# jasperlinthorst/reveal

Measured on AMD Instinct MI355X. Metric: Mbp/s indexed+MUM-anchored (reveal rem), higher is better.
Workload: dtype int32

## Files before the change

### include/reveal_amd.h

```cpp
#ifndef REVEAL_AMD_H
#define REVEAL_AMD_H
#include <stdint.h>

#ifdef __cplusplus
extern "C" {
#endif

typedef struct rv_index rv_index;

const char *rv_last_error(void);
int  rv_abi_version(void);
int  rv_sa_bits(void);
int  rv_device_count(void);

rv_index *rv_new(int device);
void rv_free(rv_index *h);

int rv_add_sample(rv_index *h);
int rv_add_sequence(rv_index *h, const char *seq, int64_t len, int64_t *begin, int64_t *end);
int rv_reset(rv_index *h);
int rv_reserve_text(rv_index *h, int64_t bytes);
int64_t rv_n(const rv_index *h);
int rv_nsamples(const rv_index *h);
int rv_nnodes(const rv_index *h);
int rv_add_sequences(rv_index *h, const char *text, int64_t total, const int64_t *lens, int64_t count);
int rv_node_list(const rv_index *h, int64_t *begin_end);

int rv_construct(rv_index *h, int rc, const char *safile, const char *lcpfile, int cache);
int rv_upload(rv_index *h);
int rv_upload_again(rv_index *h);

enum { RV_T = 0, RV_SA = 1, RV_SAI = 2, RV_LCP = 3, RV_SO = 4, RV_NSEP = 5, RV_NODES = 6 };
int64_t rv_get_array(rv_index *h, int which, void *out, int64_t cap);

int64_t rv_getmums(rv_index *h, int minl);
int rv_fetch_mums(rv_index *h, uint32_t *l, int64_t *a, int64_t *b, int64_t cap);
int64_t rv_getmultimums(rv_index *h, int minlength, int minn, int mems, int64_t *members);
int rv_fetch_multi(rv_index *h, uint32_t *l, int32_t *n, int64_t *off, uint16_t *so, int64_t *pos);

typedef struct {
    int64_t n;
    int32_t depth;
    int32_t nsamples;
    int32_t nnodes;
    int32_t parent;
    int32_t kind;
    int32_t reserved;
    int64_t nmums;
    int64_t nmembers;
} rv_sub;

int rv_align_begin(rv_index *h, int minl, int minn);
int rv_frontier_size(rv_index *h);
int rv_frontier_scan(rv_index *h);
int rv_sub_skip_scan(rv_index *h, int s);
int rv_sub_info(rv_index *h, int s, rv_sub *out);
int rv_sub_nodes(rv_index *h, int s, int64_t *begin_end );
int rv_sub_mums(rv_index *h, int s, uint32_t *l, int32_t *n, int64_t *off, uint16_t *so, int64_t *pos);
int64_t rv_sub_array(rv_index *h, int s, int which, void *out, int64_t cap);
int rv_sub_split(rv_index *h, int s, uint32_t l, int nsp, const int64_t *sp,
                 const int64_t *lead, int nlead, const int64_t *trail, int ntrail,
                 const int64_t *match, int nmatch, const int64_t *rest, int nrest);
int rv_frontier_commit(rv_index *h, int32_t *children);
int rv_align_end(rv_index *h);

typedef struct {
    int64_t steps;
    int64_t splits;
    int64_t anchored_bp;
    int32_t levels;
    int32_t maxdepth;
    int64_t scanned_ranks;
    double  t_scan, t_host, t_split, t_bubble;
} rv_align_stats;
int rv_align_builtin(rv_index *h, int minl, int minn, rv_align_stats *st);

int rv_align_builtin_until(rv_index *h, int minl, int minn, int stop_subs, rv_align_stats *st);
int rv_align_builtin_resume(rv_index *h, rv_align_stats *st);
int rv_align_builtin_continue(rv_index *h, int stop_subs, rv_align_stats *st);
int rv_frontier_counts(rv_index *h, int64_t *out);
int rv_frontier_export(rv_index *h, int64_t *meta, int64_t *node_first, int64_t *nodes);
int64_t rv_frontier_pack(rv_index *h, const int32_t *subs, int k, void *sa, void *lcp, void *bwt, int on_device);
int rv_frontier_import(rv_index *h, int minl, int minn, uint32_t maxlcp, int level, int nsubs, const int64_t *meta,
                       const int64_t *node_first, const int64_t *nodes, int64_t m,
                       const void *sa, const void *lcp, const void *bwt, int on_device);
int64_t rv_frontier_seeds_export(rv_index *h, const int32_t *subs, int k, int64_t *out, int64_t cap);
int rv_frontier_seeds_import(rv_index *h, int nsubs, const int64_t *words, int64_t nwords);
uint32_t rv_maxlcp(const rv_index *h);
int rv_cascade_info(const rv_index *h, int64_t *out);
int rv_capacity_events(const rv_index *h, int64_t *out);
const char *rv_cascade_why(const rv_index *h);
int64_t rv_anchor_count(rv_index *h, int64_t *members);
int rv_fetch_anchors(rv_index *h, uint32_t *l, int64_t *off, int64_t *pos);
int rv_set_result_buffers(rv_index *h, uint32_t *l, int64_t l_cap, int64_t *off, int64_t off_cap, int64_t *pos, int64_t pos_cap);
typedef struct {
    int64_t  key, n;
    int32_t  depth, nsamples, nnodes, picked;
    int64_t  nmums;
    uint32_t l; int32_t mn;
    int64_t  sp_min;
    uint64_t h_sa, h_lcp, h_mums;
} rv_trace;
int rv_set_trace(rv_index *h, int on);
int rv_set_preselect(rv_index *h, int64_t maxmums);
int rv_set_option(rv_index *h, const char *name, int64_t value);
int rv_get_option(rv_index *h, const char *name, int64_t *value);
int rv_set_launch_trace(int on);
int rv_option_count(void);
const char *rv_option_name(int k);
int64_t rv_trace_count(rv_index *h);
int rv_fetch_trace(rv_index *h, rv_trace *out, int64_t cap);

typedef struct rv_subindex rv_subindex;
rv_index *rv_clone(rv_index *h);
rv_subindex *rv_sx_main(rv_index *h);
rv_subindex *rv_sx_copy(rv_subindex *x);
void rv_sx_free(rv_subindex *x);
int rv_sx_info(const rv_subindex *x, rv_sub *out);
int rv_sx_nodes(const rv_subindex *x, int64_t *begin_end);
int64_t rv_sx_array(rv_subindex *x, int which, void *out, int64_t cap);
int64_t rv_sx_scan(rv_subindex *x, int minl, int minn, int64_t *members);
int rv_sx_fetch(rv_subindex *x, uint32_t *l, int32_t *n, int64_t *off, uint16_t *so, int64_t *pos);
int rv_sx_split(rv_subindex *x, const int64_t *lead, int nlead, const int64_t *trail, int ntrail,
                const int64_t *match, int nmatch, const int64_t *rest, int nrest, rv_subindex **out);
int rv_sx_extract(rv_subindex *x, int64_t *intervals, int niv);

int64_t rv_chain(int64_t m, int k, const uint32_t *len, const int32_t *nmem, const int64_t *crd, const int64_t *left,
                 const int64_t *right, int64_t wscore, int64_t wpen, int model, int64_t *out_idx, int64_t *out_score);

typedef struct { int64_t wscore, wpen, maxmums, seedsize; int gcmodel; int trim; double pcutoff; } rv_picker_args;
typedef struct {
    int picked; uint32_t pick_l; int32_t pick_n; int pick_members; uint16_t *pick_so; int64_t *pick_pos; int64_t member_cap;
    int64_t nleft, nright, nseed_members, seed_cap, seed_member_cap;
    uint32_t *seed_l; int32_t *seed_n; int64_t *seed_off; uint16_t *seed_so; int64_t *seed_pos; int64_t *seed_score; uint8_t *seed_right;
} rv_picker_out;
int rv_set_picker(rv_index *h, int kind, const rv_picker_args *args);
int rv_picker_info(const rv_index *h, int64_t *out);
int rv_pick_chain(const rv_picker_args *args, int nsub, int64_t m, const uint32_t *l, const int32_t *n, const int64_t *off, const uint16_t *so,
                  const int64_t *pos, int nsamples, const int64_t *seq_begin, const int64_t *iv_begin, const int64_t *iv_end, int minlength,
                  rv_picker_out *out);

typedef struct rv_graph rv_graph;
rv_graph *rv_graph_import(int64_t nnodes, const int64_t *node_b, const int64_t *node_e, const int8_t *node_aligned, const int8_t *node_sent,
                          const int64_t *off_ptr, const int32_t *off_sid, const int64_t *off_val,
                          int64_t nedges, const int32_t *edge_u, const int32_t *edge_v, const int64_t *edge_ptr, const int32_t *edge_paths,
                          const int64_t *pred_ptr, const int32_t *pred_edge, int npaths, const uint8_t *star, const int64_t *id2end,
                          int nstart, const int32_t *start_nodes, int literal_segments);
int rv_graph_pick(rv_graph *g, const rv_picker_args *args, int nsub, int64_t m, const uint32_t *l, const int32_t *n, const int64_t *off, const uint16_t *so, const int64_t *pos,
                  const int64_t *left, const int64_t *right, int minlength, rv_picker_out *out);
int rv_graph_align(rv_graph *g, const int64_t *nodes, int64_t nn, const int64_t *left, const int64_t *right, uint32_t l, const int64_t *pos, int npos,
                   int64_t *counts, int64_t *out6);
int rv_graph_align_fetch(rv_graph *g, int64_t *out);
int rv_set_graph_picker(rv_index *h, rv_graph *g, const rv_picker_args *args);
rv_graph *rv_graph_new(void);
int rv_graph_add_linear(rv_graph *g, int64_t b, int64_t e, int star);
int64_t rv_graph_read_gfa(rv_graph *g, rv_index *h, int64_t *text_n, const char *data, int64_t len, const char **names);
typedef struct GfaParsed rv_gfa_parsed;
rv_gfa_parsed *rv_gfa_parse(const char *data, int64_t len);
int64_t rv_graph_adopt(rv_graph *g, rv_index *h, int64_t *text_n, rv_gfa_parsed *parsed, const char **names);
void rv_gfa_parsed_free(rv_gfa_parsed *parsed);
int rv_graph_seal(rv_graph *g);
int rv_graph_paths(const rv_graph *g, int64_t *id2end);
int rv_graph_node_kinds(const rv_graph *g, int8_t *out);
int rv_graph_literal(const rv_graph *g);
int rv_graph_finish(rv_graph *g);
rv_graph *rv_graph_replay_begin(int nseq, const int64_t *begin, const int64_t *end);
int rv_set_replay_graph(rv_index *h, rv_graph *g);
rv_graph *rv_graph_replay(int nseq, const int64_t *begin, const int64_t *end, int64_t na, const uint32_t *an_l, const int64_t *an_off, const int64_t *an_pos);
const char *rv_graph_error(const rv_graph *g);
int rv_graph_sizes(const rv_graph *g, int64_t *out);
int rv_graph_export(const rv_graph *g, int64_t *node_b, int64_t *node_e, int8_t *node_aligned, int64_t *off_ptr, int32_t *off_sid, int64_t *off_val,
                    int64_t *succ_ptr, int32_t *succ_to, int32_t *succ_edge, int64_t *pred_ptr, int32_t *pred_from, int32_t *pred_edge, int64_t *edge_ptr, int32_t *edge_paths);
int rv_graph_prune(rv_graph *g, const char *T);
int64_t rv_graph_gfa(rv_graph *g, const char *T, int npaths, const char *const *names, const char *cmdline, const char **out);
void rv_graph_free(rv_graph *g);

enum { RV_K_SCAN_PAIR = 0, RV_K_SCAN_MULTI = 1, RV_K_SA_SORT = 2, RV_K_LCP = 3, RV_K_SPLIT = 4, RV_K_LABEL = 5,
       RV_K_BUBBLE = 6,
       RV_K_RADIX_SCATTER = 7, RV_K_RADIX_HIST = 8, RV_K_TEXT_ROUND = 9,
       RV_K_CASCADE = 10,
       RV_K_DIAG_TABLE = 11,
       RV_K_INIT_KEYS = 12,
       RV_K_PUBLISH = 13,
       RV_K_COUNT = 14 };
int rv_prof_enable(rv_index *h, int on);
int rv_prof_reset(rv_index *h);
int rv_prof_get(rv_index *h, int k, int64_t *launches, double *ms, double *bytes);
typedef struct rv_batch rv_batch;
rv_batch *rv_batch_new(void);
int rv_batch_add(rv_batch *b, rv_index *h);
int rv_batch_run(rv_batch *b, int minl, int minn, int construct, rv_align_stats *stats, int *status);
int rv_batch_info(const rv_batch *b, int64_t *out);
void rv_batch_free(rv_batch *b);
typedef struct rv_many rv_many;
rv_many *rv_many_new(int device);
void rv_many_free(rv_many *m);
int rv_many_option(rv_many *m, const char *name, int64_t value);
int rv_many_set_picker(rv_many *m, int kind, const rv_picker_args *args);
int64_t rv_many_add(rv_many *m, const char *const *seqs, const int64_t *lens, int k);
int rv_many_clear(rv_many *m);
int rv_many_run(rv_many *m, int minl, int minn, rv_align_stats *total);
int64_t rv_many_anchor_count(rv_many *m, int64_t *first, int64_t *members);
int rv_many_fetch(rv_many *m, uint32_t *l, int64_t *off, int64_t *pos);
int64_t rv_many_text(rv_many *m, int64_t job, char *out, int64_t cap);
int rv_many_info(const rv_many *m, int64_t *out);
int64_t rv_many_arrays(rv_many *m, int64_t job, int which, void *out, int64_t cap);
void *rv_dev_alloc(int device, int64_t bytes);
int rv_dev_free(int device, void *p);
int rv_ipc_export(int device, const void *p, uint8_t handle[64]);
void *rv_ipc_open(int device, const uint8_t handle[64]);
int rv_ipc_close(int device, void *p);
int rv_dev_copy(int device, void *dst, const void *src, int64_t bytes);
int rv_measure_bandwidth(int device, int64_t bytes, int iters, double *read_gbs, double *copy_gbs);
int rv_sa_stats(rv_index *h, int *sigma, int *bits, int *k0, int *rounds, int64_t *sorted_elems, int *radix_passes);
int rv_sa_diag_table(rv_index *h);
int rv_sa_tail(rv_index *h, int64_t *out);

int rv_test_exclusive_sum_u32(const uint32_t *in, uint32_t *out, int64_t n);
int rv_test_inclusive_max_u32(const uint32_t *in, uint32_t *out, int64_t n);
int rv_test_radix_sort(uint64_t *keys, uint32_t *vals, int64_t n, int bit_lo, int bit_hi);
int rv_test_radix_time(int64_t n, int bits, int dist, int flags, int iters, double *ms, int64_t *bad);

#ifdef __cplusplus
}
#endif
#endif
```

### reveal_amd/_index.py

```python
import ctypes
import mmap
import os
import sys
import numpy as np

from . import _lib
from ._lib import RV_T, RV_SA, RV_SAI, RV_LCP, RV_SO, RV_NSEP


def _page_array(count, dtype):
    nbytes = max(int(count), 1) * np.dtype(dtype).itemsize
    m = mmap.mmap(-1, (nbytes + mmap.PAGESIZE - 1) // mmap.PAGESIZE * mmap.PAGESIZE)
    return np.frombuffer(m, dtype=dtype, count=max(int(count), 1))


def _pairs(iv, sa64):
    a = np.ascontiguousarray(np.array([(int(b), int(e)) for b, e in iv], dtype=np.int64).reshape(-1, 2))
    return a, len(a)


_OPTION_DEFAULTS = {}


def make_index_type(sa64, error):
# ... 426 lines not shown
            if self._dll.rv_sx_extract(sx, a.ctypes.data, k) != 0:
                self._fail()
            if isinstance(intervals, list):
                for q in range(k):
                    if (a[q] != before[q]).any():
                        intervals[q] = (int(a[q][0]), int(a[q][1]))
            return None

        def copy(self):
            if not self._constructed:
                raise TypeError("Index not yet constructed.")
            if self._slot is not None:
                raise error("not available on a sub-index handed to an align() callback")
            c = index.__new__(index)
            c._lib, c._dll = self._lib, self._dll
            c._safile, c._lcpfile, c._cache = "", "", 0
            c._samples, c._nodes, c.skipmums = list(self._samples), set(self._nodes), list(self.skipmums)
            c._leftnode, c._rightnode, c._depth = self._leftnode, self._rightnode, self._depth
            c._constructed, c._slot, c._sx = True, None, None
            c._n_sub = c._nsamples_sub = None
            c._rc = getattr(self, "_rc", 0)
            if self._main is self:
                if self._sx:
                    raise error("copy() after extract() / splitindex() on the main index is not supported")
                c._h = self._dll.rv_clone(self._h)
                if not c._h:
                    self._fail()
                c._main = c
            else:
                c._h, c._main = self._h, self._main
                c._samples = self._main._samples
                c._sx = self._dll.rv_sx_copy(self._sx)
                if not c._sx:
                    self._fail()
            return c

        def preselect(self, maxmums):
            if self._depth != 0:
                raise error("preselect() is set on the main index")
            if self._dll.rv_set_preselect(self._h, int(maxmums or 0)) != 0:
                self._fail()

        def align_builtin(self, minl=20, minn=2, trace=False):
            if not self._constructed:
                raise error("Index not yet constructed, alignment stopped.")
            dll, h = self._dll, self._h
            dll.rv_set_trace(h, 1 if trace else 0)
            self._offer_result_buffers()
            st = _lib.RvAlignStats()
            if dll.rv_align_builtin(h, int(minl), int(minn), ctypes.byref(st)) != 0:
                self._fail()
            return self._builtin_result(st, trace)

        def set_picker(self, args=None):
            from . import schemes
            if args is None:
                r = self._dll.rv_set_picker(self._h, 0, None)
            else:
                if args.maxsize is not None or args.maxdepth is not None:
                    raise error("the native picker does not take --maxbubblesize / maxdepth")
                A = schemes._RvPickerArgs(int(args.wscore), int(args.wpen), int(args.maxmums or 0), int(args.seedsize or 0), schemes.GCMODELS[args.gcmodel],
                                          1 if args.trim else 0, float(args.pcutoff))
                r = self._dll.rv_set_picker(self._h, 1, ctypes.byref(A))
            if r != 0:
                self._fail()

        def set_replay_graph(self, graph=None):
            if graph is not None and graph._dll is not self._dll:
                raise error("the graph was made by the other build of the library (32 / 64-bit suffix arrays)")
            if self._dll.rv_set_replay_graph(self._h, None if graph is None else graph._g) != 0:
                self._fail()

        def _sync_nodes(self):
            self._nodes_stale = False
            k = self._dll.rv_nnodes(self._h)
            if k != len(self._nodes):
                buf = np.zeros(2 * max(k, 1), np.int64)
                if self._dll.rv_node_list(self._h, buf.ctypes.data) != 0:
                    self._fail()
                self._nodes = set(map(tuple, buf[:2 * k].reshape(-1, 2).tolist()))
                self._constructed = False

        def set_graph_picker(self, graph=None, args=None):
            from . import schemes
            if graph is None:
                r = self._dll.rv_set_graph_picker(self._h, None, None)
            else:
                if args.maxsize is not None or args.maxdepth is not None:
                    raise error("the native picker does not take --maxbubblesize / maxdepth")
                if graph._dll is not self._dll:
                    raise error("the graph was made by the other build of the library (32 / 64-bit suffix arrays)")
                A = schemes._RvPickerArgs(int(args.wscore), int(args.wpen), int(args.maxmums or 0), int(args.seedsize or 0), schemes.GCMODELS[args.gcmodel],
                                          1 if args.trim else 0, float(args.pcutoff))
                r = self._dll.rv_set_graph_picker(self._h, graph._g, ctypes.byref(A))
            if r != 0:
                self._fail()

        def picker_info(self):
            o = (ctypes.c_int64 * 6)()
            self._dll.rv_picker_info(self._h, o)
            return dict(kind=int(o[0]), calls=int(o[1]), seeded=int(o[2]), picker_s=o[3] / 1e9, lists_s=o[4] / 1e9, graphalign_s=o[5] / 1e9)

        def _result_buffers_free(self):
            c = self.__dict__.get("_res_bufs")
            if c is not None and sys.getrefcount(c[0]) == 2 and sys.getrefcount(c[1]) == 2 and sys.getrefcount(c[2]) == 2:
                return c
            return None

        def _offer_result_buffers(self):
            c = self._result_buffers_free()
            if c is not None:
                self._dll.rv_set_result_buffers(self._h, c[0].ctypes.data, len(c[0]), c[1].ctypes.data, len(c[1]), c[2].ctypes.data, len(c[2]))
            else:
                self._dll.rv_set_result_buffers(self._h, None, 0, None, 0, None, 0)

        def _builtin_result(self, st, trace):
            dll, h = self._dll, self._h
            mem = ctypes.c_int64(0)
            na = dll.rv_anchor_count(h, ctypes.byref(mem))
            c = self._result_buffers_free()
            if c is not None and len(c[0]) >= max(na, 1) and len(c[1]) >= na + 1 and len(c[2]) >= max(mem.value, 1):
                l, off, pos = c
            else:
                dll.rv_set_result_buffers(h, None, 0, None, 0, None, 0)
                if os.environ.get("RV_RESULT_BUFS", "") == "heap":
                    l = np.empty(max(na, 1), dtype=np.uint32); off = np.empty(na + 1, dtype=np.int64); pos = np.empty(max(mem.value, 1), dtype=np.int64)
                else:
                    l = _page_array(max(na, 1), np.uint32); off = _page_array(na + 1, np.int64); pos = _page_array(max(mem.value, 1), np.int64)
                self.__dict__["_res_bufs"] = (l, off, pos)
            c = None
            off[0] = 0
            if dll.rv_fetch_anchors(h, l.ctypes.data, off.ctypes.data, pos.ctypes.data) != 0:
                self._fail()
            tr = None
            if trace:
                nt = dll.rv_trace_count(h)
                tr = np.zeros(max(nt, 1), dtype=_lib.TRACE_DTYPE)
                if dll.rv_fetch_trace(h, tr.ctypes.data, len(tr)) != 0:
                    self._fail()
                tr = tr[:nt]
            stats = {f[0]: getattr(st, f[0]) for f in _lib.RvAlignStats._fields_}
            return dict(stats=stats, anchors=(l[:na], off[:na + 1], pos[:mem.value]), trace=tr)

        @property
        def maxlcp(self):
            return int(self._dll.rv_maxlcp(self._h))

        def cascade_info(self):
            o = np.zeros(8, dtype=np.int64)
            self._dll.rv_cascade_info(self._h, o.ctypes.data)
            return dict(done=bool(o[0]), levels=int(o[1]), matches=int(o[2]), witnesses=int(o[3]), subindices=int(o[4]), undecided=int(o[5]), rebuilt_ranks=int(o[6]), decided_from_witnesses=int(o[7]),
                        why=(self._dll.rv_cascade_why(self._h) or b"").decode())

        def capacity_events(self):
            o = np.zeros(len(_lib.CAPACITY_EVENTS), dtype=np.int64)
            if self._dll.rv_capacity_events(self._main._h, o.ctypes.data) != 0:
                self._fail()
            return {k: int(v) for k, v in zip(_lib.CAPACITY_EVENTS, o)}

        def align_builtin_until(self, stop_subs, minl=20, minn=2, trace=False):
            if not self._constructed:
                raise error("Index not yet constructed, alignment stopped.")
            self._dll.rv_set_trace(self._h, 1 if trace else 0)
            self._offer_result_buffers()
            self._st = _lib.RvAlignStats()
            self._trace = bool(trace)
            r = self._dll.rv_align_builtin_until(self._h, int(minl), int(minn), int(stop_subs), ctypes.byref(self._st))
            if r < 0:
                self._fail()
            self._pending = r > 0
            return r

        def align_builtin_continue(self, stop_subs):
            if not getattr(self, "_pending", False):
                return 0
            self._offer_result_buffers()
            r = self._dll.rv_align_builtin_continue(self._h, int(stop_subs), ctypes.byref(self._st))
            if r < 0:
                self._fail()
            self._pending = r > 0
            return r

        def frontier(self):
            c = np.zeros(4, dtype=np.int64)
            if self._dll.rv_frontier_counts(self._h, c.ctypes.data) != 0:
                self._fail()
            ns, m, nn, level = (int(x) for x in c)
            meta = np.zeros((max(ns, 1), 6), dtype=np.int64); nf = np.zeros(ns + 1, dtype=np.int64); nodes = np.zeros((max(nn, 1), 2), dtype=np.int64)
            if self._dll.rv_frontier_export(self._h, meta.ctypes.data, nf.ctypes.data, nodes.ctypes.data) != 0:
                self._fail()
            return dict(level=level, m=m, meta=meta[:ns], node_first=nf, nodes=nodes[:nn])

        def frontier_pack(self, subs, sa, lcp, bwt):
            subs = np.ascontiguousarray(subs, dtype=np.int32)
            ptr, dev = _pointers(sa, lcp, bwt)
            r = self._dll.rv_frontier_pack(self._h, subs.ctypes.data, len(subs), ptr[0], ptr[1], ptr[2], dev)
            if r < 0:
                self._fail()
            return int(r)

        def frontier_seeds(self, subs):
            subs = np.ascontiguousarray(subs, dtype=np.int32)
            need = self._dll.rv_frontier_seeds_export(self._h, subs.ctypes.data, len(subs), None, 0)
            if need < 0:
                self._fail()
            out = np.zeros(max(int(need), 1), dtype=np.int64)
            if self._dll.rv_frontier_seeds_export(self._h, subs.ctypes.data, len(subs), out.ctypes.data, int(need)) != need:
                self._fail()
            return out[:int(need)]

        def frontier_import(self, part, sa, lcp, bwt, minl=20, minn=2, maxlcp=None, trace=False):
            meta = np.ascontiguousarray(part["meta"], dtype=np.int64).reshape(-1, 6)
            nf = np.ascontiguousarray(part["node_first"], dtype=np.int64); nodes = np.ascontiguousarray(part["nodes"], dtype=np.int64).reshape(-1, 2)
            m = int(meta[:, 1].sum()) if len(meta) else 0
            ptr, dev = _pointers(sa, lcp, bwt)
            self._offer_result_buffers()
            if not getattr(self, "_pending", False):
                self._dll.rv_set_trace(self._h, 1 if trace else 0)
                self._st = _lib.RvAlignStats()
                self._trace = bool(trace)
            ml = self.maxlcp if maxlcp is None else int(maxlcp)
            if self._dll.rv_frontier_import(self._h, int(minl), int(minn), ml, int(part.get("level", 1)), len(meta), meta.ctypes.data, nf.ctypes.data,
                                            nodes.ctypes.data, m, ptr[0], ptr[1], ptr[2], dev) != 0:
                self._fail()
            self._pending = True
            seeds = part.get("seeds")
            if seeds is not None and len(seeds) > len(meta):
                seeds = np.ascontiguousarray(seeds, dtype=np.int64)
                if self._dll.rv_frontier_seeds_import(self._h, len(meta), seeds.ctypes.data, len(seeds)) != 0:
                    self._fail()

        def align_builtin_resume(self):
            if getattr(self, "_pending", False):
                self._offer_result_buffers()
                if self._dll.rv_align_builtin_resume(self._h, ctypes.byref(self._st)) != 0:
                    self._fail()
            self._pending = False
            return self._builtin_result(self._st, self._trace)

        def _fetch_sub_mums(self, s, info):
            cnt, mem = info.nmums, info.nmembers
            l = np.zeros(max(cnt, 1), dtype=np.uint32); n = np.zeros(max(cnt, 1), dtype=np.int32)
            off = np.zeros(cnt + 1, dtype=np.int64)
            so = np.zeros(max(mem, 1), dtype=np.uint16); pos = np.zeros(max(mem, 1), dtype=np.int64)
            if self._dll.rv_sub_mums(self._h, s, l.ctypes.data, n.ctypes.data, off.ctypes.data, so.ctypes.data, pos.ctypes.data) != 0:
                self._fail()
            return _csr_to_tuples(cnt, l, n, off, so, pos)

        def __reduce__(self):
            return None

    index.__name__ = "index"
    index.__qualname__ = "index"
    return index


def _pointers(*bufs):
    ptr, dev = [], None
    for b in bufs:
        on_dev = bool(getattr(b, "is_cuda", False))
        if dev is not None and on_dev != dev:
            raise ValueError("sa, lcp and bwt must live in the same kind of memory")
        dev = on_dev
        if hasattr(b, "data_ptr"):
            if not b.is_contiguous():
                raise ValueError("contiguous buffers needed")
            ptr.append(b.data_ptr())
        else:
            if not b.flags["C_CONTIGUOUS"]:
                raise ValueError("contiguous buffers needed")
            ptr.append(b.ctypes.data)
    return ptr, 1 if dev else 0


def _csr_to_tuples(cnt, l, n, off, so, pos):
    l, n, off = l.tolist(), n.tolist(), off.tolist()
    members = list(zip(so.tolist(), pos.tolist()))
    return [(l[k], n[k], tuple(members[off[k]:off[k + 1]])) for k in range(cnt)]
```

### reveal_amd/_lib.py

```python
import ctypes
import importlib.util
import os
import sys
import numpy as np

_HERE = os.path.dirname(os.path.abspath(__file__))

RV_T, RV_SA, RV_SAI, RV_LCP, RV_SO, RV_NSEP, RV_NODES = range(7)
K_SCAN_PAIR, K_SCAN_MULTI, K_SA_SORT, K_LCP, K_SPLIT, K_LABEL, K_BUBBLE, K_RADIX_SCATTER, K_RADIX_HIST, K_TEXT_ROUND, K_CASCADE, K_DIAG_TABLE, K_INIT_KEYS, K_PUBLISH = range(14)

CAPACITY_EVENTS = ("pair_ovf", "pair_out", "pair_pick_ovf", "pair_second_copy", "multi_rec", "multi_mem", "multi_cand",
                   "mems_rec", "mems_mem", "mems_long")
CAP_SITES = {"multi_cand": 1, "cas_wit": 2, "cas_tables": 4, "casm_matches": 8, "casm_wit": 16, "casm_tables": 32,
             "mems_rec": 64, "mems_mem": 128, "mems_long": 256}

c_i64p = ctypes.POINTER(ctypes.c_int64)
V = ctypes.c_void_p


class RvSub(ctypes.Structure):
    _fields_ = [("n", ctypes.c_int64), ("depth", ctypes.c_int32), ("nsamples", ctypes.c_int32),
                ("nnodes", ctypes.c_int32), ("parent", ctypes.c_int32), ("kind", ctypes.c_int32),
                ("reserved", ctypes.c_int32), ("nmums", ctypes.c_int64), ("nmembers", ctypes.c_int64)]


class RvAlignStats(ctypes.Structure):
    _fields_ = [("steps", ctypes.c_int64), ("splits", ctypes.c_int64), ("anchored_bp", ctypes.c_int64),
                ("levels", ctypes.c_int32), ("maxdepth", ctypes.c_int32), ("scanned_ranks", ctypes.c_int64),
                ("t_scan", ctypes.c_double), ("t_host", ctypes.c_double), ("t_split", ctypes.c_double),
                ("t_bubble", ctypes.c_double)]


TRACE_DTYPE = np.dtype([("key", np.int64), ("n", np.int64), ("depth", np.int32), ("nsamples", np.int32),
                        ("nnodes", np.int32), ("picked", np.int32), ("nmums", np.int64), ("l", np.uint32),
                        ("mn", np.int32), ("sp_min", np.int64), ("h_sa", np.uint64), ("h_lcp", np.uint64),
                        ("h_mums", np.uint64)], align=True)

_I, _L, _D = ctypes.c_int, ctypes.c_int64, ctypes.c_double
SYMBOLS = {
    "rv_last_error": (ctypes.c_char_p, []),
    "rv_abi_version": (_I, []),
    "rv_sa_bits": (_I, []),
    "rv_device_count": (_I, []),
    "rv_new": (V, [_I]),
    "rv_free": (None, [V]),
    "rv_add_sample": (_I, [V]),
    "rv_add_sequence": (_I, [V, ctypes.c_char_p, _L, c_i64p, c_i64p]),
    "rv_reset": (_I, [V]),
    "rv_reserve_text": (_I, [V, _L]),
    "rv_n": (_L, [V]),
    "rv_nsamples": (_I, [V]),
    "rv_nnodes": (_I, [V]),
    "rv_node_list": (_I, [V, V]),
    "rv_construct": (_I, [V, _I, ctypes.c_char_p, ctypes.c_char_p, _I]),
    "rv_upload": (_I, [V]),
    "rv_upload_again": (_I, [V]),
    "rv_get_array": (_L, [V, _I, V, _L]),
    "rv_getmums": (_L, [V, _I]),
    "rv_fetch_mums": (_I, [V, V, V, V, _L]),
    "rv_getmultimums": (_L, [V, _I, _I, _I, c_i64p]),
    "rv_fetch_multi": (_I, [V, V, V, V, V, V]),
    "rv_align_begin": (_I, [V, _I, _I]),
    "rv_frontier_size": (_I, [V]),
    "rv_frontier_scan": (_I, [V]),
    "rv_sub_skip_scan": (_I, [V, _I]),
    "rv_sub_info": (_I, [V, _I, ctypes.POINTER(RvSub)]),
    "rv_sub_nodes": (_I, [V, _I, V]),
    "rv_sub_mums": (_I, [V, _I, V, V, V, V, V]),
    "rv_sub_array": (_L, [V, _I, _I, V, _L]),
    "rv_sub_split": (_I, [V, _I, ctypes.c_uint32, _I, V, V, _I, V, _I, V, _I, V, _I]),
    "rv_frontier_commit": (_I, [V, V]),
    "rv_align_end": (_I, [V]),
    "rv_align_builtin": (_I, [V, _I, _I, ctypes.POINTER(RvAlignStats)]),
    "rv_align_builtin_until": (_I, [V, _I, _I, _I, ctypes.POINTER(RvAlignStats)]),
    "rv_align_builtin_resume": (_I, [V, ctypes.POINTER(RvAlignStats)]),
    "rv_align_builtin_continue": (_I, [V, _I, ctypes.POINTER(RvAlignStats)]),
    "rv_frontier_counts": (_I, [V, V]),
    "rv_frontier_export": (_I, [V, V, V, V]),
    "rv_frontier_pack": (_L, [V, V, _I, V, V, V, _I]),
    "rv_frontier_import": (_I, [V, _I, _I, ctypes.c_uint32, _I, _I, V, V, V, _L, V, V, V, _I]),
    "rv_frontier_seeds_export": (_L, [V, V, _I, V, _L]),
    "rv_frontier_seeds_import": (_I, [V, _I, V, _L]),
    "rv_maxlcp": (ctypes.c_uint32, [V]),
    "rv_cascade_info": (ctypes.c_int, [V, V]),
    "rv_cascade_why": (ctypes.c_char_p, [V]),
    "rv_capacity_events": (_I, [V, V]),
    "rv_anchor_count": (_L, [V, c_i64p]),
    "rv_fetch_anchors": (_I, [V, V, V, V]),
    "rv_set_result_buffers": (_I, [V, V, _L, V, _L, V, _L]),
    "rv_set_trace": (_I, [V, _I]),
    "rv_set_preselect": (_I, [V, _L]),
    "rv_set_option": (_I, [V, ctypes.c_char_p, _L]),
    "rv_set_launch_trace": (_I, [_I]),
    "rv_batch_new": (V, []),
    "rv_batch_add": (_I, [V, V]),
    "rv_batch_run": (_I, [V, _I, _I, _I, V, V]),
    "rv_batch_info": (_I, [V, V]),
    "rv_batch_free": (None, [V]),
    "rv_dev_alloc": (V, [_I, _L]),
    "rv_dev_free": (_I, [_I, V]),
    "rv_ipc_export": (_I, [_I, V, V]),
    "rv_ipc_open": (V, [_I, V]),
    "rv_ipc_close": (_I, [_I, V]),
    "rv_dev_copy": (_I, [_I, V, V, _L]),
    "rv_get_option": (_I, [V, ctypes.c_char_p, c_i64p]),
    "rv_option_count": (_I, []),
    "rv_option_name": (ctypes.c_char_p, [_I]),
    "rv_trace_count": (_L, [V]),
    "rv_fetch_trace": (_I, [V, V, _L]),
    "rv_clone": (V, [V]),
    "rv_sx_main": (V, [V]),
    "rv_sx_copy": (V, [V]),
    "rv_sx_free": (None, [V]),
    "rv_sx_info": (_I, [V, ctypes.POINTER(RvSub)]),
    "rv_sx_nodes": (_I, [V, V]),
    "rv_sx_array": (_L, [V, _I, V, _L]),
    "rv_sx_scan": (_L, [V, _I, _I, c_i64p]),
    "rv_sx_fetch": (_I, [V, V, V, V, V, V]),
    "rv_sx_split": (_I, [V, V, _I, V, _I, V, _I, V, _I, V]),
    "rv_sx_extract": (_I, [V, V, _I]),
    "rv_chain": (_L, [_L, _I, V, V, V, V, V, _L, _L, _I, V, V]),
    "rv_prof_enable": (_I, [V, _I]),
    "rv_prof_reset": (_I, [V]),
    "rv_prof_get": (_I, [V, _I, c_i64p, ctypes.POINTER(_D), ctypes.POINTER(_D)]),
    "rv_measure_bandwidth": (_I, [_I, _L, _I, ctypes.POINTER(_D), ctypes.POINTER(_D)]),
    "rv_sa_stats": (_I, [V] + [ctypes.POINTER(_I)] * 4 + [c_i64p, ctypes.POINTER(_I)]),
    "rv_sa_diag_table": (_I, [V]),
    "rv_sa_tail": (_I, [V, c_i64p]),
    "rv_set_picker": (_I, [V, _I, V]),
    "rv_picker_info": (_I, [V, c_i64p]),
    "rv_pick_chain": (_I, [V, _I, _L, V, V, V, V, V, _I, V, V, V, _I, V]),
    "rv_graph_import": (V, [_L, V, V, V, V, V, V, V, _L, V, V, V, V, V, V, _I, V, V, _I, V, _I]),
    "rv_graph_pick": (_I, [V, V, _I, _L, V, V, V, V, V, V, V, _I, V]),
    "rv_graph_align": (_I, [V, V, _L, V, V, ctypes.c_uint32, V, _I, V, V]),
    "rv_graph_align_fetch": (_I, [V, V]),
    "rv_graph_finish": (_I, [V]),
    "rv_set_graph_picker": (_I, [V, V, V]),
    "rv_graph_new": (V, []),
    "rv_graph_replay_begin": (V, [_I, V, V]),
    "rv_set_replay_graph": (_I, [V, V]),
    "rv_graph_add_linear": (_I, [V, _L, _L, _I]),
    "rv_graph_read_gfa": (_L, [V, V, V, V, _L, V]),
    "rv_graph_paths": (_I, [V, V]),
    "rv_graph_seal": (_I, [V]),
    "rv_gfa_parse": (V, [V, _L]),
    "rv_graph_adopt": (_L, [V, V, V, V, V]),
    "rv_gfa_parsed_free": (None, [V]),
    "rv_add_sequences": (_I, [V, V, _L, V, _L]),
    "rv_graph_node_kinds": (_I, [V, V]),
    "rv_graph_literal": (_I, [V]),
    "rv_graph_replay": (V, [_I, V, V, _L, V, V, V]),
    "rv_graph_error": (ctypes.c_char_p, [V]),
    "rv_graph_sizes": (_I, [V, c_i64p]),
    "rv_graph_export": (_I, [V] * 15),
    "rv_graph_prune": (_I, [V, V]),
    "rv_graph_gfa": (_L, [V, V, _I, V, V, V]),
    "rv_graph_free": (None, [V]),
    "rv_many_new": (V, [_I]),
    "rv_many_free": (None, [V]),
    "rv_many_option": (_I, [V, ctypes.c_char_p, _L]),
    "rv_many_set_picker": (_I, [V, _I, V]),
    "rv_many_add": (_L, [V, V, V, _I]),
    "rv_many_clear": (_I, [V]),
    "rv_many_run": (_I, [V, _I, _I, ctypes.POINTER(RvAlignStats)]),
    "rv_many_anchor_count": (_L, [V, V, c_i64p]),
    "rv_many_fetch": (_I, [V, V, V, V]),
    "rv_many_text": (_L, [V, _L, V, _L]),
    "rv_many_info": (_I, [V, V]),
    "rv_many_arrays": (_L, [V, _L, _I, V, _L]),
    "rv_test_exclusive_sum_u32": (_I, [V, V, _L]),
    "rv_test_inclusive_max_u32": (_I, [V, V, _L]),
    "rv_test_radix_sort": (_I, [V, V, _L, _I, _I]),
    "rv_test_radix_time": (_I, [_L, _I, _I, _I, _I, ctypes.POINTER(_D), c_i64p]),
}


def _share_torch_runtime():
    if os.environ.get("RV_SYSTEM_HIP") or "torch" in sys.modules:
        return
    try:
        spec = importlib.util.find_spec("torch")
    except (ImportError, ValueError):
        spec = None
    if spec is None or not spec.origin:
        return
    path = os.path.join(os.path.dirname(spec.origin), "lib", "libamdhip64.so")
    if os.path.exists(path):
        ctypes.CDLL(path, mode=ctypes.RTLD_GLOBAL)


class Lib:
    def __init__(self, sa64=False):
        self.sa64 = sa64
        _share_torch_runtime()
        name = "libreveal_amd64.so" if sa64 else "libreveal_amd.so"
        self.path = os.path.join(os.environ.get("RV_LIB_DIR") or _HERE, name)
        if not os.path.exists(self.path):
            raise ImportError("%s is missing: build it with `python -c 'import __graft_entry__ as g; g.build()'` "
                              "(hipcc --offload-arch=gfx950); reveal_amd has no CPU fallback" % self.path)
        self.dll = ctypes.CDLL(self.path)
        for sym, (res, args) in SYMBOLS.items():
            fn = getattr(self.dll, sym)
            fn.restype, fn.argtypes = res, args
        self.sa_t = np.int64 if sa64 else np.int32
        self.lcp_t = np.uint32 if sa64 else np.int32
        assert self.dll.rv_sa_bits() == (64 if sa64 else 32)
        v = os.environ.get("RV_LAUNCH_TRACE")
        if v is not None and v.strip() not in ("", "0"):
            self.dll.rv_set_launch_trace(1)

    def err(self):
        return (self.dll.rv_last_error() or b"").decode(errors="replace")


_libs = {}
_device = 0


def set_device(i):
    global _device
    _device = int(i)


def device():
    return _device


def measure_bandwidth(nbytes=1 << 30, iters=10):
    lib = get(False)
    r, c = _D(0), _D(0)
    if lib.dll.rv_measure_bandwidth(device(), int(nbytes), int(iters), ctypes.byref(r), ctypes.byref(c)) != 0:
        raise RuntimeError(lib.err())
    return r.value, c.value


def set_launch_trace(on=True):
    return [bool(get(w).dll.rv_set_launch_trace(1 if on else 0)) for w in (False, True)]
# ... 7 lines not shown
```

### reveal_amd/csrc/rv_align.hip

```cpp
#include "rv_index.h"
#include "rv_split.h"
#include "rv_decide.h"
static_assert(RV_TSUB_TILE == RV_SPLIT_TILE, "one tile -> sub-index table serves the split passes and the multi-sample picker");
#include "rv_leaf.h"
#include "rv_cascade.h"
#include <string.h>
#include <algorithm>
#include <chrono>
#include <thread>
#include <atomic>
#include "rv_graphrem.h"

namespace {

double now_s() {
    return std::chrono::duration<double>(std::chrono::steady_clock::now().time_since_epoch()).count();
}

u64 hash_step(u64 acc, u64 i, int64_t v) {
    u64 x = (u64)v + (i + 1) * 0x9E3779B97F4A7C15ULL;
    x ^= x >> 30; x *= 0xbf58476d1ce4e5b9ULL;
    x ^= x >> 27; x *= 0x94d049bb133111ebULL;
    x ^= x >> 31;
    return acc + x;
// ... 1799 lines not shown
        th.emplace_back([=]() { for (size_t k = lo; k < hi; k++) off[k] = base + 2 * (int64_t)(k + 1); });
    }
    for (size_t k = 0; k < na / nt; k++) off[k] = base + 2 * (int64_t)(k + 1);
    for (auto &x : th) x.join();
}
static int builtin_finish(rv_index *h, rv_align_stats *out) {
    Align *a = h->al;
    hipStream_t q = h->ws.stream;
    h->rb.direct = false;
    if (a->use_leaf && a->running) {
        u32 *lf_counters = a->lf_counters; u32 *lf_l = a->lf_l; int64_t *lf_pos = a->lf_pos; rv_trace *lf_tr = a->lf_tr;
        RV_HIP(hipStreamSynchronize(a->leaf_stream));
        RV_HIP(hipStreamSynchronize(a->leaf_stream2));
        for (int k = 0; k <= RV_LEVEL_BUFS; k++) a->leaf_pending[k] = false;
        RV_TRY(a->hLeafOut.reserve(256));
        RV_HIP(hipMemcpyAsync(a->hLeafOut.p, lf_counters, 128, hipMemcpyDeviceToHost, q));
        RV_HIP(hipStreamSynchronize(q));
        u32 cnt[4]; unsigned long long stv[8];
        memcpy(cnt, a->hLeafOut.p, sizeof cnt); memcpy(stv, a->hLeafOut.as<uint8_t>() + 64, sizeof stv);
        if (h->ws.opt.leaf_prof)
            fprintf(stderr, "leaf: steps %llu splits %llu | cycles idle %llu scan %llu split %llu bubble %llu\n", stv[0], stv[1], stv[4], stv[5], stv[6], stv[7]);
        if (cnt[2]) { rv_set_error(cnt[2] & 4u ? "leaf kernel: recursion stack overflow" : "leaf kernel: a sub-index does not match its intervals"); return -1; }
        if (cnt[0] > a->leaf_anchor_cap || cnt[1] > a->leaf_trace_cap) { rv_set_error("leaf kernel: output buffer too small"); return -1; }
        a->leaf_na = 0;
        if (cnt[0]) {
            const size_t na = cnt[0];
            const size_t nl = a->an_l.size(), np = a->an_pos.size();
            rv_index::ResultBufs &rb = h->rb;
            rb.direct = rb.l && (int64_t)(nl + na) <= rb.l_cap && (int64_t)(nl + na + 1) <= rb.off_cap && (int64_t)(np + 2 * na) <= rb.pos_cap;
            int64_t *pp; u32 *pl;
            if (rb.direct) { pp = rb.pos + np; pl = rb.l + nl; }
            else { RV_TRY(a->hLeafOut.reserve(na * 20 + 64)); pp = a->hLeafOut.as<int64_t>(); pl = (u32 *)(pp + 2 * na); }
            const size_t sent = (rb.direct && a->early_l == pl && a->early_pos == pp) ? std::min(a->early_sent, na) : 0;
            if (sent < na) {
                RV_HIP(hipMemcpyAsync(pp + 2 * sent, lf_pos + 2 * sent, (na - sent) * 16, hipMemcpyDeviceToHost, a->leaf_stream));
                RV_HIP(hipMemcpyAsync(pl + sent, lf_l + sent, (na - sent) * 4, hipMemcpyDeviceToHost, a->leaf_stream));
            }
            RV_TRY(rv_ensure_working_text(h));
            RV_TRY(rv_leaf_lower_launch(h->ws, h->dT.as<uint8_t>(), lf_pos, lf_l, (u32)na));
            if (rb.direct) fill_offsets(rb.off + nl + 1, na, (int64_t)np);
            RV_HIP(hipStreamSynchronize(a->leaf_stream));
            RV_HIP(hipStreamSynchronize(q));
            a->leaf_na = na;
        }
        if (a->trace_on && cnt[1]) {
            const size_t at = a->trace.size();
            a->trace.resize(at + cnt[1]);
            RV_HIP(hipMemcpy(a->trace.data() + at, lf_tr, (size_t)cnt[1] * sizeof(rv_trace), hipMemcpyDeviceToHost));
        }
        a->st.steps += (int64_t)stv[0]; a->st.splits += (int64_t)stv[1]; a->st.anchored_bp += (int64_t)stv[2];
        if ((int64_t)stv[3] > a->st.maxdepth) a->st.maxdepth = (int32_t)stv[3];
    }
    a->running = false;
    if (out) *out = a->st;
    return 0;
}

static int install_frontier(rv_index *h, int level, int nsubs, const int64_t *meta, const int64_t *node_first, const int64_t *nodes, int64_t m,
                            const void *sa, const void *lcp, const void *bwt, int on_device);
static int builtin_cascade(rv_index *h) {
    Align *a = h->al;
    memset(&a->cas_out, 0, sizeof a->cas_out);
    if (a->trace_on || h->rc != 0 || h->n <= RV_LEAF_N || a->minl < 4 || h->ws.opt.no_cascade || a->picker != 0) return 0;
    const bool second_try = !a->multi && a->use_leaf && h->ws.opt.cascade_second == 2;
    auto interval_cascade = [&]() -> int {
        RvCascadeMultiOut mo;
        RV_TRY(rv_cascade_multi_run(h, a->cas, a->minl, &mo));
        a->cas_out.done = mo.done; a->cas_out.levels = mo.levels; a->cas_out.cands = mo.cands; a->cas_out.witnesses = mo.witnesses; a->cas_out.children = mo.children;
        a->cas_out.undecided = mo.undecided; a->cas_out.rebuilt_ranks = mo.rebuilt_ranks; a->cas_out.why = mo.why;
        if (!mo.done) return 0;
        const int k = h->nsamples;
        a->st.splits += (int64_t)mo.an_l.size(); a->st.steps += mo.steps; a->st.levels += mo.levels; a->st.scanned_ranks += h->n;
        if (mo.maxdepth > a->st.maxdepth) a->st.maxdepth = mo.maxdepth;
        h->main_arrays_freed = true;
        if (mo.undecided > 0) {
            RV_TRY(install_frontier(h, 1, (int)mo.undecided, mo.meta.data(), mo.node_first.data(), mo.nodes.data(), mo.rebuilt_ranks, mo.d_sa, mo.d_lcp, mo.d_bwt, 1));
        } else {
            a->lv.clear();
            a->level = 1;
        }
        {
            const size_t na = mo.an_l.size(), l0 = a->an_l.size(), p0 = a->an_pos.size(), o0 = a->an_off.size();
            a->an_l.insert(a->an_l.end(), mo.an_l.begin(), mo.an_l.end());
            a->an_pos.resize(p0 + na * (size_t)k);
            for (size_t x = 0; x < na * (size_t)k; x++) a->an_pos[p0 + x] = (int64_t)mo.an_pos[x];
            a->an_off.resize(o0 + na);
            for (size_t x = 0; x < na; x++) a->an_off[o0 + x] = (int64_t)(p0 + (x + 1) * (size_t)k);
            int64_t bp = 0;
            for (size_t x = 0; x < na; x++) bp += mo.an_l[x];
            a->st.anchored_bp += bp;
            (void)l0;
        }
        return 0;
    };
    if (a->multi || second_try) return interval_cascade();
    if (!a->use_leaf) return 0;
    RvCascadeIO io;
    io.anchor_count = a->lf_counters; io.anchor_cap = (u32)a->leaf_anchor_cap; io.anchor_l = a->lf_l; io.anchor_pos = a->lf_pos;
    io.stats = a->lf_stats; io.leaf_err = a->lf_counters + 2;
    io.stage_cap = (u32)h->ws.opt.leaf_acap;
    RvCascadeHost hx;
    hx.side = a->leaf_stream;
    a->early_sent = 0;
    if (h->rb.l) {
        const int64_t nl = (int64_t)a->an_l.size(), np = (int64_t)a->an_pos.size();
        const int64_t room = std::min(std::min(h->rb.l_cap - nl, h->rb.off_cap - nl - 1), (h->rb.pos_cap - np) / 2);
        if (room > 0) { hx.l = h->rb.l + nl; hx.pos = h->rb.pos + np; hx.cap = (u32)std::min<int64_t>(room, 0xffffffffll); }
    }
    io.lvSA = &a->lvSA[0]; io.lvLCP = &a->lvLCP[0]; io.lvBWT = &a->lvBWT[0]; io.roots = &a->dLeafRoots[0];
    const int dmode = (int)h->ws.opt.cascade_danger;
    RV_TRY(rv_cascade_run(h, a->cas, io, a->minl, &a->cas_out, dmode == 2 ? 1 : 0, 0, &hx));
    if (!a->cas_out.done && a->cas_out.undecided > 0 && dmode == 1) {
        RV_HIP(hipMemsetAsync(a->dLeaf.p, 0, 256, h->ws.stream));
        RV_TRY(rv_cascade_run(h, a->cas, io, a->minl, &a->cas_out, 1, 1, &hx));
    }
    if (!a->cas_out.done) {
        if (hx.l) RV_HIP(hipStreamSynchronize(a->leaf_stream));
        RV_HIP(hipMemsetAsync(a->dLeaf.p, 0, 256, h->ws.stream));
        if (a->cas_out.undecided > 0 && !h->ws.opt.cascade_second_off) return interval_cascade();
        return 0;
    }
    a->st.levels += a->cas_out.levels;
    a->st.scanned_ranks += h->n;
    a->early_sent = a->cas_out.sent; a->early_l = hx.l; a->early_pos = hx.pos;
    if (!a->cas.lin_rest.empty() && h->nodes.size() > 2) {
        std::vector<RvIntv> rest, gone;
        for (size_t k = 0; k + 1 < a->cas.lin_rest.size(); k += 2) rest.push_back({a->cas.lin_rest[k], a->cas.lin_rest[k + 1]});
        std::sort(rest.begin(), rest.end(), intv_less);
        for (const RvIntv &v : h->nodes) {
            if (v.end <= v.begin) continue;
            const auto it = std::lower_bound(rest.begin(), rest.end(), v, intv_less);
            if (it == rest.end() || it->begin != v.begin) gone.push_back(v);
        }
        RV_TRY(add_decision(h, 0, 0, nullptr, 0, gone.data(), (int)gone.size(), nullptr, 0, nullptr, 0, rest.data(), (int)rest.size()));
        a->dec.drop_lead = true;
        RV_TRY(rv_frontier_commit(h, nullptr));
        for (size_t s2 = 0; s2 < a->lv.depth.size(); s2++) a->lv.depth[s2] = a->cas.lin_rest_depth;
        return 0;
    }
    h->main_arrays_freed = true;
    a->level = 1;
    a->lv.clear();
    return 0;
}

int rv_cascade_info(const rv_index *h, int64_t *out) {
    for (int k = 0; k < 8; k++) out[k] = 0;
    if (!h->al) return 0;
    const RvCascadeOut &c = h->al->cas_out;
    out[0] = c.done ? 1 : 0; out[1] = c.levels; out[2] = c.cands; out[3] = c.witnesses; out[4] = c.children; out[5] = c.undecided; out[6] = c.rebuilt_ranks; out[7] = c.solved;
    return 0;
}

const char *rv_cascade_why(const rv_index *h) {
    if (!h->al || h->al->cas_out.done || !h->al->cas_out.why) return "";
    return h->al->cas_out.why;
}

int rv_align_builtin(rv_index *h, int minl, int minn, rv_align_stats *out) {
    RV_TRY(builtin_setup(h, minl, minn));
    Align *a = h->al;
    if (a->replay_graph && a->picker == 1) {
        a->feed = rv_replay_feed_start(a->replay_graph);
        a->fed = 0;
        a->replay_graph = nullptr;
        if (!a->feed) return -1;
    }
    int rc = builtin_cascade(h);
    if (rc == 0) rc = builtin_levels(h, 0);
    if (rc == 0) rc = builtin_finish(h, out);
    if (a->feed) {
        RvReplayFeed *f = a->feed; a->feed = nullptr;
        if (rc == 0) { if (rv_replay_feed_finish(f) != 0) return -1; }
        else { const std::string keep = rv_last_error(); (void)rv_replay_feed_finish(f); rv_set_error("%s", keep.c_str()); }
    }
    return rc;
}

int rv_align_builtin_until(rv_index *h, int minl, int minn, int stop_subs, rv_align_stats *out) {
    RV_TRY(builtin_setup(h, minl, minn));
    RV_TRY(builtin_cascade(h));
    RV_TRY(builtin_levels(h, stop_subs));
    Align *a = h->al;
    if (a->lv.size() == 0) { RV_TRY(builtin_finish(h, out)); return 0; }
    if (out) *out = a->st;
    return a->lv.size();
}

int rv_align_builtin_continue(rv_index *h, int stop_subs, rv_align_stats *out) {
    RV_TRY(need_align(h));
    if (!h->al->running) { rv_set_error("no built-in run in progress (rv_align_builtin_until / rv_frontier_import)"); return -1; }
    if (stop_subs < 1) { rv_set_error("rv_align_builtin_continue: stop_subs must be positive"); return -1; }
    RV_HIP(hipSetDevice(h->device));
    Align *a = h->al;
    RV_TRY(builtin_levels(h, std::max(stop_subs, a->lv.size() + 1)));
    if (a->lv.size() == 0) { RV_TRY(builtin_finish(h, out)); return 0; }
    if (out) *out = a->st;
    return a->lv.size();
}

int rv_align_builtin_resume(rv_index *h, rv_align_stats *out) {
    RV_TRY(need_align(h));
    if (!h->al->running) { rv_set_error("no built-in run in progress (rv_align_builtin_until / rv_frontier_import)"); return -1; }
    RV_HIP(hipSetDevice(h->device));
    RV_TRY(builtin_levels(h, 0));
    return builtin_finish(h, out);
}

int rv_frontier_counts(rv_index *h, int64_t *out) {
    RV_TRY(need_align(h));
    const Level &lv = h->al->lv;
    out[0] = lv.size(); out[1] = lv.size() ? lv.m : 0; out[2] = (int64_t)lv.nodes.size(); out[3] = h->al->level;
    return 0;
}

int rv_frontier_export(rv_index *h, int64_t *meta, int64_t *node_first, int64_t *nodes) {
    RV_TRY(need_align(h));
    if (h->al->picker == 2) { rv_set_error("rv_frontier_export: a run on a graph (rv_set_graph_picker) is not handed off -- its sub-indices share the graph"); return -1; }
    const Level &lv = h->al->lv;
    for (int s = 0; s < lv.size(); s++) {
        int64_t *m6 = meta + 6 * (size_t)s;
        m6[0] = lv.off[(size_t)s]; m6[1] = lv.n[(size_t)s]; m6[2] = lv.depth[(size_t)s]; m6[3] = lv.nsamples[(size_t)s]; m6[4] = lv.kind[(size_t)s]; m6[5] = lv.parent[(size_t)s];
    }
    for (size_t k = 0; k < lv.node_first.size(); k++) node_first[k] = lv.node_first[k];
    for (size_t k = 0; k < lv.nodes.size(); k++) { nodes[2 * k] = lv.nodes[k].begin; nodes[2 * k + 1] = lv.nodes[k].end; }
    return 0;
}

int64_t rv_frontier_pack(rv_index *h, const int32_t *subs, int k, void *sa, void *lcp, void *bwt, int on_device) {
    if (need_align(h)) return -1;
    Align *a = h->al;
    if (hipSetDevice(h->device) != hipSuccess) { rv_set_error("hipSetDevice failed"); return -1; }
    hipStream_t q = h->ws.stream;
    const Level &lv = a->lv;
    const hipMemcpyKind kind = on_device ? hipMemcpyDeviceToDevice : hipMemcpyDeviceToHost;
    int64_t at = 0;
    for (int i = 0; i < k;) {
        if (subs[i] < 0 || subs[i] >= lv.size()) { rv_set_error("sub-index %d out of range", (int)subs[i]); return -1; }
        int j = i;
        int64_t cnt = lv.n[(size_t)subs[i]];
        while (j + 1 < k && subs[j + 1] == subs[j] + 1) { j++; cnt += lv.n[(size_t)subs[j]]; }
        const int64_t off = lv.off[(size_t)subs[i]];
        hipError_t e = hipMemcpyAsync((sa_t *)sa + at, cur_sa(h) + off, (size_t)cnt * sizeof(sa_t), kind, q);
        if (e == hipSuccess) e = hipMemcpyAsync((lcp_t *)lcp + at, cur_lcp(h) + off, (size_t)cnt * sizeof(lcp_t), kind, q);
        if (e == hipSuccess) e = hipMemcpyAsync((uint8_t *)bwt + at, cur_bwt(h) + off, (size_t)cnt, kind, q);
        if (e != hipSuccess) { rv_set_error("rv_frontier_pack: copy failed: %s", hipGetErrorString(e)); return -1; }
        at += cnt;
        i = j + 1;
    }
    if (hipStreamSynchronize(q) != hipSuccess) { rv_set_error("rv_frontier_pack: stream failed"); return -1; }
    return at;
}

static int install_frontier(rv_index *h, int level, int nsubs, const int64_t *meta, const int64_t *node_first, const int64_t *nodes, int64_t m,
                            const void *sa, const void *lcp, const void *bwt, int on_device) {
    hipStream_t q = h->ws.stream;
    Align *a = h->al;
    RV_HIP(hipStreamSynchronize(q));
    if (a->leaf_stream) { RV_HIP(hipStreamSynchronize(a->leaf_stream)); RV_HIP(hipStreamSynchronize(a->leaf_stream2)); }
    for (int k = 0; k <= RV_LEVEL_BUFS; k++) a->leaf_pending[k] = false;
    RV_HIP(hipMemsetAsync(a->dErr.p, 0, 64, q));
    Level &lv = a->lv;
    lv.clear();
    int64_t off = 0;
    for (int s = 0; s < nsubs; s++) {
        const int64_t *m6 = meta + 6 * (size_t)s;
        const int64_t nf = node_first[s], nl = node_first[s + 1];
        if (m6[1] <= 0 || nf > nl) { rv_set_error("rv_frontier_import: bad sub-index %d", s); return -1; }
        lv.off.push_back(off); lv.n.push_back(m6[1]); lv.depth.push_back((int32_t)m6[2]); lv.nsamples.push_back((int32_t)m6[3]);
        lv.kind.push_back((int32_t)m6[4]); lv.parent.push_back(-1);
        for (int64_t k = nf; k < nl; k++) {
            if (nodes[2 * k] < 0 || nodes[2 * k + 1] > h->nT || nodes[2 * k] > nodes[2 * k + 1]) { rv_set_error("rv_frontier_import: interval outside the text"); return -1; }
            lv.nodes.push_back({nodes[2 * k], nodes[2 * k + 1]});
        }
        lv.node_first.push_back((int64_t)lv.nodes.size());
        off += m6[1];
    }
    if (off != m) { rv_set_error("rv_frontier_import: the sub-index sizes add up to %lld, not %lld", (long long)off, (long long)m); return -1; }
    lv.m = m;
    a->nx.clear();
    a->level = std::max(level, 1);
    a->cur = 0;
    RV_TRY(a->lvSA[0].reserve((size_t)(m + 64) * sizeof(sa_t)));
    RV_TRY(a->lvLCP[0].reserve((size_t)(m + 64) * sizeof(lcp_t)));
    RV_TRY(a->lvBWT[0].reserve((size_t)m + 64));
    const hipMemcpyKind kind = on_device ? hipMemcpyDeviceToDevice : hipMemcpyHostToDevice;
    if (m) {
        RV_HIP(hipMemcpyAsync(a->lvSA[0].p, sa, (size_t)m * sizeof(sa_t), kind, q));
        RV_HIP(hipMemcpyAsync(a->lvLCP[0].p, lcp, (size_t)m * sizeof(lcp_t), kind, q));
        RV_HIP(hipMemcpyAsync(a->lvBWT[0].p, bwt, (size_t)m, kind, q));
    }
    prep_level_tables(h, lv, m);
    a->pk.clear();
    RV_TRY(publish_next_tables(h, a->dTab0, lv.nsamples, false));
    RV_HIP(hipStreamSynchronize(q));
    a->cur_dev_ok = a->next_dev_ok; a->early_done = false; a->early_bubble = false;
    a->scanned = false; a->d_err = nullptr;
    a->dec.reset(lv.size());
    a->skip_scan.assign((size_t)lv.size(), 0);
    a->seeds_cur.clear(); a->seeds_lead.clear(); a->seeds_trail.clear();
    return 0;
}


int rv_frontier_import(rv_index *h, int minl, int minn, uint32_t maxlcp, int level, int nsubs, const int64_t *meta,
                       const int64_t *node_first, const int64_t *nodes, int64_t m, const void *sa, const void *lcp, const void *bwt, int on_device) {
// ... 431 lines not shown
```

### reveal_amd/csrc/rv_cascade.h

```cpp
#pragma once
#include "rv_common.h"
#include <vector>

struct RvCascadeBufs {
    DBuf d[40];
    HBuf hstage, hstage2;
    u32 M = 0, NW = 0;
    u32 lin_roots = 0, lin_picks = 0, lin_nA = 0, lin_nB = 0;
    int64_t lin_steps = 0; int lin_maxdepth = 0; size_t lin_off[6] = {0, 0, 0, 0, 0, 0};
    std::vector<int64_t> lin_rest; int lin_rest_depth = 0;
    hipStream_t prio_stream = nullptr; hipEvent_t ev_in = nullptr, ev_out = nullptr;
    void release() {
        for (auto &b : d) b.release(); hstage.release(); hstage2.release();
        if (prio_stream) { (void)hipStreamDestroy(prio_stream); prio_stream = nullptr; }
        if (ev_in) { (void)hipEventDestroy(ev_in); ev_in = nullptr; }
        if (ev_out) { (void)hipEventDestroy(ev_out); ev_out = nullptr; }
    }
};

struct RvCascadeIO {
    u32 *anchor_count; u32 anchor_cap; u32 *anchor_l; int64_t *anchor_pos;
    unsigned long long *stats;
    u32 *leaf_err;
    u32 stage_cap;
    DBuf *lvSA, *lvLCP, *lvBWT, *roots;
};

struct RvCascadeHost {
    hipStream_t side = nullptr;
    int64_t *pos = nullptr; u32 *l = nullptr; u32 cap = 0;
};

struct RvCascadeOut {
    bool done;
    int levels;
    int64_t cands, witnesses, children, undecided, rebuilt_ranks;
    int64_t solved, unsolved;
    const char *why;
    u32 sent;
};

#define RV_CASM_K 16
struct RvCascadeMultiOut {
    bool done; int levels; int64_t cands, witnesses, children, undecided, rebuilt_ranks, steps; int maxdepth; const char *why;
    int64_t big, big_ranks;
    std::vector<u32> an_l; std::vector<int64_t> an_pos;
    std::vector<int64_t> meta, node_first, nodes;
    const void *d_sa, *d_lcp, *d_bwt;
};

struct rv_index;
struct RvBatchGroup;
RvBatchGroup *rv_batch_group_new(int device);
void rv_batch_group_begin(RvBatchGroup *g, int total);
void rv_batch_group_leave(RvBatchGroup *g);
void rv_batch_group_free(RvBatchGroup *g);
void rv_batch_group_info(const RvBatchGroup *g, int64_t *out);
int rv_cascade_multi_run(rv_index *h, RvCascadeBufs &cb, int minl, RvCascadeMultiOut *out);
int rv_cascade_run(rv_index *h, RvCascadeBufs &cb, const RvCascadeIO &io, int minl, RvCascadeOut *out, int danger = 0, int reuse = 0,
                   const RvCascadeHost *host = nullptr);
```

### reveal_amd/csrc/rv_cascade.hip

```cpp
#include "rv_index.h"
#include "rv_cascade.h"
#include "rv_leaf.h"
#include <algorithm>
#include <string.h>
#include <stdio.h>
#include <stdlib.h>
#include <chrono>

namespace {

constexpr int TB = 256;
constexpr u32 NONE = 0xFFFFFFFFu;
#ifdef RV_SA64
constexpr int KEY_SHIFT = 40;
#else
constexpr int KEY_SHIFT = 32;
#endif
constexpr u64 KEY_LOW = (1ull << KEY_SHIFT) - 1;

struct CasIv { sa_t a0, a1, b0, b1; };
struct CasRes { sa_t qa, qb; u32 ql, lead, trail, state; };
enum { C_NCHILD = 0, C_NUND = 1, C_NWIT = 2, C_ERR = 3, C_MAXN = 4, C_LO = 5, C_HI = 6, C_LEVELS = 7, C_NSOLVED = 8, C_NUNSOLVED = 9, C_NRETRY = 10, C_TICKET = 11,
       C_NANCH = 12  };

__device__ inline bool cas_cut(const CasIv &iv, int64_t pa, int64_t pb, int64_t len, int64_t minl, int64_t *qa, int64_t *qb, int64_t *ql) {
    const int64_t ka = (int64_t)iv.a0 - pa, kb = (int64_t)iv.b0 - pb;
    int64_t k = ka > kb ? ka : kb;
    k = k > 0 ? k : 0;
    const int64_t a = pa + k, b = pb + k;
    int64_t l = len - k;
    const int64_t ra = (int64_t)iv.a1 - a, rb = (int64_t)iv.b1 - b;
    l = l < ra ? l : ra;
    l = l < rb ? l : rb;
    *qa = a; *qb = b; *ql = l;
    return l >= minl;
}
__device__ inline u64 cas_key(int64_t qa, int64_t ql) { return ((u64)ql << KEY_SHIFT) | (KEY_LOW - (u64)qa); }

__device__ inline u64 shfl_up64(u64 v, int d) {
    const u32 lo = __shfl_up((u32)v, d, 64), hi = __shfl_up((u32)(v >> 32), d, 64);
    return ((u64)hi << 32) | lo;
}
__device__ inline void seg_atomic_max64(u64 *__restrict__ dst, u32 child, u64 val, bool active) {
    const int lane = threadIdx.x & 63;
    if (!active) { child = NONE; val = 0; }
    val = rv_wave_seg_max_u64(child, val);
    const u32 nc = __shfl_down(child, 1, 64);
    const bool last = lane == 63 || nc != child;
    if (active && last && val > dst[child]) atomicMax((unsigned long long *)&dst[child], (unsigned long long)val);
}
__device__ inline void seg_atomic_max32(u32 *__restrict__ dst, u32 child, u32 val, bool active) {
    const int lane = threadIdx.x & 63;
    if (!active) { child = NONE; val = 0; }
    val = rv_wave_seg_max_u32(child, val);
    const u32 nc = __shfl_down(child, 1, 64);
    const bool last = lane == 63 || nc != child;
    if (active && last && val > dst[child]) atomicMax(&dst[child], val);
}

constexpr int WT_ITEMS = 8;
constexpr int WT_TILE = TB * WT_ITEMS;
constexpr int WT_REGIONS = RV_WIT_REGIONS;
__global__ __launch_bounds__(TB) void k_cas_witness(const sa_t *__restrict__ SA, const lcp_t *__restrict__ LCP, const uint8_t *__restrict__ BWT, int64_t n,
                                                    u32 minl, sa_t *__restrict__ w_pos, u32 *__restrict__ w_val, u32 *__restrict__ w_rank, u32 cap , u32 *__restrict__ counters ) {
    __shared__ __attribute__((aligned(16))) u32 sl0[WT_TILE + 8];
    __shared__ __attribute__((aligned(16))) uint8_t ss0[WT_TILE + 32];
    u32 *const sl = sl0 + 3;
    uint8_t *const ss = ss0 + 15;
    const int64_t j0 = (int64_t)blockIdx.x * WT_TILE;
    if (j0 + WT_TILE + 2 <= n && sizeof(lcp_t) == 4) {
        const uint4 *L4 = reinterpret_cast<const uint4 *>(LCP + j0);
        uint4 *d4 = reinterpret_cast<uint4 *>(sl + 1);
        for (int k = threadIdx.x; k < WT_TILE / 4; k += TB) d4[k] = L4[k];
        const uint4 *B4 = reinterpret_cast<const uint4 *>(BWT + j0);
        for (int k = threadIdx.x; k < WT_TILE / 16; k += TB) {
            uint4 v = B4[k];
            v.x = (v.x >> 7) & 0x01010101u; v.y = (v.y >> 7) & 0x01010101u; v.z = (v.z >> 7) & 0x01010101u; v.w = (v.w >> 7) & 0x01010101u;
            reinterpret_cast<uint4 *>(ss + 1)[k] = v;
        }
        if (threadIdx.x == 0) { sl[0] = j0 > 0 ? (u32)LCP[j0 - 1] : 0u; ss[0] = j0 > 0 ? (uint8_t)(BWT[j0 - 1] >> 7) : (uint8_t)0; }
        if (threadIdx.x == 1) { sl[WT_TILE + 1] = (u32)LCP[j0 + WT_TILE]; ss[WT_TILE + 1] = (uint8_t)(BWT[j0 + WT_TILE] >> 7); }
        if (threadIdx.x == 2) sl[WT_TILE + 2] = (u32)LCP[j0 + WT_TILE + 1];
    } else {
        for (int k = threadIdx.x; k < WT_TILE + 3; k += TB) { const int64_t j = j0 - 1 + k; sl[k] = (j >= 0 && j < n) ? (u32)LCP[j] : 0u; }
        for (int k = threadIdx.x; k < WT_TILE + 2; k += TB) { const int64_t j = j0 - 1 + k; ss[k] = (j >= 0 && j < n) ? (uint8_t)(BWT[j] >> 7) : (uint8_t)0; }
    }
    __syncthreads();
    const int lane = threadIdx.x & 63;
    const u64 lt = (lane == 0) ? 0ull : (~0ull >> (64 - lane));
#pragma unroll 1
    for (int r = 0; r < WT_ITEMS; r++) {
        const int k = r * TB + threadIdx.x;
        const int64_t j = j0 + k;
        const u32 lm1 = sl[k], l0 = sl[k + 1], l1 = sl[k + 2], l2 = sl[k + 3];
        const u32 sm1 = ss[k], s0 = ss[k + 1], s1 = ss[k + 2];
        const bool pair0 = (j >= 1) & (l0 > lm1) & (l0 > l1) & (s0 != sm1);
        const bool pair1 = (j + 1 < n) & (l1 > l0) & (l1 > l2) & (s1 != s0);
        const u32 w = pair0 ? (lm1 > l1 ? lm1 : l1) : pair1 ? (l0 > l2 ? l0 : l2) : (l0 > l1 ? l0 : l1);
        const bool hit = (j < n) & (w >= minl);
        const u64 bal = __ballot(hit);
        if (bal) {
            const u32 reg = blockIdx.x & (WT_REGIONS - 1);
            u32 base = 0;
            if (lane == 0) base = atomicAdd(&counters[reg], (u32)__popcll(bal));
            base = (u32)__shfl((int)base, 0, 64);
            if (hit) {
                const u32 i = base + (u32)__popcll(bal & lt);
                if (i < cap) { w_pos[(size_t)reg * cap + i] = SA[j]; w_val[(size_t)reg * cap + i] = w; w_rank[(size_t)reg * cap + i] = (u32)j; }
            }
        }
    }
}
__global__ __launch_bounds__(TB) void k_cas_wpack(const sa_t *__restrict__ src_pos, const u32 *__restrict__ src_val, const u32 *__restrict__ src_rank, u32 rcap,
                                                  const u32 *__restrict__ region_cnt, const u32 *__restrict__ region_off, sa_t *__restrict__ w_pos, u32 *__restrict__ w_val,
                                                  u32 *__restrict__ w_rank) {
    const u32 reg = blockIdx.y, i = blockIdx.x * TB + threadIdx.x;
    if (i >= region_cnt[reg]) return;
    const size_t f = (size_t)reg * rcap + i;
    const u32 o = region_off[reg] + i;
    w_pos[o] = src_pos[f]; w_val[o] = src_val[f]; w_rank[o] = src_rank[f];
}
__global__ __launch_bounds__(TB) void k_cas_wkeys(const u32 *__restrict__ w_rank, u32 NW, u64 *__restrict__ keys, u32 *__restrict__ vals) {
    const u32 i = blockIdx.x * TB + threadIdx.x;
    if (i < NW) { keys[i] = (u64)w_rank[i]; vals[i] = i; }
}
__global__ __launch_bounds__(TB) void k_cas_wgather(const sa_t *__restrict__ src_pos, const u32 *__restrict__ src_val, const u32 *__restrict__ perm, u32 NW,
                                                    sa_t *__restrict__ w_pos, u32 *__restrict__ w_val) {
    const u32 i = blockIdx.x * TB + threadIdx.x;
    if (i < NW) { const u32 f = perm[i]; w_pos[i] = src_pos[f]; w_val[i] = src_val[f]; }
}

__global__ __launch_bounds__(TB) void k_cas_keys(const RvPairRec *__restrict__ recs, u32 M, u64 *__restrict__ keys, u32 *__restrict__ vals) {
    const u32 i = blockIdx.x * TB + threadIdx.x;
    if (i < M) { keys[i] = (u64)recs[i].a; vals[i] = i; }
}
__global__ __launch_bounds__(TB) void k_cas_gather(const RvPairRec *__restrict__ recs, const u32 *__restrict__ perm, u32 M, sa_t *__restrict__ c_pa,
                                                   sa_t *__restrict__ c_pb, u32 *__restrict__ c_len, u32 *__restrict__ c_child) {
    const u32 i = blockIdx.x * TB + threadIdx.x;
    if (i >= M) return;
    const RvPairRec r = recs[perm[i]];
    c_pa[i] = r.a; c_pb[i] = r.b; c_len[i] = r.l; c_child[i] = 0u;
}
__global__ void k_cas_init(CasIv *__restrict__ iv, u64 *__restrict__ best, u32 *__restrict__ wmax, int32_t *__restrict__ depth, CasRes *__restrict__ res,
                           u32 *__restrict__ counters, CasIv root, u32 *__restrict__ w_child, u32 nw, u64 *__restrict__ dbest, u32 *__restrict__ dflag, u64 *__restrict__ dceil) {
    const u32 i = blockIdx.x * blockDim.x + threadIdx.x;
    if (i == 0) {
        if (dbest) { dbest[0] = 0; dflag[0] = 0; dceil[0] = 0; }
        iv[0] = root; best[0] = 0; wmax[0] = 0; depth[0] = 0;
        CasRes r; r.qa = 0; r.qb = 0; r.ql = 0; r.lead = NONE; r.trail = NONE; r.state = 0;
        res[0] = r;
        counters[C_NCHILD] = 1; counters[C_NUND] = 0; counters[C_ERR] = 0; counters[C_MAXN] = 0; counters[C_LO] = 0; counters[C_HI] = 1; counters[C_LEVELS] = 0; counters[C_NSOLVED] = 0; counters[C_NUNSOLVED] = 0; counters[C_NRETRY] = 0; counters[C_TICKET] = 0;
    }
    if (i < nw) w_child[i] = 0u;
}

struct CasRootTabs { const sa_t *beginA, *beginB; const int32_t *pickA, *pickB; const u32 *rootLead, *rootTrail; u32 nA, nB; };
__device__ inline int cas_contig_of(const sa_t *__restrict__ begins, u32 cnt, int64_t pos) {
    u32 lo = 0, hi = cnt;
    while (lo < hi) { const u32 mid = (lo + hi) >> 1; if ((int64_t)begins[mid] <= pos) lo = mid + 1; else hi = mid; }
    return (int)lo - 1;
}
__global__ void k_cas_init_roots(CasIv *__restrict__ iv, u64 *__restrict__ best, u32 *__restrict__ wmax, int32_t *__restrict__ depth, CasRes *__restrict__ res,
                                 u32 *__restrict__ counters, const CasIv *__restrict__ roots, const int32_t *__restrict__ rdepth, u32 nroots,
                                 u64 *__restrict__ dbest, u32 *__restrict__ dflag, u64 *__restrict__ dceil) {
    const u32 i = blockIdx.x * blockDim.x + threadIdx.x;
    if (i == 0) {
        counters[C_NCHILD] = nroots; counters[C_NUND] = 0; counters[C_ERR] = 0; counters[C_MAXN] = 0; counters[C_LO] = 0; counters[C_HI] = nroots; counters[C_LEVELS] = 0;
        counters[C_NSOLVED] = 0; counters[C_NUNSOLVED] = 0; counters[C_NRETRY] = 0; counters[C_TICKET] = 0;
    }
    if (i < nroots) {
        if (dbest) { dbest[i] = 0; dflag[i] = 0; dceil[i] = 0; }
        iv[i] = roots[i]; best[i] = 0; wmax[i] = 0; depth[i] = rdepth[i];
        CasRes r; r.qa = 0; r.qb = 0; r.ql = 0; r.lead = NONE; r.trail = NONE; r.state = 0;
        res[i] = r;
    }
}
__global__ __launch_bounds__(TB) void k_cas_assign_roots(const sa_t *__restrict__ c_pa, const sa_t *__restrict__ c_pb, const u32 *__restrict__ c_len, u32 *__restrict__ c_child, u32 M,
                                                         const sa_t *__restrict__ w_pos, u32 *__restrict__ w_child, u32 NW, const CasIv *__restrict__ roots, CasRootTabs t, int64_t minl) {
    const u32 i = blockIdx.x * TB + threadIdx.x;
    if (i < M) {
        const int64_t pa = (int64_t)c_pa[i], pb = (int64_t)c_pb[i], len = (int64_t)c_len[i];
        const int ca = cas_contig_of(t.beginA, t.nA, pa), cb = cas_contig_of(t.beginB, t.nB, pb);
        u32 c = NONE;
        if (ca >= 0 && cb >= 0 && t.pickA[ca] >= 0 && t.pickA[ca] == t.pickB[cb]) {
            const u32 k = (u32)t.pickA[ca];
            int64_t qa, qb, ql;
            if (t.rootLead[k] != NONE && cas_cut(roots[t.rootLead[k]], pa, pb, len, minl, &qa, &qb, &ql)) c = t.rootLead[k];
            else if (t.rootTrail[k] != NONE && cas_cut(roots[t.rootTrail[k]], pa, pb, len, minl, &qa, &qb, &ql)) c = t.rootTrail[k];
        }
        c_child[i] = c;
    }
    if (i < NW) {
        const int64_t pos = (int64_t)w_pos[i];
        const bool a_side = t.nB == 0 || pos < (int64_t)t.beginB[0];
        const int ct = a_side ? cas_contig_of(t.beginA, t.nA, pos) : cas_contig_of(t.beginB, t.nB, pos);
        u32 c = NONE;
        if (ct >= 0) {
            const int32_t k = a_side ? t.pickA[ct] : t.pickB[ct];
            if (k >= 0) {
                for (int which = 0; which < 2 && c == NONE; which++) {
                    const u32 r = which ? t.rootTrail[k] : t.rootLead[k];
                    if (r == NONE) continue;
                    const CasIv p = roots[r];
                    if ((pos >= (int64_t)p.a0 && pos < (int64_t)p.a1) || (pos >= (int64_t)p.b0 && pos < (int64_t)p.b1)) c = r;
                }
            }
        }
        w_child[i] = c;
    }
}
__global__ void k_cas_lineage_stats(unsigned long long *__restrict__ stats, unsigned long long steps, unsigned long long maxdepth) {
    if (threadIdx.x == 0 && blockIdx.x == 0) { atomicAdd(&stats[0], steps); atomicMax(&stats[3], maxdepth); }
}
__global__ __launch_bounds__(TB) void k_cas_lkeys(const sa_t *__restrict__ c_pa, const u32 *__restrict__ c_len, u32 M, u64 *__restrict__ keys, u32 *__restrict__ vals) {
    const u32 i = blockIdx.x * TB + threadIdx.x;
    if (i < M) { keys[i] = (((1ull << (64 - KEY_SHIFT)) - 1ull - (u64)c_len[i]) << KEY_SHIFT) | (u64)c_pa[i]; vals[i] = i; }
}
__global__ __launch_bounds__(TB) void k_cas_lgather(const sa_t *__restrict__ c_pa, const sa_t *__restrict__ c_pb, const u32 *__restrict__ c_len, const u32 *__restrict__ perm, u32 M,
                                                    sa_t *__restrict__ o_pa, sa_t *__restrict__ o_pb, u32 *__restrict__ o_len) {
    const u32 i = blockIdx.x * TB + threadIdx.x;
    if (i < M) { const u32 f = perm[i]; o_pa[i] = c_pa[f]; o_pb[i] = c_pb[f]; o_len[i] = c_len[f]; }
}

constexpr int CAS_ITEMS = 4;
__global__ __launch_bounds__(TB) void k_cas_assign(const sa_t *__restrict__ c_pa, const sa_t *__restrict__ c_pb, const u32 *__restrict__ c_len, u32 *__restrict__ c_child,
                                                   u32 M, const sa_t *__restrict__ w_pos, const u32 *__restrict__ w_val, u32 *__restrict__ w_child, u32 NW,
                                                   const CasIv *__restrict__ iv, const CasRes *__restrict__ res, u64 *__restrict__ best, u32 *__restrict__ wmax,
                                                   int64_t minl, int first, const u64 *__restrict__ ceil ) {
    const u32 mblocks = (M + TB * CAS_ITEMS - 1) / (TB * CAS_ITEMS);
    for (int it = 0; it < CAS_ITEMS; it++) {
    if (blockIdx.x < mblocks) {
        const u32 i = (blockIdx.x * CAS_ITEMS + (u32)it) * TB + threadIdx.x;
        u32 c = i < M ? c_child[i] : NONE;
        bool live = c != NONE;
        u64 key = 0;
        if (live) {
            const int64_t pa = (int64_t)c_pa[i], pb = (int64_t)c_pb[i], len = (int64_t)c_len[i];
            int64_t qa, qb, ql;
            if (!first) {
                const CasRes r = res[c];
                const CasIv p = iv[c];
                u32 nc = NONE;
                if (r.state == 1u) {
                    CasIv lv; lv.a0 = p.a0; lv.a1 = r.qa; lv.b0 = p.b0; lv.b1 = r.qb;
                    CasIv tv; tv.a0 = (sa_t)((int64_t)r.qa + r.ql); tv.a1 = p.a1; tv.b0 = (sa_t)((int64_t)r.qb + r.ql); tv.b1 = p.b1;
                    if (r.lead != NONE && cas_cut(lv, pa, pb, len, minl, &qa, &qb, &ql)) nc = r.lead;
                    else if (r.trail != NONE && cas_cut(tv, pa, pb, len, minl, &qa, &qb, &ql)) nc = r.trail;
                } else if (r.state == 3u) {
                    if (cas_cut(p, pa, pb, len, minl, &qa, &qb, &ql)) nc = r.lead;
                }
                c = nc;
                c_child[i] = c;
                live = c != NONE;
            } else {
                live = cas_cut(iv[c], pa, pb, len, minl, &qa, &qb, &ql);
                if (!live) { c = NONE; c_child[i] = NONE; }
            }
            if (live) key = cas_key(qa, ql);
        }
        bool bid = live;
        if (live && ceil) { const u64 ce = ceil[c]; bid = ce == 0 || key < ce; }
        seg_atomic_max64(best, c, key, bid);
    } else {
        const u32 i = ((blockIdx.x - mblocks) * CAS_ITEMS + (u32)it) * TB + threadIdx.x;
        u32 c = i < NW ? w_child[i] : NONE;
        bool live = c != NONE;
        u32 v = 0;
        if (live) {
            const int64_t pos = (int64_t)w_pos[i];
            v = w_val[i];
            if (!first) {
                const CasRes r = res[c];
                const CasIv p = iv[c];
                u32 nc = NONE;
                if (r.state == 1u) {
                    const int64_t ea = (int64_t)r.qa + r.ql, eb = (int64_t)r.qb + r.ql;
                    const bool in_lead = (pos >= p.a0 && pos < r.qa) || (pos >= p.b0 && pos < r.qb);
                    const bool in_trail = (pos >= ea && pos < p.a1) || (pos >= eb && pos < p.b1);
                    nc = in_lead ? r.lead : in_trail ? r.trail : NONE;
                } else if (r.state == 3u) nc = r.lead;
                c = nc;
                w_child[i] = c;
                live = c != NONE;
            } else {
                const CasIv p = iv[c];
                live = (pos >= p.a0 && pos < p.a1) || (pos >= p.b0 && pos < p.b1);
                if (!live) { c = NONE; w_child[i] = NONE; }
            }
        }
        seg_atomic_max32(wmax, c, v, live);
    }
    }
}

__global__ __launch_bounds__(TB) void k_cas_winner(const sa_t *__restrict__ c_pa, const sa_t *__restrict__ c_pb, const u32 *__restrict__ c_len,
                                                   const u32 *__restrict__ c_child, u32 M, const CasIv *__restrict__ iv, CasRes *__restrict__ res,
                                                   const u64 *__restrict__ best, int64_t minl) {
    const u32 i = blockIdx.x * TB + threadIdx.x;
    if (i >= M) return;
    const u32 c = c_child[i];
    if (c == NONE) return;
    int64_t qa, qb, ql;
    if (!cas_cut(iv[c], (int64_t)c_pa[i], (int64_t)c_pb[i], (int64_t)c_len[i], minl, &qa, &qb, &ql)) return;
    if (cas_key(qa, ql) == best[c]) { res[c].qa = (sa_t)qa; res[c].qb = (sa_t)qb; res[c].ql = (u32)ql; }
}

constexpr u32 DWALK = 1024;
struct CasDanger { u64 *best; u32 *flag; sa_t *qb; u64 *ceil; u32 *m1, *p1, *m2; u64 *key; const uint8_t *T0; const lcp_t *LCP; const u64 *rank; u32 leaf_n; uint8_t *dflag; const uint8_t *wcls; };
__device__ inline bool cas_is_danger(const CasIv &p, u64 bk, u32 wm, u32 minl, u32 leaf_n, u32 *theta) {
    const int64_t la = (int64_t)p.a1 - p.a0, lb = (int64_t)p.b1 - p.b0;
    const u32 bl = (u32)(bk >> KEY_SHIFT);
    const bool can = (la >= (int64_t)minl) & (lb >= (int64_t)minl);
    const bool split = can & (bl >= minl) & (bl > wm);
    *theta = bl >= minl ? bl : minl;
    return can & !split & (wm >= minl) & ((u64)(la + lb) > (u64)leaf_n);
}
__global__ __launch_bounds__(TB) void k_cas_dmark(const CasIv *__restrict__ iv, const u64 *__restrict__ best, const u32 *__restrict__ wmax, u32 minl, const u32 *__restrict__ counters, CasDanger dg) {
    const u32 lo = counters[C_LO], hi = counters[C_HI];
    for (u32 id = lo + blockIdx.x * TB + threadIdx.x; id < hi; id += gridDim.x * TB) {
        u32 theta;
        dg.dflag[id] = cas_is_danger(iv[id], best[id], wmax[id], minl, dg.leaf_n, &theta) ? 1 : 0;
    }
}
__global__ __launch_bounds__(TB) void k_cas_dwalk(const sa_t *__restrict__ w_pos, const u32 *__restrict__ w_val, const u32 *__restrict__ w_child, u32 NW,
                                                  const CasIv *__restrict__ iv, const u64 *__restrict__ best, const u32 *__restrict__ wmax, u32 minl, CasDanger dg) {
    const u32 i = blockIdx.x * TB + threadIdx.x;
    if (i >= NW) return;
    if (dg.wcls && dg.wcls[i]) return;
    const u32 c = w_child[i];
    if (c == NONE || !dg.dflag[c]) return;
    dg.m1[i] = 0; dg.key[i] = 0;
    const CasIv p = iv[c];
    u32 theta;
    if (!cas_is_danger(p, best[c], wmax[c], minl, dg.leaf_n, &theta)) return;
    const int64_t pos = (int64_t)w_pos[i];
    const int64_t cap = (pos < (int64_t)p.a1 ? (int64_t)p.a1 : (int64_t)p.b1) - pos;
    if (w_val[i] < theta || cap < (int64_t)theta) return;
    u32 b1 = 0, b2 = 0, part = NONE;
    bool over = false;
#pragma unroll 1
    for (int dir = -1; dir <= 1; dir += 2) {
        u32 steps = 0;
        u64 rk = dg.rank[i];
        u32 run = 0xFFFFFFFFu;
        for (int64_t k = (int64_t)i + dir; k >= 0 && k < (int64_t)NW; k += dir) {
            const u64 r2 = dg.rank[k];
            if (r2 != rk + (u64)(int64_t)dir) break;
            const u32 g = (u32)dg.LCP[dir > 0 ? r2 : rk];
            run = g < run ? g : run;
            rk = r2;
            if (run < theta) break;
            if (++steps > DWALK) { over = true; break; }
            if (w_child[k] != c || w_val[k] < theta) continue;
            const int64_t pk = (int64_t)w_pos[k];
            const int64_t ck = (pk < (int64_t)p.a1 ? (int64_t)p.a1 : (int64_t)p.b1) - pk;
            if (ck < (int64_t)theta) continue;
            u32 l = (u32)(cap < ck ? cap : ck);
            l = run < l ? run : l;
            if (l > b1) { b2 = b1; b1 = l; part = (u32)k; }
            else if (l > b2) b2 = l;
            if (run <= b2) break;
        }
    }
    if (over) atomicOr(&dg.flag[c], 2u);
    dg.m1[i] = b1 >= theta ? b1 : 0u; dg.p1[i] = part; dg.m2[i] = b2;
}
constexpr u32 BLK_MIN = 64, BLK_MAX = 1024;
__global__ __launch_bounds__(TB) void k_cas_blk_flags(const u64 *__restrict__ rank, const lcp_t *__restrict__ LCP, u32 NW, u32 minl, u32 *__restrict__ flag) {
    const u32 i = blockIdx.x * TB + threadIdx.x;
    if (i >= NW) return;
    flag[i] = (i == 0 || rank[i] != rank[i - 1] + 1 || (u32)LCP[rank[i]] < minl) ? 1u : 0u;
}
__global__ __launch_bounds__(TB) void k_cas_blk_off(const u32 *__restrict__ flag, const u32 *__restrict__ bid, u32 NW, u32 nb, u32 *__restrict__ boff) {
    const u32 i = blockIdx.x * TB + threadIdx.x;
    if (i == 0) boff[nb] = NW;
    if (i < NW && flag[i]) boff[bid[i]] = i;
}
__global__ __launch_bounds__(TB) void k_cas_blk_class(const u32 *__restrict__ flag, const u32 *__restrict__ bid, const u32 *__restrict__ boff, u32 NW, u32 *__restrict__ mflag, uint8_t *__restrict__ wcls) {
    const u32 i = blockIdx.x * TB + threadIdx.x;
    if (i >= NW) return;
    const u32 b = bid[i] + flag[i] - 1u;
    const u32 size = boff[b + 1] - boff[b];
    const bool med = size > BLK_MIN && size <= BLK_MAX;
    wcls[i] = med ? 1 : 0;
    if (flag[i]) mflag[b] = med ? 1u : 0u;
}
__global__ __launch_bounds__(TB) void k_cas_blk_list(const u32 *__restrict__ mflag, const u32 *__restrict__ mid, u32 nb, u32 *__restrict__ mlist) {
    const u32 b = blockIdx.x * TB + threadIdx.x;
    if (b < nb && mflag[b]) mlist[mid[b]] = b;
}
__global__ __launch_bounds__(TB) void k_cas_dwalk_blk(const sa_t *__restrict__ w_pos, const u32 *__restrict__ w_val, const u32 *__restrict__ w_child, const u32 *__restrict__ boff,
                                                      const u32 *__restrict__ mlist, u32 nmed, const CasIv *__restrict__ iv, const u64 *__restrict__ best, const u32 *__restrict__ wmax,
                                                      u32 minl, CasDanger dg) {
    __shared__ u32 cc[BLK_MAX], vv[BLK_MAX], ll[BLK_MAX];
    __shared__ sa_t pp[BLK_MAX];
    __shared__ u32 s_any;
    const u32 b = mlist[blockIdx.x];
    const u32 s0 = boff[b], size = boff[b + 1] - s0;
    if (threadIdx.x == 0) s_any = 0;
    __syncthreads();
    bool any = false;
    for (u32 j = threadIdx.x; j < size; j += TB) {
        const u32 c = w_child[s0 + j];
        cc[j] = c;
        any |= c != NONE && dg.dflag[c];
    }
    if (__ballot(any) && (threadIdx.x & 63) == 0) s_any = 1;
    __syncthreads();
    if (!s_any) return;
    for (u32 j = threadIdx.x; j < size; j += TB) {
        vv[j] = w_val[s0 + j]; pp[j] = w_pos[s0 + j];
        ll[j] = (u32)dg.LCP[dg.rank[s0 + j]];
    }
    __syncthreads();
    for (u32 j = threadIdx.x; j < size; j += TB) {
        const u32 c = cc[j];
        if (c == NONE || !dg.dflag[c]) continue;
        const u32 i = s0 + j;
        dg.m1[i] = 0; dg.key[i] = 0;
        const CasIv p = iv[c];
        u32 theta;
        if (!cas_is_danger(p, best[c], wmax[c], minl, dg.leaf_n, &theta)) continue;
        const int64_t pos = (int64_t)pp[j];
        const int64_t cap = (pos < (int64_t)p.a1 ? (int64_t)p.a1 : (int64_t)p.b1) - pos;
        if (vv[j] < theta || cap < (int64_t)theta) continue;
        u32 b1 = 0, b2 = 0, part = NONE;
#pragma unroll 1
        for (int dir = -1; dir <= 1; dir += 2) {
            u32 run = 0xFFFFFFFFu;
            for (int64_t k = (int64_t)j + dir; k >= 0 && k < (int64_t)size; k += dir) {
                const u32 g = ll[dir > 0 ? k : k + 1];
                run = g < run ? g : run;
                if (run < theta) break;
                if (cc[k] != c || vv[k] < theta) continue;
                const int64_t pk = (int64_t)pp[k];
                const int64_t ck = (pk < (int64_t)p.a1 ? (int64_t)p.a1 : (int64_t)p.b1) - pk;
                if (ck < (int64_t)theta) continue;
                u32 l = (u32)(cap < ck ? cap : ck);
                l = run < l ? run : l;
                if (l > b1) { b2 = b1; b1 = l; part = s0 + (u32)k; }
                else if (l > b2) b2 = l;
                if (run <= b2) break;
            }
        }
        dg.m1[i] = b1 >= theta ? b1 : 0u; dg.p1[i] = part; dg.m2[i] = b2;
    }
}
__global__ __launch_bounds__(TB) void k_cas_dpick(const sa_t *__restrict__ w_pos, const u32 *__restrict__ w_val, const u32 *__restrict__ w_child, u32 NW,
                                                  const CasIv *__restrict__ iv, const CasRes *__restrict__ res, const u64 *__restrict__ best, const u32 *__restrict__ wmax,
                                                  u32 minl, CasDanger dg) {
    const u32 i = blockIdx.x * TB + threadIdx.x;
    if (i >= NW) return;
    const u32 c = w_child[i];
    if (c == NONE || !dg.dflag[c]) return;
    const CasIv p = iv[c];
    u32 theta;
    const u64 bk = best[c];
    if (!cas_is_danger(p, bk, wmax[c], minl, dg.leaf_n, &theta)) return;
    const int64_t pos = (int64_t)w_pos[i];
    const int64_t cap = (pos < (int64_t)p.a1 ? (int64_t)p.a1 : (int64_t)p.b1) - pos;
    if (w_val[i] < theta || cap < (int64_t)theta) return;
    if ((u32)(bk >> KEY_SHIFT) >= minl) { const CasRes r = res[c]; if (pos == (int64_t)r.qa || pos == (int64_t)r.qb) atomicOr(&dg.flag[c], 1u); }
    const u32 b1 = dg.m1[i];
    if (b1 == 0) return;
    const u32 w = dg.p1[i];
    if (dg.m1[w] != b1 || dg.p1[w] != i || b1 <= dg.m2[i] || b1 <= dg.m2[w]) return;
    const int64_t pw = (int64_t)w_pos[w];
    const bool a_side = pos < (int64_t)p.a1, w_a_side = pw < (int64_t)p.a1;
    if (!a_side || w_a_side) return;
    const int64_t qa = pos, qb = pw;
    if (!(qa == (int64_t)p.a0 || qb == (int64_t)p.b0)) {
        const uint8_t ca = dg.T0[qa - 1];
        if (ca == dg.T0[qb - 1] && ca != 'N' && ca != '$' && !(ca >= 'a' && ca <= 'z')) return;
    }
    const u64 key = cas_key(qa, (int64_t)b1);
    dg.key[i] = key;
    if (key > dg.best[c]) atomicMax((unsigned long long *)&dg.best[c], (unsigned long long)key);
}
__global__ __launch_bounds__(TB) void k_cas_dwrite(const sa_t *__restrict__ w_pos, const u32 *__restrict__ w_child, u32 NW, CasDanger dg) {
    const u32 i = blockIdx.x * TB + threadIdx.x;
    if (i >= NW) return;
    const u32 c = w_child[i];
    if (c == NONE || !dg.dflag[c]) return;
    const u64 key = dg.key[i];
    if (key == 0) return;
    if (key == dg.best[c]) dg.qb[c] = w_pos[dg.p1[i]];
}

__global__ __launch_bounds__(TB) void k_cas_decide(CasIv *__restrict__ iv, u64 *__restrict__ best, u32 *__restrict__ wmax, int32_t *__restrict__ depth,
                                                   CasRes *__restrict__ res, u32 minl, u32 *__restrict__ counters, u32 child_cap,
                                                   u32 *__restrict__ und_list, u32 leaf_n, RvCascadeIO io, CasDanger dg, int danger) {
    __shared__ u32 s_cnt[TB / 64][3];
    __shared__ u32 s_base[3];
    const u32 lo = counters[C_LO], hi = counters[C_HI];
    const int lane = threadIdx.x & 63, w = threadIdx.x >> 6;
    const u64 lt = (lane == 0) ? 0ull : (~0ull >> (64 - lane));
    for (u32 first = lo + blockIdx.x * TB; first < hi; first += gridDim.x * TB) {
        const u32 id = first + threadIdx.x;
        const bool in = id < hi;
        CasIv p; p.a0 = p.a1 = p.b0 = p.b1 = 0;
        u64 bk = 0; u32 wm = 0; int32_t dp = 0;
        CasRes r; r.qa = r.qb = 0; r.ql = 0; r.lead = r.trail = NONE; r.state = 2;
        if (in) { p = iv[id]; bk = best[id]; wm = wmax[id]; dp = depth[id]; r = res[id]; }
        const int64_t la = (int64_t)p.a1 - p.a0, lb = (int64_t)p.b1 - p.b0;
        const u32 bl = (u32)(bk >> KEY_SHIFT);
        const bool can = in & (la >= (int64_t)minl) & (lb >= (int64_t)minl);
        bool split = can & (bl >= minl) & (bl > wm);
        bool und = can & !split & (wm >= minl);
        bool forced = false, retry = false;
        if (danger && und && (u64)(la + lb) > (u64)dg.leaf_n) {
            const u32 fl = dg.flag[id];
            const u64 kh = dg.best[id], kc = (bl >= minl && !(fl & 1u)) ? bk : 0ull;
            if (!(fl & 2u)) {
                if (kh == 0 && kc == 0) {
                    if (bl < minl) und = false;
                    else if ((fl >> 8) < 16u) { retry = true; und = false; }
                } else {
                    if (kh > kc) { r.qa = (sa_t)(KEY_LOW - (kh & KEY_LOW)); r.qb = dg.qb[id]; r.ql = (u32)(kh >> KEY_SHIFT); }
                    split = true; forced = true; und = false;
                }
            }
            if (!retry) atomicAdd(&counters[und ? C_NUNSOLVED : C_NSOLVED], 1u);
        }
        bool lead = retry, trail = false;
        if (split) {
            if (!forced && r.ql != bl) atomicOr(&counters[C_ERR], 2u);
            lead = ((int64_t)r.qa - p.a0) + ((int64_t)r.qb - p.b0) > 0;
            trail = ((int64_t)p.a1 - r.qa - r.ql) + ((int64_t)p.b1 - r.qb - r.ql) > 0;
        }
        const u64 b_lead = __ballot(lead), b_trail = __ballot(trail), b_split = __ballot(split), b_und = __ballot(und);
        if (retry) atomicAdd(&counters[C_NRETRY], 1u);
        if (lane == 0) { s_cnt[w][0] = (u32)__popcll(b_lead) + (u32)__popcll(b_trail); s_cnt[w][1] = (u32)__popcll(b_split); s_cnt[w][2] = (u32)__popcll(b_und); }
        __syncthreads();
        if (threadIdx.x < 3) {
            u32 tot = 0;
            for (int k = 0; k < TB / 64; k++) tot += s_cnt[k][threadIdx.x];
            u32 *ctr = threadIdx.x == 0 ? &counters[C_NCHILD] : threadIdx.x == 1 ? io.anchor_count : &counters[C_NUND];
            s_base[threadIdx.x] = tot ? atomicAdd(ctr, tot) : 0u;
        }
        __syncthreads();
        u32 base_c = s_base[0], base_a = s_base[1], base_u = s_base[2];
        for (int k = 0; k < w; k++) { base_c += s_cnt[k][0]; base_a += s_cnt[k][1]; base_u += s_cnt[k][2]; }
        if (retry) {
            const u32 slot = base_c + (u32)__popcll(b_lead & lt) + (u32)__popcll(b_trail & lt);
            CasRes nr; nr.qa = 0; nr.qb = 0; nr.ql = 0; nr.lead = NONE; nr.trail = NONE; nr.state = 0;
            if (slot < child_cap) {
                iv[slot] = p; best[slot] = 0; wmax[slot] = 0; depth[slot] = dp; res[slot] = nr;
                dg.best[slot] = 0; dg.flag[slot] = ((dg.flag[id] >> 8) + 1u) << 8; dg.ceil[slot] = bk;
                r.lead = slot; r.trail = NONE;
            } else atomicOr(&counters[C_ERR], 1u);
            r.state = 3;
        } else if (split) {
            u32 slot = base_c + (u32)__popcll(b_lead & lt) + (u32)__popcll(b_trail & lt);
            CasRes nr; nr.qa = 0; nr.qb = 0; nr.ql = 0; nr.lead = NONE; nr.trail = NONE; nr.state = 0;
            if (lead) {
                if (slot < child_cap) {
                    CasIv c; c.a0 = p.a0; c.a1 = r.qa; c.b0 = p.b0; c.b1 = r.qb;
                    iv[slot] = c; best[slot] = 0; wmax[slot] = 0; depth[slot] = dp + 1; res[slot] = nr;
                    if (danger) { dg.best[slot] = 0; dg.flag[slot] = 0; dg.ceil[slot] = 0; }
                    r.lead = slot;
                } else atomicOr(&counters[C_ERR], 1u);
                slot++;
            }
            if (trail) {
                if (slot < child_cap) {
                    CasIv c; c.a0 = (sa_t)((int64_t)r.qa + r.ql); c.a1 = p.a1; c.b0 = (sa_t)((int64_t)r.qb + r.ql); c.b1 = p.b1;
                    iv[slot] = c; best[slot] = 0; wmax[slot] = 0; depth[slot] = dp + 1; res[slot] = nr;
                    if (danger) { dg.best[slot] = 0; dg.flag[slot] = 0; dg.ceil[slot] = 0; }
                    r.trail = slot;
                } else atomicOr(&counters[C_ERR], 1u);
            }
            const u32 as = base_a + (u32)__popcll(b_split & lt);
            if (as < io.anchor_cap) { io.anchor_l[as] = r.ql; io.anchor_pos[2 * (size_t)as] = (int64_t)r.qa; io.anchor_pos[2 * (size_t)as + 1] = (int64_t)r.qb; }
            else atomicOr(&counters[C_ERR], 4u);
            r.state = 1;
        } else {
            r.state = 2;
        }
        if (in) res[id] = r;
        if (und) {
            und_list[base_u + (u32)__popcll(b_und & lt)] = id;
            if ((u64)(la + lb) > (u64)leaf_n) atomicMax(&counters[C_MAXN], (u32)((la + lb) > 0xFFFFFFFFll ? 0xFFFFFFFFll : (la + lb)));
        }
        __syncthreads();
    }
    if (threadIdx.x == 0) {
        __threadfence();
        if (atomicAdd(&counters[C_TICKET], 1u) == gridDim.x - 1) {
            if (hi > lo) counters[C_LEVELS]++;
            const u32 made = atomicAdd(&counters[C_NCHILD], 0u);
            counters[C_LO] = hi; counters[C_HI] = made < child_cap ? made : child_cap;
            counters[C_NANCH] = atomicAdd(io.anchor_count, 0u);
            counters[C_TICKET] = 0;
        }
    }
}
__global__ __launch_bounds__(TB) void k_cas_stats(const u32 *__restrict__ counters, const int32_t *__restrict__ depth, RvCascadeIO io) {
    __shared__ unsigned long long s_bp[TB / 64];
    __shared__ u32 s_md[TB / 64];
    const u32 nchild = counters[C_NCHILD], na = *io.anchor_count;
    unsigned long long bp = 0; u32 md = 0;
    for (u32 i = blockIdx.x * TB + threadIdx.x; i < na; i += gridDim.x * TB) bp += io.anchor_l[i];
    for (u32 i = blockIdx.x * TB + threadIdx.x; i < nchild; i += gridDim.x * TB) { const u32 d = (u32)depth[i]; md = d > md ? d : md; }
#pragma unroll
    for (int d = 32; d >= 1; d >>= 1) {
        bp += ((unsigned long long)(u32)__shfl_down((u32)(bp >> 32), d, 64) << 32) + (unsigned long long)(u32)__shfl_down((u32)bp, d, 64);
        const u32 om = __shfl_down(md, d, 64);
        md = om > md ? om : md;
    }
    if ((threadIdx.x & 63) == 0) { s_bp[threadIdx.x >> 6] = bp; s_md[threadIdx.x >> 6] = md; }
    __syncthreads();
    if (threadIdx.x == 0) {
        for (int k = 1; k < TB / 64; k++) { bp += s_bp[k]; md = s_md[k] > md ? s_md[k] : md; }
        if (bp) atomicAdd(&io.stats[2], bp);
        if (md) atomicMax(&io.stats[3], (unsigned long long)md);
        if (blockIdx.x == 0) { atomicAdd(&io.stats[0], (unsigned long long)(nchild - counters[C_NUND] - counters[C_NRETRY])); atomicAdd(&io.stats[1], (unsigned long long)na); }
    }
}

__global__ __launch_bounds__(TB) void k_cas_sizes(const u32 *__restrict__ und_list, u32 U, const CasIv *__restrict__ iv, u64 *__restrict__ sizes) {
    const u32 u = blockIdx.x * TB + threadIdx.x;
    if (u < U) { const CasIv p = iv[und_list[u]]; sizes[u] = (u64)(((int64_t)p.a1 - p.a0) + ((int64_t)p.b1 - p.b0)); }
    if (u == U) sizes[u] = 0;
}
__global__ __launch_bounds__(TB) void k_cas_roots(const u32 *__restrict__ und_list, u32 U, const CasIv *__restrict__ iv, const int32_t *__restrict__ depth,
                                                  const u64 *__restrict__ offs, RvLeafRoot *__restrict__ roots) {
    const u32 u = blockIdx.x * TB + threadIdx.x;
    if (u >= U) return;
    const u32 id = und_list[u];
    const CasIv p = iv[id];
    RvLeafRoot r;
    r.off = (int64_t)offs[u]; r.n = (int32_t)(((int64_t)p.a1 - p.a0) + ((int64_t)p.b1 - p.b0)); r.depth = depth[id];
    r.a0 = p.a0; r.a1 = p.a1; r.b0 = p.b0; r.b1 = p.b1;
    roots[u] = r;
}

constexpr int BN = RV_LEAF_N;
__device__ inline int cas_first_diff(const uint8_t *txt, int i, int j, int lim) {
    int x = 0;
    while (x + 8 <= lim) {
        u64 a, b;
        __builtin_memcpy(&a, txt + i + x, 8);
        __builtin_memcpy(&b, txt + j + x, 8);
        if (a != b) return x + (__builtin_ctzll(a ^ b) >> 3);
        x += 8;
    }
    while (x < lim && txt[i + x] == txt[j + x]) x++;
    return x;
}
__global__ __launch_bounds__(TB) void k_cas_rank(const RvLeafRoot *__restrict__ roots, const uint8_t *__restrict__ T0, uint16_t *__restrict__ ord) {
    __shared__ __attribute__((aligned(8))) uint8_t txt[BN + 24];
    const RvLeafRoot root = roots[blockIdx.x];
    const int la = (int)(root.a1 - root.a0), lb = (int)(root.b1 - root.b0), n = la + lb;
    if ((int)blockIdx.y * TB >= n) return;
    for (int k = threadIdx.x; k < n; k += TB) txt[k] = k < la ? T0[root.a0 + k] : T0[root.b0 + (k - la)];
    __syncthreads();
    const int i = (int)blockIdx.y * TB + threadIdx.x;
    if (i >= n) return;
    const int ri = (i < la ? la : n) - i;
    int cnt = 0;
    u64 ki = 0, wj = 0;
#pragma unroll
    for (int b = 0; b < 8; b++) { ki |= (u64)txt[i + b] << (8 * b); wj |= (u64)txt[b] << (8 * b); }
    for (int j0 = 0; j0 < n; j0 += 8) {
        u64 nxt = *reinterpret_cast<const u64 *>(txt + j0 + 8);
#pragma unroll
        for (int e = 0; e < 8; e++) {
            const int j = j0 + e;
            if (j < n) {
                const int rj = (j < la ? la : n) - j;
                const int lim = ri < rj ? ri : rj;
                const u64 d = ki ^ wj;
                int k = d ? (__builtin_ctzll(d) >> 3) : 8;
                bool j_less;
                if (k < 8 && k < lim) j_less = (u32)((wj >> (8 * k)) & 0xffu) < (u32)((ki >> (8 * k)) & 0xffu);
                else {
                    if (k >= 8 && lim > 8 && j != i) k = 8 + cas_first_diff(txt, i + 8, j + 8, lim - 8);
                    else if (j == i) k = lim;
                    j_less = (k < lim) ? (txt[j + k] < txt[i + k]) : ((rj < ri) | ((rj == ri) & (j < i)));
                }
                cnt += j_less ? 1 : 0;
            }
            wj = (wj >> 8) | (nxt << 56);
            nxt >>= 8;
        }
    }
    ord[root.off + cnt] = (uint16_t)i;
}
__global__ __launch_bounds__(TB) void k_cas_emit(const RvLeafRoot *__restrict__ roots, const uint8_t *__restrict__ T0, const uint16_t *__restrict__ ord, sa_t *__restrict__ SA,
                                                 lcp_t *__restrict__ LCP, uint8_t *__restrict__ BWT, int64_t nsep0, int64_t root_a0, int64_t root_b0,
                                                 const sa_t *__restrict__ beginA, u32 nA, const sa_t *__restrict__ beginB, u32 nB) {
    __shared__ uint8_t txt[BN + 8];
    const RvLeafRoot root = roots[blockIdx.x];
    const int la = (int)(root.a1 - root.a0), lb = (int)(root.b1 - root.b0), n = la + lb;
    if ((int)blockIdx.y * TB >= n) return;
    for (int k = threadIdx.x; k < n; k += TB) txt[k] = k < la ? T0[root.a0 + k] : T0[root.b0 + (k - la)];
    __syncthreads();
    const int r = (int)blockIdx.y * TB + threadIdx.x;
    if (r >= n) return;
    const int i = ord[root.off + r];
    const int ri = (i < la ? la : n) - i;
    u32 l = 0;
    if (r > 0) {
        const int j = ord[root.off + r - 1];
        const int rj = (j < la ? la : n) - j;
        const int lim = ri < rj ? ri : rj;
        int k = 0;
        while (k < lim) { const uint8_t c = txt[i + k]; if (c != txt[j + k] || c == '$' || c == 'N') break; k++; }
        l = (u32)k;
    }
    const int64_t gp = i < la ? root.a0 + i : root.b0 + (i - la);
    uint8_t ch = gp > 0 ? T0[gp - 1] : (uint8_t)'$';
    bool at_seq_start;
    if (beginA) {
        const int c = i < la ? cas_contig_of(beginA, nA, (int64_t)root.a0) : cas_contig_of(beginB, nB, (int64_t)root.b0);
        at_seq_start = i < la ? (c >= 0 && (int64_t)beginA[c] == (int64_t)root.a0) : (c >= 0 && (int64_t)beginB[c] == (int64_t)root.b0);
    } else at_seq_start = i < la ? !(root.a0 > root_a0) : !(root.b0 > root_b0);
    const bool behind_anchor = (i < la ? i == 0 : i == la) && !at_seq_start;
    if (behind_anchor && ch >= 'A' && ch <= 'Z') ch += 32;
    const int64_t o = root.off + r;
    SA[o] = (sa_t)gp; LCP[o] = (lcp_t)l; BWT[o] = (uint8_t)(ch | (gp > nsep0 ? RV_BWT_SIDE : 0u));
}

int bitlen64(u64 x) { int b = 0; while (x) { b++; x >>= 1; } return b; }
double cas_now() { return std::chrono::duration<double>(std::chrono::steady_clock::now().time_since_epoch()).count(); }

}

static int cas_lineage(rv_index *h, RvCascadeBufs &cb, u32 M, u32 NW, u32 minl, const std::vector<RvIntv> &CA, const std::vector<RvIntv> &CB, const char **why) {
    Workspace &ws = h->ws;
    hipStream_t q = ws.stream;
    *why = nullptr;
    DBuf &k0 = cb.d[0], &k1 = cb.d[1], &v0 = cb.d[2], &v1 = cb.d[3], &bpa = cb.d[4], &bpb = cb.d[5], &blen = cb.d[6], &bwp = cb.d[8], &bwv = cb.d[9];
    DBuf &spa = cb.d[27], &spb = cb.d[28], &slen = cb.d[29], &broots = cb.d[30], &bdepth = cb.d[31], &btabs = cb.d[32], &banch = cb.d[33];
    RV_TRY(spa.reserve((size_t)M * sizeof(sa_t))); RV_TRY(spb.reserve((size_t)M * sizeof(sa_t))); RV_TRY(slen.reserve((size_t)M * 4));
    const unsigned mb = (unsigned)ceil_div((int64_t)M, TB);
    hipLaunchKernelGGL(k_cas_lkeys, dim3(mb), dim3(TB), 0, q, (const sa_t *)bpa.as<sa_t>(), (const u32 *)blen.as<u32>(), M, k0.as<u64>(), v0.as<u32>());
    RV_LAUNCH_CHECK();
    int in1 = 0;
    RV_TRY(rv_radix_sort_pairs<u32>(ws, k0.as<u64>(), v0.as<u32>(), k1.as<u64>(), v1.as<u32>(), (int64_t)M, 0, 64, &in1));
    hipLaunchKernelGGL(k_cas_lgather, dim3(mb), dim3(TB), 0, q, (const sa_t *)bpa.as<sa_t>(), (const sa_t *)bpb.as<sa_t>(), (const u32 *)blen.as<u32>(),
                       (const u32 *)(in1 ? v1.as<u32>() : v0.as<u32>()), M, spa.as<sa_t>(), spb.as<sa_t>(), slen.as<u32>());
    RV_LAUNCH_CHECK();
    std::vector<sa_t> ha(M), hb(M), hwp(NW);
    std::vector<u32> hl(M), hwv(NW);
    RV_HIP(hipMemcpyAsync(ha.data(), spa.p, (size_t)M * sizeof(sa_t), hipMemcpyDeviceToHost, q));
    RV_HIP(hipMemcpyAsync(hb.data(), spb.p, (size_t)M * sizeof(sa_t), hipMemcpyDeviceToHost, q));
    RV_HIP(hipMemcpyAsync(hl.data(), slen.p, (size_t)M * 4, hipMemcpyDeviceToHost, q));
    if (NW) {
        RV_HIP(hipMemcpyAsync(hwp.data(), bwp.p, (size_t)NW * sizeof(sa_t), hipMemcpyDeviceToHost, q));
        RV_HIP(hipMemcpyAsync(hwv.data(), bwv.p, (size_t)NW * 4, hipMemcpyDeviceToHost, q));
    }
    RV_HIP(hipStreamSynchronize(q));
    const size_t nA = CA.size(), nB = CB.size();
    auto contig = [](const std::vector<RvIntv> &C, int64_t pos) -> int {
        size_t lo = 0, hi = C.size();
        while (lo < hi) { const size_t mid = (lo + hi) / 2; if (C[mid].begin <= pos) lo = mid + 1; else hi = mid; }
        return (int)lo - 1;
    };
    std::vector<u32> wA(nA, 0), wB(nB, 0);
    const int64_t firstB = CB[0].begin;
    for (u32 i = 0; i < NW; i++) {
        const int64_t pos = (int64_t)hwp[i];
        if (pos < firstB) { const int c = contig(CA, pos); if (c >= 0 && pos < CA[(size_t)c].end) wA[(size_t)c] = std::max(wA[(size_t)c], hwv[i]); }
        else { const int c = contig(CB, pos); if (c >= 0 && pos < CB[(size_t)c].end) wB[(size_t)c] = std::max(wB[(size_t)c], hwv[i]); }
    }
    struct Ent { u32 w; int side; u32 c; };
    std::vector<Ent> byw;
    for (size_t c = 0; c < nA; c++) byw.push_back({wA[c], 0, (u32)c});
    for (size_t c = 0; c < nB; c++) byw.push_back({wB[c], 1, (u32)c});
    std::sort(byw.begin(), byw.end(), [](const Ent &x, const Ent &y) { return x.w > y.w; });
    std::vector<uint8_t> liveA(nA, 1), liveB(nB, 1);
    size_t wptr = 0, nLiveA = nA, nLiveB = nB;
    auto chain_wmax = [&]() -> u32 {
        while (wptr < byw.size() && !(byw[wptr].side ? liveB[byw[wptr].c] : liveA[byw[wptr].c])) wptr++;
        return wptr < byw.size() ? byw[wptr].w : 0u;
    };
    std::vector<CasIv> roots; std::vector<int32_t> rdepth;
    bool stalled = false;
    std::vector<int32_t> pickA(nA, -1), pickB(nB, -1);
    std::vector<u32> rootLead, rootTrail, anl; std::vector<int64_t> anp;
    int32_t depth = 0;
    for (u32 i = 0; i < M && nLiveA && nLiveB; i++) {
        const u32 l = hl[i];
        if (l < minl) break;
        const int64_t a = (int64_t)ha[i], b = (int64_t)hb[i];
        const int ca = contig(CA, a), cb2 = contig(CB, b);
        if (ca < 0 || cb2 < 0 || !liveA[(size_t)ca] || !liveB[(size_t)cb2]) continue;
        if (a + (int64_t)l > CA[(size_t)ca].end || b + (int64_t)l > CB[(size_t)cb2].end) { *why = "a match that leaves its sequence"; return 0; }
        if (l <= chain_wmax()) { stalled = true; break; }
        const u32 k = (u32)anl.size();
        if (ws.opt.cascade_log) fprintf(stderr, "cascade: chain member %u chooses %u at %lld / %lld (sequences %d / %d), bound %u\n", k, l, (long long)a, (long long)b, ca, cb2, chain_wmax());
        anl.push_back(l); anp.push_back(a); anp.push_back(b);
        pickA[(size_t)ca] = (int32_t)k; pickB[(size_t)cb2] = (int32_t)k;
        u32 rl = NONE, rt = NONE;
        if ((a - CA[(size_t)ca].begin) + (b - CB[(size_t)cb2].begin) > 0) {
            CasIv c; c.a0 = (sa_t)CA[(size_t)ca].begin; c.a1 = (sa_t)a; c.b0 = (sa_t)CB[(size_t)cb2].begin; c.b1 = (sa_t)b;
            rl = (u32)roots.size(); roots.push_back(c); rdepth.push_back(depth + 1);
        }
        if ((CA[(size_t)ca].end - a - (int64_t)l) + (CB[(size_t)cb2].end - b - (int64_t)l) > 0) {
            CasIv c; c.a0 = (sa_t)(a + (int64_t)l); c.a1 = (sa_t)CA[(size_t)ca].end; c.b0 = (sa_t)(b + (int64_t)l); c.b1 = (sa_t)CB[(size_t)cb2].end;
            rt = (u32)roots.size(); roots.push_back(c); rdepth.push_back(depth + 1);
        }
        rootLead.push_back(rl); rootTrail.push_back(rt);
        liveA[(size_t)ca] = 0; liveB[(size_t)cb2] = 0; nLiveA--; nLiveB--;
        depth++;
    }
    if (anl.empty()) { *why = stalled ? "a repeat as long as the best match of the root" : "no match between two sequences at the top level"; return 0; }
    int64_t steps = (int64_t)anl.size();
    int maxdepth = depth - 1;
    cb.lin_rest.clear(); cb.lin_rest_depth = depth;
    if (ws.opt.cascade_log) fprintf(stderr, "cascade: chain of %zu choices, %zu + %zu sequences left, stalled %d, bound %u\n", anl.size(), nLiveA, nLiveB, (int)stalled, chain_wmax());
    if (nLiveA + nLiveB > 0) {
        if (stalled || (nLiveA && nLiveB && chain_wmax() >= minl)) {
            for (size_t c = 0; c < nA; c++) if (liveA[c]) { cb.lin_rest.push_back(CA[c].begin); cb.lin_rest.push_back(CA[c].end); }
            for (size_t c = 0; c < nB; c++) if (liveB[c]) { cb.lin_rest.push_back(CB[c].begin); cb.lin_rest.push_back(CB[c].end); }
        } else { steps++; maxdepth = depth; }
    }
    const u32 R = (u32)roots.size(), P = (u32)anl.size();
    RV_TRY(broots.reserve((size_t)std::max<u32>(R, 1) * sizeof(CasIv))); RV_TRY(bdepth.reserve((size_t)std::max<u32>(R, 1) * 4));
    const size_t tab_bytes = (nA + nB) * (sizeof(sa_t) + 4) + (size_t)P * 8 + 64;
    RV_TRY(btabs.reserve(tab_bytes + 64)); RV_TRY(banch.reserve((size_t)P * (4 + 16) + 64));
    std::vector<uint8_t> stage(tab_bytes + 64, 0);
    size_t o = 0;
    auto put = [&](const void *src, size_t bytes) { memcpy(stage.data() + o, src, bytes); const size_t at = o; o += (bytes + 15) / 16 * 16; return at; };
    std::vector<sa_t> bA(nA), bB(nB);
    for (size_t c = 0; c < nA; c++) bA[c] = (sa_t)CA[c].begin;
    for (size_t c = 0; c < nB; c++) bB[c] = (sa_t)CB[c].begin;
    stage.resize((nA + nB) * (sizeof(sa_t) + 4) + (size_t)P * 8 + 16 * 8 + 64);
    const size_t oA = put(bA.data(), nA * sizeof(sa_t)), oB = put(bB.data(), nB * sizeof(sa_t)), opA = put(pickA.data(), nA * 4), opB = put(pickB.data(), nB * 4),
                 oL = put(rootLead.data(), (size_t)P * 4), oT = put(rootTrail.data(), (size_t)P * 4);
    RV_TRY(btabs.reserve(o + 64));
    RV_HIP(hipMemcpyAsync(btabs.p, stage.data(), o, hipMemcpyHostToDevice, q));
    if (R) {
        RV_HIP(hipMemcpyAsync(broots.p, roots.data(), (size_t)R * sizeof(CasIv), hipMemcpyHostToDevice, q));
        RV_HIP(hipMemcpyAsync(bdepth.p, rdepth.data(), (size_t)R * 4, hipMemcpyHostToDevice, q));
    }
    RV_HIP(hipMemcpyAsync(banch.p, anp.data(), (size_t)P * 16, hipMemcpyHostToDevice, q));
    RV_HIP(hipMemcpyAsync((uint8_t *)banch.p + (size_t)P * 16, anl.data(), (size_t)P * 4, hipMemcpyHostToDevice, q));
    RV_HIP(hipStreamSynchronize(q));
    cb.lin_roots = R; cb.lin_picks = P; cb.lin_nA = (u32)nA; cb.lin_nB = (u32)nB; cb.lin_steps = steps; cb.lin_maxdepth = maxdepth;
    cb.lin_off[0] = oA; cb.lin_off[1] = oB; cb.lin_off[2] = opA; cb.lin_off[3] = opB; cb.lin_off[4] = oL; cb.lin_off[5] = oT;
    return 0;
}

int rv_cascade_run(rv_index *h, RvCascadeBufs &cb, const RvCascadeIO &io, int minl_in, RvCascadeOut *out, int danger, int reuse, const RvCascadeHost *host) {
    memset(out, 0, sizeof *out);
    out->done = false;
    Workspace &ws = h->ws;
    hipStream_t q = ws.stream;
    const int64_t n = h->n;
    const u32 minl = (u32)std::max(minl_in, 1);
    const bool verbose = (ws.opt.cascade_log != 0);
    double tp[6] = {0, 0, 0, 0, 0, 0};
    if (verbose) { (void)hipStreamSynchronize(q); tp[0] = cas_now(); }
#define GIVE_UP(msg) do { out->why = msg; if (verbose) fprintf(stderr, "cascade: gave up: %s\n", msg); return 0; } while (0)
    if (h->nsamples != 2 || h->nsep.size() != 1 || h->nodes.size() < 2) GIVE_UP("not two samples");
    std::vector<RvIntv> CA, CB;
    for (const RvIntv &v : h->nodes) if (v.end > v.begin) (v.begin < h->nsep[0] ? CA : CB).push_back(v);
    std::sort(CA.begin(), CA.end(), [](const RvIntv &x, const RvIntv &y) { return x.begin < y.begin; });
    std::sort(CB.begin(), CB.end(), [](const RvIntv &x, const RvIntv &y) { return x.begin < y.begin; });
    if (CA.empty() || CB.empty()) GIVE_UP("an empty sample");
    const bool chain = CA.size() > 1 || CB.size() > 1;
    if (chain && ws.opt.no_cascade_chain) GIVE_UP("several sequences per sample (switched off)");
    if (n >= ((int64_t)1 << 32) - 2) GIVE_UP("index above 2^32 positions");
#ifdef RV_SA64
    if ((u64)h->maxlcp >= (1ull << 24) || n >= ((int64_t)1 << 40)) GIVE_UP("bid word too narrow");
#endif
    CasIv root; root.a0 = root.a1 = root.b0 = root.b1 = 0;
    root.a0 = (sa_t)CA[0].begin; root.a1 = (sa_t)CA[0].end; root.b0 = (sa_t)CB[0].begin; root.b1 = (sa_t)CB[0].end;
    if (root.a0 >= root.a1 || root.b0 >= root.b1 || (int64_t)root.a1 > h->nsep[0] || (int64_t)root.b0 <= h->nsep[0]) GIVE_UP("an empty sample");

    const sa_t *SA = h->dSA.as<sa_t>(); const lcp_t *LCP = h->dLCP.as<lcp_t>(); const uint8_t *BWT = h->dBWT.as<uint8_t>();

    const int64_t ntile = ceil_div(n, RV_PAIR_TILE);
    DBuf &bcnt = ws.misc[14], &btab = ws.misc[2], &bslot = ws.misc[3], &bovf = ws.misc[4], &bout = ws.misc[5];
    if (bcnt.cap == 0) { RV_TRY(bcnt.reserve(64)); RV_HIP(hipMemsetAsync(bcnt.p, 0, 64, q)); }
    RV_TRY(btab.reserve((size_t)(ntile + 1) * 3 * sizeof(u32)));
    RV_TRY(bslot.reserve((size_t)ntile * RV_PAIR_SLOTS * sizeof(RvPairRec)));
    if (bovf.cap < 4096 * sizeof(RvPairRec)) RV_TRY(bovf.reserve(4096 * sizeof(RvPairRec)));
    if (bout.cap < 4096 * sizeof(RvPairRec)) RV_TRY(bout.reserve(sizeof(RvPairRec) * (size_t)std::max<int64_t>(4096, n / 64)));
    u32 *tilecnt = btab.as<u32>(), *tileovf = tilecnt + (ntile + 1), *tileoff = tileovf + (ntile + 1);
    const bool wit_pass = ws.opt.cas_witness_pass != 0;
    const int64_t wtile = wit_pass ? WT_TILE : RV_PAIR_WG_TILE;
    const int64_t rcap64 = std::min<int64_t>(n / WT_REGIONS + wtile, std::max<int64_t>(16384, n / 1024));
    const u32 wcap = (u32)std::min<int64_t>(rcap64 * WT_REGIONS, 0x7fffffff);
    const u32 wrcap = ws.cap_first(RV_CS_CAS_WIT, wcap / WT_REGIONS);
    DBuf &bwp0 = cb.d[19], &bwv0 = cb.d[20], &bwr = cb.d[21], &bwrk = cb.d[22], &bwrk0 = cb.d[23];
    u32 hreg[2 * WT_REGIONS];
    RV_TRY(bwp0.reserve((size_t)wcap * sizeof(sa_t))); RV_TRY(bwv0.reserve((size_t)wcap * 4)); RV_TRY(bwr.reserve(2 * WT_REGIONS * 4 + 64));
    RV_TRY(bwrk.reserve((size_t)wcap * 4)); RV_TRY(bwrk0.reserve((size_t)wcap * 4));
    const RvScanWit swit = {bwp0.as<sa_t>(), bwv0.as<u32>(), bwrk0.as<u32>(), wrcap, bwr.as<u32>()};
    u32 M = reuse ? cb.M : 0;
    for (int attempt = 0; !reuse; attempt++) {
        if (attempt == 3) { rv_set_error("cascade: scan buffer sizing failed"); return -1; }
        const size_t ocap = bout.cap / sizeof(RvPairRec) - RV_PAIR_HDR, vcap = bovf.cap / sizeof(RvPairRec);
        if (!wit_pass) RV_HIP(hipMemsetAsync(bwr.p, 0, 2 * WT_REGIONS * 4, q));
        hipEvent_t ev_a, ev_b;
        (void)h->prof.attach(RV_K_SCAN_PAIR, (double)n * 8.0, &ev_a, &ev_b);
        RV_TRY(rv_scan_pair_launch(ws, SA, LCP, n, BWT, (sa_t)h->nsep[0], (int)minl, bslot.as<RvPairRec>(), bovf.as<RvPairRec>(),
                                   (u32)std::min<size_t>(vcap, 0xffffffffu), bcnt.as<u32>(), tilecnt, tileovf, nullptr, nullptr, 0, ev_a, ev_b, wit_pass ? nullptr : &swit));
        RV_TRY(rv_exclusive_sum_u32(ws, tilecnt, tileoff, ntile + 1));
        RV_TRY(rv_pair_compact_launch(ws, bslot.as<RvPairRec>(), bovf.as<RvPairRec>(), tilecnt, tileovf, tileoff, ntile, bout.as<RvPairRec>(),
                                      (u32)std::min<size_t>(ocap, 0xffffffffu), bcnt.as<u32>(), nullptr, (u32)std::min<size_t>(vcap, 0xffffffffu)));
        u32 hdr[4];
        if (wit_pass) RV_TRY(rv_read_back(ws, hdr, bout.p, sizeof hdr));
        else RV_TRY(rv_read_back2(ws, hdr, bout.p, sizeof hdr, hreg, bwr.p, WT_REGIONS * 4));
        const u32 total = hdr[0], novf = hdr[1];
        if (total <= ocap && novf <= vcap) { M = total; break; }
        if (novf > vcap) { ws.cap_events[RV_CE_PAIR_OVF]++; RV_TRY(bovf.reserve((size_t)novf * sizeof(RvPairRec))); }
        if (total > ocap) { ws.cap_events[RV_CE_PAIR_OUT]++; RV_TRY(bout.reserve(((size_t)total + RV_PAIR_HDR) * sizeof(RvPairRec))); }
    }
    if (verbose) tp[1] = cas_now();
    out->cands = M;
    struct ProfSpan { Workspace &w; int id; ~ProfSpan() { w.prof_end(id); } } span{ws, ws.prof_begin(RV_K_CASCADE, (wit_pass ? 5.0 * (double)n : 0.0) + 16.0 * (double)M)};
    if (M == 0) GIVE_UP("no match at the top level");
    const RvPairRec *recs = bout.as<RvPairRec>() + RV_PAIR_HDR;
    cb.M = M;

    const int64_t ccap64 = n / (int64_t)minl + 16;
    if (ccap64 >= 0x7fffffff) GIVE_UP("too many sub-indices possible");
    const u32 ccap = (u32)ccap64;
    const u32 ccap_k = ws.cap_first(RV_CS_CAS_TABLES, ccap, 32u);
    RvCascadeIO iok = io;
    iok.anchor_cap = ws.cap_first(RV_CS_CAS_TABLES, io.anchor_cap);
    DBuf &k0 = cb.d[0], &k1 = cb.d[1], &v0 = cb.d[2], &v1 = cb.d[3], &bpa = cb.d[4], &bpb = cb.d[5], &blen = cb.d[6], &bcc = cb.d[7], &bwp = cb.d[8], &bwv = cb.d[9],
         &bwc = cb.d[10], &biv = cb.d[11], &bbest = cb.d[12], &bwm = cb.d[13], &bdep = cb.d[14], &bres = cb.d[15], &bctr = cb.d[16], &bund = cb.d[17], &bsz = cb.d[18];
    RV_TRY(k0.reserve((size_t)M * 8)); RV_TRY(k1.reserve((size_t)M * 8)); RV_TRY(v0.reserve((size_t)M * 4)); RV_TRY(v1.reserve((size_t)M * 4));
    RV_TRY(bpa.reserve((size_t)M * sizeof(sa_t))); RV_TRY(bpb.reserve((size_t)M * sizeof(sa_t))); RV_TRY(blen.reserve((size_t)M * 4)); RV_TRY(bcc.reserve((size_t)M * 4));
    RV_TRY(bwp.reserve((size_t)wcap * sizeof(sa_t))); RV_TRY(bwv.reserve((size_t)wcap * 4)); RV_TRY(bwc.reserve((size_t)wcap * 4));
    RV_TRY(biv.reserve((size_t)ccap * sizeof(CasIv))); RV_TRY(bbest.reserve((size_t)ccap * 8)); RV_TRY(bwm.reserve((size_t)ccap * 4)); RV_TRY(bdep.reserve((size_t)ccap * 4));
    RV_TRY(bres.reserve((size_t)ccap * sizeof(CasRes))); RV_TRY(bctr.reserve(64)); RV_TRY(bund.reserve((size_t)ccap * 4));
    u32 *counters = bctr.as<u32>();
    RV_HIP(hipMemsetAsync(counters, 0, 64, q));

    u32 hc[16];
    u32 NW = reuse ? cb.NW : 0;
    if (!reuse) {
        u32 *wreg = bwr.as<u32>();
        u32 wmaxc = 0;
        auto pack = [&]() -> int {
            for (int r = 0; r < WT_REGIONS; r++) { hreg[WT_REGIONS + r] = NW; NW += hreg[r]; wmaxc = std::max(wmaxc, hreg[r]); }
            out->witnesses = NW;
            if (wmaxc > wrcap || NW == 0) return 0;
            RV_HIP(hipMemcpyAsync(wreg + WT_REGIONS, hreg + WT_REGIONS, WT_REGIONS * 4, hipMemcpyHostToDevice, q));
            RV_HIP(hipStreamSynchronize(q));
            hipLaunchKernelGGL(k_cas_wpack, dim3((unsigned)std::max<int64_t>(1, ceil_div((int64_t)wmaxc, TB)), WT_REGIONS), dim3(TB), 0, q, (const sa_t *)bwp0.as<sa_t>(),
                               (const u32 *)bwv0.as<u32>(), (const u32 *)bwrk0.as<u32>(), wrcap, (const u32 *)wreg, (const u32 *)(wreg + WT_REGIONS), bwp.as<sa_t>(), bwv.as<u32>(),
                               bwrk.as<u32>());
            RV_LAUNCH_CHECK();
            return 0;
        };
        if (wit_pass) {
            RV_HIP(hipMemsetAsync(wreg, 0, 2 * WT_REGIONS * 4, q));
            hipLaunchKernelGGL(k_cas_witness, dim3((unsigned)ceil_div(n, WT_TILE)), dim3(TB), 0, q, SA, LCP, BWT, n, minl, bwp0.as<sa_t>(), bwv0.as<u32>(), bwrk0.as<u32>(), wrcap, wreg);
            RV_LAUNCH_CHECK();
        } else {
            RV_TRY(pack());
            if (wmaxc > wrcap) GIVE_UP("too many repeat witnesses (a repetitive input)");
        }
        {
            const unsigned mb = (unsigned)ceil_div((int64_t)M, TB);
            hipLaunchKernelGGL(k_cas_keys, dim3(mb), dim3(TB), 0, q, recs, M, k0.as<u64>(), v0.as<u32>());
            RV_LAUNCH_CHECK();
            int in1 = 0;
            RV_TRY(rv_radix_sort_pairs<u32>(ws, k0.as<u64>(), v0.as<u32>(), k1.as<u64>(), v1.as<u32>(), (int64_t)M, 0, bitlen64((u64)n), &in1));
            hipLaunchKernelGGL(k_cas_gather, dim3(mb), dim3(TB), 0, q, recs, (const u32 *)(in1 ? v1.as<u32>() : v0.as<u32>()), M, bpa.as<sa_t>(), bpb.as<sa_t>(),
                               blen.as<u32>(), bcc.as<u32>());
            RV_LAUNCH_CHECK();
        }
        if (wit_pass) {
            RV_TRY(rv_read_back(ws, hreg, wreg, WT_REGIONS * 4));
            RV_TRY(pack());
            if (wmaxc > wrcap) GIVE_UP("too many repeat witnesses (a repetitive input)");
        }
        cb.NW = NW;
        if (chain) {
            const char *why = nullptr;
            RV_TRY(cas_lineage(h, cb, M, NW, minl, CA, CB, &why));
            if (why) { cb.lin_picks = 0; cb.lin_rest.clear(); GIVE_UP(why); }
        }
    } else {
        if (chain && cb.lin_picks == 0) GIVE_UP("the chain of rest sub-indices was not decided");
        RV_HIP(hipMemsetAsync(bcc.p, 0, (size_t)M * 4, q));
        out->witnesses = NW;
    }
    const sa_t *wp = bwp.as<sa_t>(); const u32 *wv = bwv.as<u32>();
    CasDanger dg; memset(&dg, 0, sizeof dg);
    u32 dwalk_nmed = 0; const u32 *dwalk_boff = nullptr, *dwalk_mlist = nullptr;
    if (danger) {
        if (NW) {
            RV_TRY(k0.reserve((size_t)NW * 8)); RV_TRY(k1.reserve((size_t)NW * 8)); RV_TRY(v0.reserve((size_t)NW * 4)); RV_TRY(v1.reserve((size_t)NW * 4));
            const unsigned wb = (unsigned)ceil_div((int64_t)NW, TB);
            hipLaunchKernelGGL(k_cas_wkeys, dim3(wb), dim3(TB), 0, q, (const u32 *)bwrk.as<u32>(), NW, k0.as<u64>(), v0.as<u32>());
            RV_LAUNCH_CHECK();
            int in1 = 0;
            RV_TRY(rv_radix_sort_pairs<u32>(ws, k0.as<u64>(), v0.as<u32>(), k1.as<u64>(), v1.as<u32>(), (int64_t)NW, 0, bitlen64((u64)n), &in1));
            hipLaunchKernelGGL(k_cas_wgather, dim3(wb), dim3(TB), 0, q, (const sa_t *)bwp.as<sa_t>(), (const u32 *)bwv.as<u32>(), (const u32 *)(in1 ? v1.as<u32>() : v0.as<u32>()), NW,
                               bwp0.as<sa_t>(), bwv0.as<u32>());
            RV_LAUNCH_CHECK();
            wp = bwp0.as<sa_t>(); wv = bwv0.as<u32>();
            dg.rank = in1 ? k1.as<u64>() : k0.as<u64>();
        }
        DBuf &bdc = cb.d[24], &bdw = cb.d[25];
        const size_t per_child = 8 + 8 + 4 + sizeof(sa_t) + 1, per_wit = 4 + 4 + 4 + 8;
        RV_TRY(bdc.reserve((size_t)ccap * per_child + 64)); RV_TRY(bdw.reserve((size_t)std::max<u32>(NW, 1) * per_wit + 64));
        dg.best = bdc.as<u64>(); dg.ceil = dg.best + ccap; dg.qb = (sa_t *)(dg.ceil + ccap); dg.flag = (u32 *)(dg.qb + ccap); dg.dflag = (uint8_t *)(dg.flag + ccap);
        dg.key = bdw.as<u64>(); dg.m1 = (u32 *)(dg.key + std::max<u32>(NW, 1)); dg.p1 = dg.m1 + std::max<u32>(NW, 1); dg.m2 = dg.p1 + std::max<u32>(NW, 1);
        dg.T0 = h->dT0.as<uint8_t>(); dg.LCP = LCP;
        if (NW && !ws.opt.no_dwalk_blocks) {
            DBuf &bfl = cb.d[35], &bbid = cb.d[36], &bboff = cb.d[37], &bml = cb.d[38], &bwcls = cb.d[39];
            RV_TRY(bfl.reserve((size_t)(NW + 1) * 4)); RV_TRY(bbid.reserve((size_t)(NW + 1) * 4)); RV_TRY(bwcls.reserve((size_t)NW + 16));
            const unsigned wb = (unsigned)ceil_div((int64_t)NW, TB);
            hipLaunchKernelGGL(k_cas_blk_flags, dim3(wb), dim3(TB), 0, q, dg.rank, LCP, NW, minl, bfl.as<u32>());
            RV_LAUNCH_CHECK();
            RV_HIP(hipMemsetAsync(bfl.as<u32>() + NW, 0, 4, q));
            RV_TRY(rv_exclusive_sum_u32(ws, bfl.as<u32>(), bbid.as<u32>(), (int64_t)NW + 1));
            u32 nb = 0;
            RV_TRY(rv_read_back(ws, &nb, bbid.as<u32>() + NW, 4));
            RV_TRY(bboff.reserve((size_t)(nb + 2) * 4)); RV_TRY(bml.reserve((size_t)(nb + 2) * 4 * 3));
            u32 *mflag = bml.as<u32>(), *mid = mflag + (nb + 1), *mlist = mid + (nb + 1);
            hipLaunchKernelGGL(k_cas_blk_off, dim3(wb), dim3(TB), 0, q, (const u32 *)bfl.as<u32>(), (const u32 *)bbid.as<u32>(), NW, nb, bboff.as<u32>());
            RV_LAUNCH_CHECK();
            hipLaunchKernelGGL(k_cas_blk_class, dim3(wb), dim3(TB), 0, q, (const u32 *)bfl.as<u32>(), (const u32 *)bbid.as<u32>(), (const u32 *)bboff.as<u32>(), NW, mflag, bwcls.as<uint8_t>());
            RV_LAUNCH_CHECK();
            RV_HIP(hipMemsetAsync(mflag + nb, 0, 4, q));
            RV_TRY(rv_exclusive_sum_u32(ws, mflag, mid, (int64_t)nb + 1));
            RV_TRY(rv_read_back(ws, &dwalk_nmed, mid + nb, 4));
            if (dwalk_nmed) {
                hipLaunchKernelGGL(k_cas_blk_list, dim3((unsigned)ceil_div((int64_t)nb, TB)), dim3(TB), 0, q, (const u32 *)mflag, (const u32 *)mid, nb, mlist);
                RV_LAUNCH_CHECK();
                dg.wcls = bwcls.as<uint8_t>();
                dwalk_boff = bboff.as<u32>(); dwalk_mlist = mlist;
            }
        }
        dg.leaf_n = (u32)ws.opt.cascade_danger_min;
    }
    const sa_t *d_beginA = nullptr, *d_beginB = nullptr;
    if (!chain) {
        hipLaunchKernelGGL(k_cas_init, dim3((unsigned)std::max<int64_t>(1, ceil_div((int64_t)NW, TB))), dim3(TB), 0, q, biv.as<CasIv>(), bbest.as<u64>(), bwm.as<u32>(),
                           bdep.as<int32_t>(), bres.as<CasRes>(), counters, root, bwc.as<u32>(), NW, dg.best, dg.flag, dg.ceil);
        RV_LAUNCH_CHECK();
    } else {
        const u32 R = cb.lin_roots, P = cb.lin_picks;
        if ((int64_t)R + 16 > (int64_t)ccap_k || P > iok.anchor_cap) GIVE_UP("more sequences than the cascade's tables hold");
        const uint8_t *tb = cb.d[32].as<uint8_t>();
        CasRootTabs rt;
        rt.beginA = (const sa_t *)(tb + cb.lin_off[0]); rt.beginB = (const sa_t *)(tb + cb.lin_off[1]);
        rt.pickA = (const int32_t *)(tb + cb.lin_off[2]); rt.pickB = (const int32_t *)(tb + cb.lin_off[3]);
        rt.rootLead = (const u32 *)(tb + cb.lin_off[4]); rt.rootTrail = (const u32 *)(tb + cb.lin_off[5]);
        rt.nA = cb.lin_nA; rt.nB = cb.lin_nB;
        d_beginA = rt.beginA; d_beginB = rt.beginB;
        hipLaunchKernelGGL(k_cas_init_roots, dim3((unsigned)std::max<int64_t>(1, ceil_div((int64_t)R, TB))), dim3(TB), 0, q, biv.as<CasIv>(), bbest.as<u64>(), bwm.as<u32>(),
                           bdep.as<int32_t>(), bres.as<CasRes>(), counters, (const CasIv *)cb.d[30].as<CasIv>(), (const int32_t *)cb.d[31].as<int32_t>(), R, dg.best, dg.flag, dg.ceil);
        RV_LAUNCH_CHECK();
        hipLaunchKernelGGL(k_cas_assign_roots, dim3((unsigned)std::max<int64_t>(1, ceil_div((int64_t)std::max(M, NW), TB))), dim3(TB), 0, q, (const sa_t *)bpa.as<sa_t>(),
                           (const sa_t *)bpb.as<sa_t>(), (const u32 *)blen.as<u32>(), bcc.as<u32>(), M, wp, bwc.as<u32>(), NW, (const CasIv *)cb.d[30].as<CasIv>(), rt, (int64_t)minl);
        RV_LAUNCH_CHECK();
        RV_HIP(hipMemcpyAsync(io.anchor_pos, cb.d[33].p, (size_t)P * 16, hipMemcpyDeviceToDevice, q));
        RV_HIP(hipMemcpyAsync(io.anchor_l, (const uint8_t *)cb.d[33].p + (size_t)P * 16, (size_t)P * 4, hipMemcpyDeviceToDevice, q));
        RV_HIP(hipMemcpyAsync(io.anchor_count, &cb.lin_picks, 4, hipMemcpyHostToDevice, q));
    }

    if (verbose) { (void)hipStreamSynchronize(q); tp[2] = cas_now(); }
    const unsigned agrid = (unsigned)(ceil_div((int64_t)M, TB * CAS_ITEMS) + ceil_div((int64_t)NW, TB * CAS_ITEMS));
    const int batch = std::max(1, (int)ws.opt.cascade_batch);
    int queued = 0;
    RV_TRY(rv_working_text_begin(h, host ? host->side : nullptr));
    u32 sent = 0, known = 0;
    auto send_known = [&]() -> int {
        if (!host || !host->side || !host->l || known <= sent || known > host->cap) return 0;
        RV_HIP(hipMemcpyAsync(host->pos + 2 * (size_t)sent, io.anchor_pos + 2 * (size_t)sent, (size_t)(known - sent) * 16, hipMemcpyDeviceToHost, host->side));
        RV_HIP(hipMemcpyAsync(host->l + sent, io.anchor_l + sent, (size_t)(known - sent) * 4, hipMemcpyDeviceToHost, host->side));
        sent = known;
        return 0;
    };
    struct PrioScope {
        Workspace &w; hipStream_t home; RvCascadeBufs &cb; bool on = false;
        ~PrioScope() { leave(); }
        void leave() {
            if (!on) return;
            on = false;
            (void)hipEventRecord(cb.ev_out, w.stream);
            w.stream = home;
            (void)hipStreamWaitEvent(home, cb.ev_out, 0);
        }
    } prio{ws, q, cb};
    if (ws.opt.cascade_prio) {
        if (!cb.prio_stream) {
            int plo = 0, phi = 0;
            RV_HIP(hipDeviceGetStreamPriorityRange(&plo, &phi));
            RV_HIP(hipStreamCreateWithPriority(&cb.prio_stream, hipStreamNonBlocking, phi));
            RV_HIP(hipEventCreateWithFlags(&cb.ev_in, hipEventDisableTiming));
            RV_HIP(hipEventCreateWithFlags(&cb.ev_out, hipEventDisableTiming));
        }
        RV_HIP(hipEventRecord(cb.ev_in, q));
        RV_HIP(hipStreamWaitEvent(cb.prio_stream, cb.ev_in, 0));
        ws.stream = cb.prio_stream; prio.on = true;
        q = cb.prio_stream;
    }
    for (;;) {
        for (int b = 0; b < batch; b++, queued++) {
            hipLaunchKernelGGL(k_cas_assign, dim3(agrid), dim3(TB), 0, q, (const sa_t *)bpa.as<sa_t>(), (const sa_t *)bpb.as<sa_t>(), (const u32 *)blen.as<u32>(), bcc.as<u32>(), M,
                               wp, wv, bwc.as<u32>(), NW, (const CasIv *)biv.as<CasIv>(), (const CasRes *)bres.as<CasRes>(),
                               bbest.as<u64>(), bwm.as<u32>(), (int64_t)minl, queued == 0 ? 1 : 0, (const u64 *)((danger && NW) ? dg.ceil : nullptr));
            RV_LAUNCH_CHECK();
            hipLaunchKernelGGL(k_cas_winner, dim3((unsigned)ceil_div((int64_t)M, TB)), dim3(TB), 0, q, (const sa_t *)bpa.as<sa_t>(), (const sa_t *)bpb.as<sa_t>(),
                               (const u32 *)blen.as<u32>(), (const u32 *)bcc.as<u32>(), M, (const CasIv *)biv.as<CasIv>(), bres.as<CasRes>(), (const u64 *)bbest.as<u64>(), (int64_t)minl);
            RV_LAUNCH_CHECK();
            if (danger && NW) {
                const unsigned wb = (unsigned)ceil_div((int64_t)NW, TB);
                hipLaunchKernelGGL(k_cas_dmark, dim3(256), dim3(TB), 0, q, (const CasIv *)biv.as<CasIv>(), (const u64 *)bbest.as<u64>(), (const u32 *)bwm.as<u32>(), minl, (const u32 *)counters, dg);
                RV_LAUNCH_CHECK();
                hipLaunchKernelGGL(k_cas_dwalk, dim3(wb), dim3(TB), 0, q, wp, wv, (const u32 *)bwc.as<u32>(), NW, (const CasIv *)biv.as<CasIv>(), (const u64 *)bbest.as<u64>(),
                                   (const u32 *)bwm.as<u32>(), minl, dg);
                RV_LAUNCH_CHECK();
                if (dwalk_nmed) {
                    hipLaunchKernelGGL(k_cas_dwalk_blk, dim3((unsigned)dwalk_nmed), dim3(TB), 0, q, wp, wv, (const u32 *)bwc.as<u32>(), dwalk_boff, dwalk_mlist, dwalk_nmed,
                                       (const CasIv *)biv.as<CasIv>(), (const u64 *)bbest.as<u64>(), (const u32 *)bwm.as<u32>(), minl, dg);
                    RV_LAUNCH_CHECK();
                }
                hipLaunchKernelGGL(k_cas_dpick, dim3(wb), dim3(TB), 0, q, wp, wv, (const u32 *)bwc.as<u32>(), NW, (const CasIv *)biv.as<CasIv>(), (const CasRes *)bres.as<CasRes>(),
                                   (const u64 *)bbest.as<u64>(), (const u32 *)bwm.as<u32>(), minl, dg);
                RV_LAUNCH_CHECK();
                hipLaunchKernelGGL(k_cas_dwrite, dim3(wb), dim3(TB), 0, q, wp, (const u32 *)bwc.as<u32>(), NW, dg);
                RV_LAUNCH_CHECK();
            }
            hipLaunchKernelGGL(k_cas_decide, dim3(256), dim3(TB), 0, q, biv.as<CasIv>(), bbest.as<u64>(), bwm.as<u32>(), bdep.as<int32_t>(),
                               bres.as<CasRes>(), minl, counters, ccap_k, bund.as<u32>(), (u32)RV_LEAF_N, iok, dg, (danger && NW) ? 1 : 0);
            RV_LAUNCH_CHECK();
        }
        RV_TRY(send_known());
        RV_TRY(rv_read_back(ws, hc, counters, sizeof hc));
        if (hc[C_ERR] & ~5u) { rv_set_error("cascade: device error %u", hc[C_ERR]); return -1; }
        if (hc[C_ERR]) GIVE_UP("the cascade's tables are full");
        known = hc[C_NANCH];
        if (hc[C_MAXN] > (u32)RV_LEAF_N) break;
        if (hc[C_HI] == hc[C_LO]) break;
        if (queued > 1000000) { rv_set_error("cascade: no progress"); return -1; }
    }
    prio.leave(); q = ws.stream;
    const int level = (int)hc[C_LEVELS];
    const u32 hi = hc[C_NCHILD];
    if (verbose) tp[3] = cas_now();
    out->levels = level; out->children = hi; out->solved = hc[C_NSOLVED]; out->unsolved = hc[C_NUNSOLVED];
    const u32 U = hc[C_NUND];
    out->undecided = U;
    if (hc[C_MAXN] > (u32)RV_LEAF_N) {
        out->why = "an undecided sub-index above the leaf kernel's size";
        if (verbose) fprintf(stderr, "cascade%s: gave up: %s (%u ranks; %u levels, %u sub-indices, %u undecided, %u decided from witnesses, %u not)\n", danger ? " (second attempt)" : "", out->why, hc[C_MAXN], level, hi, U, hc[C_NSOLVED], hc[C_NUNSOLVED]);
        return 0;
    }
    hipLaunchKernelGGL(k_cas_stats, dim3(256), dim3(TB), 0, q, (const u32 *)counters, (const int32_t *)bdep.as<int32_t>(), io);
    RV_LAUNCH_CHECK();
    RV_TRY(send_known());
    if (chain) {
        hipLaunchKernelGGL(k_cas_lineage_stats, dim3(1), dim3(64), 0, q, io.stats, (unsigned long long)cb.lin_steps, (unsigned long long)cb.lin_maxdepth);
        RV_LAUNCH_CHECK();
    }
    if (U > 0) {
        RV_TRY(bsz.reserve((size_t)(U + 1) * 8));
        u64 *sizes = bsz.as<u64>();
        hipLaunchKernelGGL(k_cas_sizes, dim3((unsigned)ceil_div((int64_t)U + 1, TB)), dim3(TB), 0, q, (const u32 *)bund.as<u32>(), U, (const CasIv *)biv.as<CasIv>(), sizes);
        RV_LAUNCH_CHECK();
        RV_TRY(rv_exclusive_sum_u64(ws, sizes, sizes, (int64_t)U + 1));
        u64 mu = 0;
        RV_TRY(rv_read_back(ws, &mu, sizes + U, 8));
        out->rebuilt_ranks = (int64_t)mu;
        RV_TRY(io.lvSA->reserve((size_t)(mu + 64) * sizeof(sa_t))); RV_TRY(io.lvLCP->reserve((size_t)(mu + 64) * sizeof(lcp_t))); RV_TRY(io.lvBWT->reserve((size_t)mu + 64));
        RV_TRY(io.roots->reserve((size_t)U * sizeof(RvLeafRoot)));
        RvLeafRoot *roots = io.roots->as<RvLeafRoot>();
        hipLaunchKernelGGL(k_cas_roots, dim3((unsigned)ceil_div((int64_t)U, TB)), dim3(TB), 0, q, (const u32 *)bund.as<u32>(), U, (const CasIv *)biv.as<CasIv>(),
                           (const int32_t *)bdep.as<int32_t>(), (const u64 *)sizes, roots);
        RV_LAUNCH_CHECK();
        DBuf &bord = cb.d[26];
        RV_TRY(bord.reserve((size_t)(mu + 64) * 2));
        hipLaunchKernelGGL(k_cas_rank, dim3(U, BN / TB), dim3(TB), 0, q, (const RvLeafRoot *)roots, (const uint8_t *)h->dT0.as<uint8_t>(), bord.as<uint16_t>());
        RV_LAUNCH_CHECK();
        hipLaunchKernelGGL(k_cas_emit, dim3(U, BN / TB), dim3(TB), 0, q, (const RvLeafRoot *)roots, (const uint8_t *)h->dT0.as<uint8_t>(), (const uint16_t *)bord.as<uint16_t>(),
                           io.lvSA->as<sa_t>(), io.lvLCP->as<lcp_t>(), io.lvBWT->as<uint8_t>(), h->nsep[0], (int64_t)root.a0, (int64_t)root.b0,
                           d_beginA, cb.lin_nA, d_beginB, cb.lin_nB);
        RV_LAUNCH_CHECK();
        RvLeafArgs la;
        la.roots = roots;
        la.SA = io.lvSA->as<sa_t>(); la.LCP = io.lvLCP->as<lcp_t>(); la.BWT = io.lvBWT->as<uint8_t>();
        la.nsep0 = h->nsep[0]; la.minl = minl_in; la.lcap = h->maxlcp;
        la.stage_cap = io.stage_cap;
        la.anchor_count = io.anchor_count; la.anchor_cap = io.anchor_cap; la.anchor_l = io.anchor_l; la.anchor_pos = io.anchor_pos;
        la.stats = io.stats;
        la.trace = 0; la.trace_count = io.anchor_count + 1; la.trace_cap = 0; la.trace_out = nullptr;
        la.err = io.leaf_err;
        RV_TRY(rv_leaf_launch(ws, la, (int)U));
    }
    if (verbose) {
        (void)hipStreamSynchronize(q); tp[4] = cas_now();
        fprintf(stderr, "cascade%s: %u matches, %u witnesses, %d levels, %u sub-indices, %u undecided (%lld ranks rebuilt), %lld decided from witnesses | ms: scan %.2f witnesses+sort %.2f levels %.2f rebuild+leaf %.2f\n",
                danger ? " (second attempt)" : "", M, NW, level, hi, U, (long long)out->rebuilt_ranks, (long long)out->solved, (tp[1] - tp[0]) * 1e3, (tp[2] - tp[1]) * 1e3, (tp[3] - tp[2]) * 1e3, (tp[4] - tp[3]) * 1e3);
    }
    out->done = true;
    out->sent = sent;
    return 0;
#undef GIVE_UP
}
```

### reveal_amd/csrc/rv_common.h

```cpp
#pragma once
#include <algorithm>
#include <mutex>
#include <thread>
#include <vector>
#include <utility>
#include <hip/hip_runtime.h>
#include <stdint.h>
#include <string.h>
#include <stddef.h>
#include <vector>
#include <string>

#ifdef RV_SA64
typedef int64_t  sa_t;
typedef uint32_t lcp_t;
#else
typedef int32_t  sa_t;
typedef int32_t  lcp_t;
#endif

typedef unsigned long long u64;
typedef unsigned int       u32;

void rv_set_error(const char *fmt, ...);

#define RV_HIP(x)                                                                              \
    do {                                                                                       \
        hipError_t e_ = (x);                                                                   \
        if (e_ != hipSuccess) {                                                                \
            rv_set_error("%s:%d %s: %s", __FILE__, __LINE__, #x, hipGetErrorString(e_));       \
            return -1;                                                                         \
        }                                                                                      \
    } while (0)
#define RV_TRY(x)                                                                              \
    do {                                                                                       \
        int r_ = (x);                                                                          \
        if (r_ != 0) return r_;                                                                \
    } while (0)
#define RV_OPTION_LIST(X) \
    X(bubble_par_min, "RV_BUBBLE_PAR_MIN", -1) \
    X(presel_log, "RV_PRESEL_LOG", 0) \
    X(presel_host, "RV_PRESEL_HOST", 0) \
    X(leaf_acap, "RV_LEAF_ACAP", 256) \
    X(bubble_lds_always, "RV_BUBBLE_LDS_ALWAYS", 0) \
    X(no_early_bubble, "RV_NO_EARLY_BUBBLE", 0) \
    X(early_bubble_many, "RV_EARLY_BUBBLE_MANY", 0) \
    X(no_early_split, "RV_NO_EARLY_SPLIT", 0) \
    X(keep_dead, "RV_KEEP_DEAD", 0) \
    X(bubble_no_lds, "RV_BUBBLE_NO_LDS", 0) \
    X(bubble_no_join, "RV_BUBBLE_NO_JOIN", 0) \
    X(bubble_no_merge, "RV_BUBBLE_NO_MERGE", 0) \
    X(tables_memcpy, "RV_TABLES_MEMCPY", 0) \
    X(bubble_parent_scratch, "RV_BUBBLE_PARENT_SCRATCH", 0) \
    X(level_log, "RV_LEVEL_LOG", 0) \
    X(pb_two_pass, "RV_PB_TWO_PASS", 0) \
    X(no_leaf, "RV_NO_LEAF", 0) \
    X(leaf_prof, "RV_LEAF_PROF", 0) \
    X(no_cascade, "RV_NO_CASCADE", 0) \
    X(cascade_second, "RV_CASCADE_SECOND", 0) \
    X(cascade_danger, "RV_CASCADE_DANGER", 1) \
    X(cascade_second_off, "RV_CASCADE_SECOND_OFF", 0) \
    X(sync_block, "RV_SYNC_BLOCK", 0) \
    X(pb_refresh_tmin, "RV_PB_REFRESH_TMIN", 0) \
    X(cascade_log, "RV_CASCADE_LOG", 0) \
    X(cascade_danger_min, "RV_CASCADE_DANGER_MIN", 0) \
    X(cascade_batch, "RV_CASCADE_BATCH", 8) \
    X(lcp_by_rank, "RV_LCP_BY_RANK", 0) \
    X(no_tiny_sa, "RV_NO_TINY_SA", 0) \
    X(no_short_alphabet, "RV_NO_SHORT_ALPHABET", 0) \
    X(no_fused_lcp, "RV_NO_FUSED_LCP", 0) \
    X(no_diag, "RV_NO_DIAG", 0) \
    X(no_packed_text, "RV_NO_PACKED_TEXT", 0) \
    X(no_heads_fusion, "RV_NO_HEADS_FUSION", 0) \
    X(no_twin_collapse, "RV_NO_TWIN_COLLAPSE", 0) \
    X(no_far_twins, "RV_NO_FAR_TWINS", 0) \
    X(no_lcp_list, "RV_NO_LCP_LIST", 0) \
    X(no_text_jump, "RV_NO_TEXT_JUMP", 0) \
    X(far_table, "RV_FAR_TABLE", 0) \
    X(no_slow_class, "RV_NO_SLOW_CLASS", 0) \
    X(no_dwalk_blocks, "RV_NO_DWALK_BLOCKS", 0) \
    X(no_pub_twins, "RV_NO_PUB_TWINS", 0) \
    X(sa_no_text, "RV_SA_NO_TEXT", 0) \
    X(text_mode, "RV_TEXT_MODE", -1) \
    X(carry_ch, "RV_CARRY_CH", -1) \
    X(rs_bits, "RV_RS_BITS", 8) \
    X(rs_xcd, "RV_RS_XCD", 1) \
    X(rs_cnt16, "RV_RS_CNT16", 1) \
    X(rs_no_digit_bytes, "RV_RS_NO_DIGIT_BYTES", 0) \
    X(diag_table, "RV_DIAG_TABLE", -1) \
    X(no_cascade_chain, "RV_NO_CASCADE_CHAIN", 0) \
    X(casm_rank_count, "RV_CASM_RANK_COUNT", 0) \
    X(casm_big_min, "RV_CASM_BIG_MIN", -1) \
    X(casm_no_big, "RV_CASM_NO_BIG", 0) \
    X(casm_big_root, "RV_CASM_BIG_ROOT", 1 << 22) \
    X(casm_big_total, "RV_CASM_BIG_TOTAL", 1 << 26) \
    X(lock_any, "RV_LOCK_ANY", 0) \
    X(presel_dev_min, "RV_PRESEL_DEV_MIN", 65536) \
    X(scan_v1, "RV_SCAN_V1", 0) \
    X(pick_threads, "RV_PICK_THREADS", 0) \
    X(cascade_prio, "RV_CASCADE_PRIO", 0) \
    X(cas_witness_pass, "RV_CAS_WITNESS_PASS", 0) \
    X(cap_limit, "RV_CAP_LIMIT", 0) \
    X(cap_sites, "RV_CAP_SITES", -1) \
    X(many_chain_multi, "RV_MANY_CHAIN_MULTI", 0)
struct RvOptions {
#define RV_X_(f, name, def) int64_t f = def;
    RV_OPTION_LIST(RV_X_)
#undef RV_X_
    int64_t *find(const char *name) {
#define RV_X_(f, nm, def) if (strcmp(name, nm) == 0) return &f;
        RV_OPTION_LIST(RV_X_)
#undef RV_X_
        return nullptr;
    }
};
extern int g_rv_launch_trace;
static inline bool rv_launch_trace_on() { return g_rv_launch_trace != 0; }
#define RV_LAUNCH_CHECK()                                                                      \
    do {                                                                                       \
        RV_HIP(hipGetLastError());                                                             \
        if (rv_launch_trace_on()) {                                                            \
            fprintf(stderr, "launch %s:%d\n", __FILE__, __LINE__);                             \
            fflush(stderr);                                                                    \
            RV_HIP(hipDeviceSynchronize());                                                    \
        }                                                                                      \
    } while (0)

static inline int64_t ceil_div(int64_t a, int64_t b) { return (a + b - 1) / b; }

#define RV_BWT_SIDE 0x80u
#define RV_BWT_CHAR 0x7fu

#ifdef __HIPCC__
__device__ inline u32 rv_wave_min_u32(u32 v) {
    const int inf = -1;
    int x = (int)v, y;
#define RV_DPP_MIN(ctrl, rmask)                                                        \
    y = __builtin_amdgcn_update_dpp(inf, x, ctrl, rmask, 0xf, false);                  \
    x = (int)(((u32)y < (u32)x) ? (u32)y : (u32)x);
    RV_DPP_MIN(0xB1, 0xf)
    RV_DPP_MIN(0x4E, 0xf)
    RV_DPP_MIN(0x141, 0xf)
    RV_DPP_MIN(0x140, 0xf)
    RV_DPP_MIN(0x142, 0xa)
    RV_DPP_MIN(0x143, 0xc)
#undef RV_DPP_MIN
    return (u32)__builtin_amdgcn_readlane(x, 63);
}
#endif

#ifdef __HIPCC__
template <int CTRL, int ROWMASK> __device__ inline u32 rv_dpp_u32(u32 x) { return (u32)__builtin_amdgcn_update_dpp(0, (int)x, CTRL, ROWMASK, 0xf, false); }
#define RV_WAVE_SCAN_STEPS(STEP)                                                     \
    STEP(0x111, 0xf, (lane & 15) >= 1)                                               \
    STEP(0x112, 0xf, (lane & 15) >= 2)                                               \
    STEP(0x114, 0xf, (lane & 15) >= 4)                                               \
    STEP(0x118, 0xf, (lane & 15) >= 8)                                               \
    STEP(0x142, 0xa, (lane & 31) >= 16)                                              \
    STEP(0x143, 0xc, lane >= 32)
__device__ inline u64 rv_wave_max_u64(u64 v) {
#define RV_STEP_(CTRL, RM, TAKE) { const u64 t = ((u64)rv_dpp_u32<CTRL, RM>((u32)(v >> 32)) << 32) | rv_dpp_u32<CTRL, RM>((u32)v); v = t > v ? t : v; }
    RV_WAVE_SCAN_STEPS(RV_STEP_)
#undef RV_STEP_
    return ((u64)(u32)__builtin_amdgcn_readlane((int)(u32)(v >> 32), 63) << 32) | (u32)__builtin_amdgcn_readlane((int)(u32)v, 63);
}
__device__ inline u64 rv_wave_seg_max_u64(u32 seg, u64 v) {
    const int lane = threadIdx.x & 63;
    u32 lo = (u32)v, hi = (u32)(v >> 32);
#define RV_STEP_(CTRL, RM, TAKE) { const u32 os = rv_dpp_u32<CTRL, RM>(seg), ol = rv_dpp_u32<CTRL, RM>(lo), oh = rv_dpp_u32<CTRL, RM>(hi); \
                                   const bool up = (TAKE) && os == seg && (oh > hi || (oh == hi && ol > lo)); lo = up ? ol : lo; hi = up ? oh : hi; }
    RV_WAVE_SCAN_STEPS(RV_STEP_)
#undef RV_STEP_
    return ((u64)hi << 32) | lo;
}
__device__ inline u32 rv_wave_seg_max_u32(u32 seg, u32 v) {
    const int lane = threadIdx.x & 63;
#define RV_STEP_(CTRL, RM, TAKE) { const u32 os = rv_dpp_u32<CTRL, RM>(seg), ov = rv_dpp_u32<CTRL, RM>(v); v = ((TAKE) && os == seg && ov > v) ? ov : v; }
    RV_WAVE_SCAN_STEPS(RV_STEP_)
#undef RV_STEP_
    return v;
}
__device__ inline u32 rv_wave_incl_sum_u32(u32 v) {
    const int lane = threadIdx.x & 63;
#define RV_STEP_(CTRL, RM, TAKE) { const u32 t = rv_dpp_u32<CTRL, RM>(v); v += (TAKE) ? t : 0u; }
    RV_WAVE_SCAN_STEPS(RV_STEP_)
#undef RV_STEP_
    return v;
}
#endif

bool rv_oom_trim();

inline hipError_t rv_event_wait(hipEvent_t ev) {
    hipError_t e;
    for (int spins = 0; (e = hipEventQuery(ev)) == hipErrorNotReady; spins++) {
        if (spins < 64) { __builtin_ia32_pause(); continue; }
        if (spins < 640) { std::this_thread::yield(); continue; }
        return hipEventSynchronize(ev);
    }
    return e;
}

struct DBuf {
    void  *p = nullptr;
    size_t cap = 0;
    int reserve(size_t bytes) {
        if (bytes <= cap) return 0;
        if (p) { (void)hipFree(p); p = nullptr; cap = 0; }
        size_t want = bytes + (bytes >= ((size_t)256 << 20) ? bytes / 64 : bytes / 8) + 256;
        hipError_t e = hipMalloc(&p, want);
        if (e == hipErrorOutOfMemory) {
            (void)hipGetLastError();
            if (rv_oom_trim()) e = hipMalloc(&p, want);
            if (e == hipErrorOutOfMemory) { (void)hipGetLastError(); want = bytes + 256; e = hipMalloc(&p, want); }
        }
        if (e != hipSuccess) { p = nullptr; rv_set_error("%s:%d hipMalloc(%zu bytes): %s", __FILE__, __LINE__, want, hipGetErrorString(e)); return -1; }
        cap = want;
        return 0;
    }
    void release() { if (p) (void)hipFree(p); p = nullptr; cap = 0; }
    template <class T> T *as() const { return (T *)p; }
};

struct RvPools {
    std::mutex mu;
    std::vector<std::pair<int, hipStream_t>> streams;
    struct Pin { int dev; void *p; size_t cap; };
    std::vector<Pin> pinned;
    size_t pinned_bytes = 0;
};
inline RvPools &rv_pools() { static RvPools *p = new RvPools(); return *p; }
inline hipError_t rv_stream_get(hipStream_t *s) {
    int dev = 0; (void)hipGetDevice(&dev);
    {
        RvPools &P = rv_pools();
        std::lock_guard<std::mutex> g(P.mu);
        for (size_t k = P.streams.size(); k-- > 0;)
            if (P.streams[k].first == dev) { *s = P.streams[k].second; P.streams.erase(P.streams.begin() + (ptrdiff_t)k); return hipSuccess; }
    }
    return hipStreamCreateWithFlags(s, hipStreamNonBlocking);
}
inline void rv_stream_put(hipStream_t s) {
    if (!s) return;
    (void)hipStreamSynchronize(s);
    int dev = 0; (void)hipGetDevice(&dev);
    RvPools &P = rv_pools();
    {
        std::lock_guard<std::mutex> g(P.mu);
        if (P.streams.size() < 64) { P.streams.push_back({dev, s}); return; }
    }
    (void)hipStreamDestroy(s);
}
inline hipError_t rv_pinned_get(size_t bytes, void **p, size_t *cap) {
    int dev = 0; (void)hipGetDevice(&dev);
    {
        RvPools &P = rv_pools();
        std::lock_guard<std::mutex> g(P.mu);
// ... 116 lines not shown
```

Baseline: 23900.

## Compact live cascade lists, skip empty levels, finish small tails in one workgroup

The cascade level loop now counts live matches and witnesses after each batch and packs the lists into fresh buffers when the live fraction drops below a threshold. Kernels exit early when the level range is empty. Once the live set is small enough, the remaining levels run inside a single-workgroup tail kernel that uses coherent atomic loads. The aim is to stop launching and scanning dead entries and to cut per-level launch overhead on the long shallow tail, at the cost of extra count, scan and pack kernels and more buffers.

After: 23710. Within noise of the previous version (-0.8%).

```diff
diff --git a/include/reveal_amd.h b/include/reveal_amd.h
--- a/include/reveal_amd.h
+++ b/include/reveal_amd.h
@@ -88,6 +88,7 @@
 int rv_frontier_seeds_import(rv_index *h, int nsubs, const int64_t *words, int64_t nwords);
 uint32_t rv_maxlcp(const rv_index *h);
 int rv_cascade_info(const rv_index *h, int64_t *out);
+int rv_cascade_tail_info(const rv_index *h, int64_t *out);
 int rv_capacity_events(const rv_index *h, int64_t *out);
 const char *rv_cascade_why(const rv_index *h);
 int64_t rv_anchor_count(rv_index *h, int64_t *members);
diff --git a/reveal_amd/_index.py b/reveal_amd/_index.py
--- a/reveal_amd/_index.py
+++ b/reveal_amd/_index.py
@@ -602,6 +602,11 @@
             return dict(done=bool(o[0]), levels=int(o[1]), matches=int(o[2]), witnesses=int(o[3]), subindices=int(o[4]), undecided=int(o[5]), rebuilt_ranks=int(o[6]), decided_from_witnesses=int(o[7]),
                         why=(self._dll.rv_cascade_why(self._h) or b"").decode())
 
+        def cascade_tail_info(self):
+            o = np.zeros(4, dtype=np.int64)
+            self._dll.rv_cascade_tail_info(self._h, o.ctypes.data)
+            return dict(compactions=int(o[0]), tail_entries=int(o[1]), tail_from=int(o[2]), tail_levels=int(o[3]))
+
         def capacity_events(self):
             o = np.zeros(len(_lib.CAPACITY_EVENTS), dtype=np.int64)
             if self._dll.rv_capacity_events(self._main._h, o.ctypes.data) != 0:
diff --git a/reveal_amd/_lib.py b/reveal_amd/_lib.py
--- a/reveal_amd/_lib.py
+++ b/reveal_amd/_lib.py
@@ -83,6 +83,7 @@
     "rv_frontier_seeds_import": (_I, [V, _I, V, _L]),
     "rv_maxlcp": (ctypes.c_uint32, [V]),
     "rv_cascade_info": (ctypes.c_int, [V, V]),
+    "rv_cascade_tail_info": (ctypes.c_int, [V, V]),
     "rv_cascade_why": (ctypes.c_char_p, [V]),
     "rv_capacity_events": (_I, [V, V]),
     "rv_anchor_count": (_L, [V, c_i64p]),
diff --git a/reveal_amd/csrc/rv_align.hip b/reveal_amd/csrc/rv_align.hip
--- a/reveal_amd/csrc/rv_align.hip
+++ b/reveal_amd/csrc/rv_align.hip
@@ -1975,6 +1975,14 @@
     return 0;
 }
 
+int rv_cascade_tail_info(const rv_index *h, int64_t *out) {
+    for (int k = 0; k < 4; k++) out[k] = 0;
+    if (!h->al) return 0;
+    const RvCascadeOut &c = h->al->cas_out;
+    out[0] = c.compactions; out[1] = c.tail_entries; out[2] = c.tail_from; out[3] = c.tail_levels;
+    return 0;
+}
+
 const char *rv_cascade_why(const rv_index *h) {
     if (!h->al || h->al->cas_out.done || !h->al->cas_out.why) return "";
     return h->al->cas_out.why;
diff --git a/reveal_amd/csrc/rv_cascade.h b/reveal_amd/csrc/rv_cascade.h
--- a/reveal_amd/csrc/rv_cascade.h
+++ b/reveal_amd/csrc/rv_cascade.h
@@ -3,7 +3,7 @@
 #include <vector>
 
 struct RvCascadeBufs {
-    DBuf d[40];
+    DBuf d[43];
     HBuf hstage, hstage2;
     u32 M = 0, NW = 0;
     u32 lin_roots = 0, lin_picks = 0, lin_nA = 0, lin_nB = 0;
@@ -37,6 +37,7 @@
     int64_t cands, witnesses, children, undecided, rebuilt_ranks;
     int64_t solved, unsolved;
     const char *why;
+    int64_t compactions, tail_entries, tail_from, tail_levels;
     u32 sent;
 };
 
diff --git a/reveal_amd/csrc/rv_cascade.hip b/reveal_amd/csrc/rv_cascade.hip
--- a/reveal_amd/csrc/rv_cascade.hip
+++ b/reveal_amd/csrc/rv_cascade.hip
@@ -21,7 +21,9 @@
 struct CasIv { sa_t a0, a1, b0, b1; };
 struct CasRes { sa_t qa, qb; u32 ql, lead, trail, state; };
 enum { C_NCHILD = 0, C_NUND = 1, C_NWIT = 2, C_ERR = 3, C_MAXN = 4, C_LO = 5, C_HI = 6, C_LEVELS = 7, C_NSOLVED = 8, C_NUNSOLVED = 9, C_NRETRY = 10, C_TICKET = 11,
-       C_NANCH = 12  };
+       C_NANCH = 12 ,
+       C_LIVEM = 13, C_LIVEW = 14 ,
+       C_TAILLV = 15  };
 
 __device__ inline bool cas_cut(const CasIv &iv, int64_t pa, int64_t pb, int64_t len, int64_t minl, int64_t *qa, int64_t *qb, int64_t *ql) {
     const int64_t ka = (int64_t)iv.a0 - pa, kb = (int64_t)iv.b0 - pb;
@@ -222,91 +224,111 @@
     if (i < M) { const u32 f = perm[i]; o_pa[i] = c_pa[f]; o_pb[i] = c_pb[f]; o_len[i] = c_len[f]; }
 }
 
-constexpr int CAS_ITEMS = 4;
-__global__ __launch_bounds__(TB) void k_cas_assign(const sa_t *__restrict__ c_pa, const sa_t *__restrict__ c_pb, const u32 *__restrict__ c_len, u32 *__restrict__ c_child,
-                                                   u32 M, const sa_t *__restrict__ w_pos, const u32 *__restrict__ w_val, u32 *__restrict__ w_child, u32 NW,
-                                                   const CasIv *__restrict__ iv, const CasRes *__restrict__ res, u64 *__restrict__ best, u32 *__restrict__ wmax,
-                                                   int64_t minl, int first, const u64 *__restrict__ ceil ) {
-    const u32 mblocks = (M + TB * CAS_ITEMS - 1) / (TB * CAS_ITEMS);
-    for (int it = 0; it < CAS_ITEMS; it++) {
-    if (blockIdx.x < mblocks) {
-        const u32 i = (blockIdx.x * CAS_ITEMS + (u32)it) * TB + threadIdx.x;
-        u32 c = i < M ? c_child[i] : NONE;
-        bool live = c != NONE;
-        u64 key = 0;
-        if (live) {
-            const int64_t pa = (int64_t)c_pa[i], pb = (int64_t)c_pb[i], len = (int64_t)c_len[i];
-            int64_t qa, qb, ql;
-            if (!first) {
-                const CasRes r = res[c];
-                const CasIv p = iv[c];
-                u32 nc = NONE;
-                if (r.state == 1u) {
-                    CasIv lv; lv.a0 = p.a0; lv.a1 = r.qa; lv.b0 = p.b0; lv.b1 = r.qb;
-                    CasIv tv; tv.a0 = (sa_t)((int64_t)r.qa + r.ql); tv.a1 = p.a1; tv.b0 = (sa_t)((int64_t)r.qb + r.ql); tv.b1 = p.b1;
-                    if (r.lead != NONE && cas_cut(lv, pa, pb, len, minl, &qa, &qb, &ql)) nc = r.lead;
-                    else if (r.trail != NONE && cas_cut(tv, pa, pb, len, minl, &qa, &qb, &ql)) nc = r.trail;
-                } else if (r.state == 3u) {
-                    if (cas_cut(p, pa, pb, len, minl, &qa, &qb, &ql)) nc = r.lead;
-                }
-                c = nc;
-                c_child[i] = c;
-                live = c != NONE;
-            } else {
-                live = cas_cut(iv[c], pa, pb, len, minl, &qa, &qb, &ql);
-                if (!live) { c = NONE; c_child[i] = NONE; }
+template <bool COH> __device__ inline u64 cas_ld(const u64 *p) {
+    if (COH) return __hip_atomic_load(const_cast<u64 *>(p), __ATOMIC_RELAXED, __HIP_MEMORY_SCOPE_AGENT);
+    return *p;
+}
+template <bool COH> __device__ inline u32 cas_ld(const u32 *p) {
+    if (COH) return __hip_atomic_load(const_cast<u32 *>(p), __ATOMIC_RELAXED, __HIP_MEMORY_SCOPE_AGENT);
+    return *p;
+}
+__device__ inline void cas_assign_match(u32 i, const sa_t *c_pa, const sa_t *c_pb, const u32 *c_len, u32 *c_child, u32 M, const CasIv *iv, const CasRes *res,
+                                        u64 *best, int64_t minl, int first, const u64 *ceil) {
+    u32 c = i < M ? c_child[i] : NONE;
+    bool live = c != NONE;
+    u64 key = 0;
+    if (live) {
+        const int64_t pa = (int64_t)c_pa[i], pb = (int64_t)c_pb[i], len = (int64_t)c_len[i];
+        int64_t qa, qb, ql;
+        if (!first) {
+            const CasRes r = res[c];
+            const CasIv p = iv[c];
+            u32 nc = NONE;
+            if (r.state == 1u) {
+                CasIv lv; lv.a0 = p.a0; lv.a1 = r.qa; lv.b0 = p.b0; lv.b1 = r.qb;
+                CasIv tv; tv.a0 = (sa_t)((int64_t)r.qa + r.ql); tv.a1 = p.a1; tv.b0 = (sa_t)((int64_t)r.qb + r.ql); tv.b1 = p.b1;
+                if (r.lead != NONE && cas_cut(lv, pa, pb, len, minl, &qa, &qb, &ql)) nc = r.lead;
+                else if (r.trail != NONE && cas_cut(tv, pa, pb, len, minl, &qa, &qb, &ql)) nc = r.trail;
+            } else if (r.state == 3u) {
+                if (cas_cut(p, pa, pb, len, minl, &qa, &qb, &ql)) nc = r.lead;
             }
-            if (live) key = cas_key(qa, ql);
-        }
-        bool bid = live;
-        if (live && ceil) { const u64 ce = ceil[c]; bid = ce == 0 || key < ce; }
-        seg_atomic_max64(best, c, key, bid);
-    } else {
-        const u32 i = ((blockIdx.x - mblocks) * CAS_ITEMS + (u32)it) * TB + threadIdx.x;
-        u32 c = i < NW ? w_child[i] : NONE;
-        bool live = c != NONE;
-        u32 v = 0;
-        if (live) {
-            const int64_t pos = (int64_t)w_pos[i];
-            v = w_val[i];
-            if (!first) {
-                const CasRes r = res[c];
-                const CasIv p = iv[c];
-                u32 nc = NONE;
-                if (r.state == 1u) {
-                    const int64_t ea = (int64_t)r.qa + r.ql, eb = (int64_t)r.qb + r.ql;
-                    const bool in_lead = (pos >= p.a0 && pos < r.qa) || (pos >= p.b0 && pos < r.qb);
-                    const bool in_trail = (pos >= ea && pos < p.a1) || (pos >= eb && pos < p.b1);
-                    nc = in_lead ? r.lead : in_trail ? r.trail : NONE;
-                } else if (r.state == 3u) nc = r.lead;
-                c = nc;
-                w_child[i] = c;
-                live = c != NONE;
-            } else {
-                const CasIv p = iv[c];
-                live = (pos >= p.a0 && pos < p.a1) || (pos >= p.b0 && pos < p.b1);
-                if (!live) { c = NONE; w_child[i] = NONE; }
-            }
-        }
-        seg_atomic_max32(wmax, c, v, live);
-    }
-    }
-}
-
-__global__ __launch_bounds__(TB) void k_cas_winner(const sa_t *__restrict__ c_pa, const sa_t *__restrict__ c_pb, const u32 *__restrict__ c_len,
-                                                   const u32 *__restrict__ c_child, u32 M, const CasIv *__restrict__ iv, CasRes *__restrict__ res,
-                                                   const u64 *__restrict__ best, int64_t minl) {
-    const u32 i = blockIdx.x * TB + threadIdx.x;
+            c = nc;
+            c_child[i] = c;
+            live = c != NONE;
+        } else {
+            live = cas_cut(iv[c], pa, pb, len, minl, &qa, &qb, &ql);
+            if (!live) { c = NONE; c_child[i] = NONE; }
+        }
+        if (live) key = cas_key(qa, ql);
+    }
+    bool bid = live;
+    if (live && ceil) { const u64 ce = ceil[c]; bid = ce == 0 || key < ce; }
+    seg_atomic_max64(best, c, key, bid);
+}
+__device__ inline void cas_assign_witness(u32 i, const sa_t *w_pos, const u32 *w_val, u32 *w_child, u32 NW, const CasIv *iv, const CasRes *res, u32 *wmax, int first) {
+    u32 c = i < NW ? w_child[i] : NONE;
+    bool live = c != NONE;
+    u32 v = 0;
+    if (live) {
+        const int64_t pos = (int64_t)w_pos[i];
+        v = w_val[i];
+        if (!first) {
+            const CasRes r = res[c];
+            const CasIv p = iv[c];
+            u32 nc = NONE;
+            if (r.state == 1u) {
+                const int64_t ea = (int64_t)r.qa + r.ql, eb = (int64_t)r.qb + r.ql;
+                const bool in_lead = (pos >= p.a0 && pos < r.qa) || (pos >= p.b0 && pos < r.qb);
+                const bool in_trail = (pos >= ea && pos < p.a1) || (pos >= eb && pos < p.b1);
+                nc = in_lead ? r.lead : in_trail ? r.trail : NONE;
+            } else if (r.state == 3u) nc = r.lead;
+            c = nc;
+            w_child[i] = c;
+            live = c != NONE;
+        } else {
+            const CasIv p = iv[c];
+            live = (pos >= p.a0 && pos < p.a1) || (pos >= p.b0 && pos < p.b1);
+            if (!live) { c = NONE; w_child[i] = NONE; }
+        }
+    }
+    seg_atomic_max32(wmax, c, v, live);
+}
+template <bool COH>
+__device__ inline void cas_winner_match(u32 i, const sa_t *c_pa, const sa_t *c_pb, const u32 *c_len, const u32 *c_child, u32 M, const CasIv *iv, CasRes *res,
+                                        const u64 *best, int64_t minl) {
     if (i >= M) return;
     const u32 c = c_child[i];
     if (c == NONE) return;
     int64_t qa, qb, ql;
     if (!cas_cut(iv[c], (int64_t)c_pa[i], (int64_t)c_pb[i], (int64_t)c_len[i], minl, &qa, &qb, &ql)) return;
-    if (cas_key(qa, ql) == best[c]) { res[c].qa = (sa_t)qa; res[c].qb = (sa_t)qb; res[c].ql = (u32)ql; }
+    if (cas_key(qa, ql) == cas_ld<COH>(&best[c])) { res[c].qa = (sa_t)qa; res[c].qb = (sa_t)qb; res[c].ql = (u32)ql; }
+}
+
+constexpr int CAS_ITEMS = 4;
+__global__ __launch_bounds__(TB) void k_cas_assign(const sa_t *__restrict__ c_pa, const sa_t *__restrict__ c_pb, const u32 *__restrict__ c_len, u32 *__restrict__ c_child,
+                                                   u32 M, const sa_t *__restrict__ w_pos, const u32 *__restrict__ w_val, u32 *__restrict__ w_child, u32 NW,
+                                                   const CasIv *__restrict__ iv, const CasRes *__restrict__ res, u64 *__restrict__ best, u32 *__restrict__ wmax,
+                                                   int64_t minl, int first, const u64 *__restrict__ ceil ,
+                                                   const u32 *__restrict__ range ) {
+    if (range && range[C_LO] == range[C_HI]) return;
+    const u32 mblocks = (M + TB * CAS_ITEMS - 1) / (TB * CAS_ITEMS);
+    for (int it = 0; it < CAS_ITEMS; it++) {
+        if (blockIdx.x < mblocks) cas_assign_match((blockIdx.x * CAS_ITEMS + (u32)it) * TB + threadIdx.x, c_pa, c_pb, c_len, c_child, M, iv, res, best, minl, first, ceil);
+        else cas_assign_witness(((blockIdx.x - mblocks) * CAS_ITEMS + (u32)it) * TB + threadIdx.x, w_pos, w_val, w_child, NW, iv, res, wmax, first);
+    }
+}
+
+__global__ __launch_bounds__(TB) void k_cas_winner(const sa_t *__restrict__ c_pa, const sa_t *__restrict__ c_pb, const u32 *__restrict__ c_len,
+                                                   const u32 *__restrict__ c_child, u32 M, const CasIv *__restrict__ iv, CasRes *__restrict__ res,
+                                                   const u64 *__restrict__ best, int64_t minl, const u32 *__restrict__ range) {
+    if (range && range[C_LO] == range[C_HI]) return;
+    cas_winner_match<false>(blockIdx.x * TB + threadIdx.x, c_pa, c_pb, c_len, c_child, M, iv, res, best, minl);
 }
 
 constexpr u32 DWALK = 1024;
-struct CasDanger { u64 *best; u32 *flag; sa_t *qb; u64 *ceil; u32 *m1, *p1, *m2; u64 *key; const uint8_t *T0; const lcp_t *LCP; const u64 *rank; u32 leaf_n; uint8_t *dflag; const uint8_t *wcls; };
+struct CasDanger { u64 *best; u32 *flag; sa_t *qb; u64 *ceil; u32 *m1, *p1, *m2; u64 *key; const uint8_t *T0; const lcp_t *LCP; const u64 *rank; u32 leaf_n; uint8_t *dflag; const uint8_t *wcls;
+                   const u32 *range ; };
+__device__ inline bool cas_range_empty(const u32 *range) { return range && range[C_LO] == range[C_HI]; }
 __device__ inline bool cas_is_danger(const CasIv &p, u64 bk, u32 wm, u32 minl, u32 leaf_n, u32 *theta) {
     const int64_t la = (int64_t)p.a1 - p.a0, lb = (int64_t)p.b1 - p.b0;
     const u32 bl = (u32)(bk >> KEY_SHIFT);
@@ -325,7 +347,7 @@
 __global__ __launch_bounds__(TB) void k_cas_dwalk(const sa_t *__restrict__ w_pos, const u32 *__restrict__ w_val, const u32 *__restrict__ w_child, u32 NW,
                                                   const CasIv *__restrict__ iv, const u64 *__restrict__ best, const u32 *__restrict__ wmax, u32 minl, CasDanger dg) {
     const u32 i = blockIdx.x * TB + threadIdx.x;
-    if (i >= NW) return;
+    if (i >= NW || cas_range_empty(dg.range)) return;
     if (dg.wcls && dg.wcls[i]) return;
     const u32 c = w_child[i];
     if (c == NONE || !dg.dflag[c]) return;
@@ -395,6 +417,7 @@
     __shared__ u32 cc[BLK_MAX], vv[BLK_MAX], ll[BLK_MAX];
     __shared__ sa_t pp[BLK_MAX];
     __shared__ u32 s_any;
+    if (cas_range_empty(dg.range)) return;
     const u32 b = mlist[blockIdx.x];
     const u32 s0 = boff[b], size = boff[b + 1] - s0;
     if (threadIdx.x == 0) s_any = 0;
@@ -450,7 +473,7 @@
                                                   const CasIv *__restrict__ iv, const CasRes *__restrict__ res, const u64 *__restrict__ best, const u32 *__restrict__ wmax,
                                                   u32 minl, CasDanger dg) {
     const u32 i = blockIdx.x * TB + threadIdx.x;
-    if (i >= NW) return;
+    if (i >= NW || cas_range_empty(dg.range)) return;
     const u32 c = w_child[i];
     if (c == NONE || !dg.dflag[c]) return;
     const CasIv p = iv[c];
@@ -479,7 +502,7 @@
 }
 __global__ __launch_bounds__(TB) void k_cas_dwrite(const sa_t *__restrict__ w_pos, const u32 *__restrict__ w_child, u32 NW, CasDanger dg) {
     const u32 i = blockIdx.x * TB + threadIdx.x;
-    if (i >= NW) return;
+    if (i >= NW || cas_range_empty(dg.range)) return;
     const u32 c = w_child[i];
     if (c == NONE || !dg.dflag[c]) return;
     const u64 key = dg.key[i];
@@ -487,103 +510,109 @@
     if (key == dg.best[c]) dg.qb[c] = w_pos[dg.p1[i]];
 }
 
+template <int NT, bool COH>
+__device__ inline void cas_decide_stretch(u32 first, u32 hi, CasIv *iv, u64 *best, u32 *wmax, int32_t *depth, CasRes *res, u32 minl, u32 *counters, u32 child_cap,
+                                          u32 *und_list, u32 leaf_n, const RvCascadeIO &io, const CasDanger &dg, int danger, u32 (*s_cnt)[3], u32 *s_base) {
+    const int lane = threadIdx.x & 63, w = threadIdx.x >> 6;
+    const u64 lt = (lane == 0) ? 0ull : (~0ull >> (64 - lane));
+    const u32 id = first + threadIdx.x;
+    const bool in = id < hi;
+    CasIv p; p.a0 = p.a1 = p.b0 = p.b1 = 0;
+    u64 bk = 0; u32 wm = 0; int32_t dp = 0;
+    CasRes r; r.qa = r.qb = 0; r.ql = 0; r.lead = r.trail = NONE; r.state = 2;
+    if (in) { p = iv[id]; bk = cas_ld<COH>(&best[id]); wm = cas_ld<COH>(&wmax[id]); dp = depth[id]; r = res[id]; }
+    const int64_t la = (int64_t)p.a1 - p.a0, lb = (int64_t)p.b1 - p.b0;
+    const u32 bl = (u32)(bk >> KEY_SHIFT);
+    const bool can = in & (la >= (int64_t)minl) & (lb >= (int64_t)minl);
+    bool split = can & (bl >= minl) & (bl > wm);
+    bool und = can & !split & (wm >= minl);
+    bool forced = false, retry = false;
+    if (danger && und && (u64)(la + lb) > (u64)dg.leaf_n) {
+        const u32 fl = dg.flag[id];
+        const u64 kh = dg.best[id], kc = (bl >= minl && !(fl & 1u)) ? bk : 0ull;
+        if (!(fl & 2u)) {
+            if (kh == 0 && kc == 0) {
+                if (bl < minl) und = false;
+                else if ((fl >> 8) < 16u) { retry = true; und = false; }
+            } else {
+                if (kh > kc) { r.qa = (sa_t)(KEY_LOW - (kh & KEY_LOW)); r.qb = dg.qb[id]; r.ql = (u32)(kh >> KEY_SHIFT); }
+                split = true; forced = true; und = false;
+            }
+        }
+        if (!retry) atomicAdd(&counters[und ? C_NUNSOLVED : C_NSOLVED], 1u);
+    }
+    bool lead = retry, trail = false;
+    if (split) {
+        if (!forced && r.ql != bl) atomicOr(&counters[C_ERR], 2u);
+        lead = ((int64_t)r.qa - p.a0) + ((int64_t)r.qb - p.b0) > 0;
+        trail = ((int64_t)p.a1 - r.qa - r.ql) + ((int64_t)p.b1 - r.qb - r.ql) > 0;
+    }
+    const u64 b_lead = __ballot(lead), b_trail = __ballot(trail), b_split = __ballot(split), b_und = __ballot(und);
+    if (retry) atomicAdd(&counters[C_NRETRY], 1u);
+    if (lane == 0) { s_cnt[w][0] = (u32)__popcll(b_lead) + (u32)__popcll(b_trail); s_cnt[w][1] = (u32)__popcll(b_split); s_cnt[w][2] = (u32)__popcll(b_und); }
+    __syncthreads();
+    if (threadIdx.x < 3) {
+        u32 tot = 0;
+        for (int k = 0; k < NT / 64; k++) tot += s_cnt[k][threadIdx.x];
+        u32 *ctr = threadIdx.x == 0 ? &counters[C_NCHILD] : threadIdx.x == 1 ? io.anchor_count : &counters[C_NUND];
+        s_base[threadIdx.x] = tot ? atomicAdd(ctr, tot) : 0u;
+    }
+    __syncthreads();
+    u32 base_c = s_base[0], base_a = s_base[1], base_u = s_base[2];
+    for (int k = 0; k < w; k++) { base_c += s_cnt[k][0]; base_a += s_cnt[k][1]; base_u += s_cnt[k][2]; }
+    if (retry) {
+        const u32 slot = base_c + (u32)__popcll(b_lead & lt) + (u32)__popcll(b_trail & lt);
+        CasRes nr; nr.qa = 0; nr.qb = 0; nr.ql = 0; nr.lead = NONE; nr.trail = NONE; nr.state = 0;
+        if (slot < child_cap) {
+            iv[slot] = p; best[slot] = 0; wmax[slot] = 0; depth[slot] = dp; res[slot] = nr;
+            dg.best[slot] = 0; dg.flag[slot] = ((dg.flag[id] >> 8) + 1u) << 8; dg.ceil[slot] = bk;
+            r.lead = slot; r.trail = NONE;
+        } else atomicOr(&counters[C_ERR], 1u);
+        r.state = 3;
+    } else if (split) {
+        u32 slot = base_c + (u32)__popcll(b_lead & lt) + (u32)__popcll(b_trail & lt);
+        CasRes nr; nr.qa = 0; nr.qb = 0; nr.ql = 0; nr.lead = NONE; nr.trail = NONE; nr.state = 0;
+        if (lead) {
+            if (slot < child_cap) {
+                CasIv c; c.a0 = p.a0; c.a1 = r.qa; c.b0 = p.b0; c.b1 = r.qb;
+                iv[slot] = c; best[slot] = 0; wmax[slot] = 0; depth[slot] = dp + 1; res[slot] = nr;
+                if (danger) { dg.best[slot] = 0; dg.flag[slot] = 0; dg.ceil[slot] = 0; }
+                r.lead = slot;
+            } else atomicOr(&counters[C_ERR], 1u);
+            slot++;
+        }
+        if (trail) {
+            if (slot < child_cap) {
+                CasIv c; c.a0 = (sa_t)((int64_t)r.qa + r.ql); c.a1 = p.a1; c.b0 = (sa_t)((int64_t)r.qb + r.ql); c.b1 = p.b1;
+                iv[slot] = c; best[slot] = 0; wmax[slot] = 0; depth[slot] = dp + 1; res[slot] = nr;
+                if (danger) { dg.best[slot] = 0; dg.flag[slot] = 0; dg.ceil[slot] = 0; }
+                r.trail = slot;
+            } else atomicOr(&counters[C_ERR], 1u);
+        }
+        const u32 as = base_a + (u32)__popcll(b_split & lt);
+        if (as < io.anchor_cap) { io.anchor_l[as] = r.ql; io.anchor_pos[2 * (size_t)as] = (int64_t)r.qa; io.anchor_pos[2 * (size_t)as + 1] = (int64_t)r.qb; }
+        else atomicOr(&counters[C_ERR], 4u);
+        r.state = 1;
+    } else {
+        r.state = 2;
+    }
+    if (in) res[id] = r;
+    if (und) {
+        und_list[base_u + (u32)__popcll(b_und & lt)] = id;
+        if ((u64)(la + lb) > (u64)leaf_n) atomicMax(&counters[C_MAXN], (u32)((la + lb) > 0xFFFFFFFFll ? 0xFFFFFFFFll : (la + lb)));
+    }
+    __syncthreads();
+}
+
 __global__ __launch_bounds__(TB) void k_cas_decide(CasIv *__restrict__ iv, u64 *__restrict__ best, u32 *__restrict__ wmax, int32_t *__restrict__ depth,
                                                    CasRes *__restrict__ res, u32 minl, u32 *__restrict__ counters, u32 child_cap,
-                                                   u32 *__restrict__ und_list, u32 leaf_n, RvCascadeIO io, CasDanger dg, int danger) {
+                                                   u32 *__restrict__ und_list, u32 leaf_n, RvCascadeIO io, CasDanger dg, int danger, int skip_empty) {
     __shared__ u32 s_cnt[TB / 64][3];
     __shared__ u32 s_base[3];
     const u32 lo = counters[C_LO], hi = counters[C_HI];
-    const int lane = threadIdx.x & 63, w = threadIdx.x >> 6;
-    const u64 lt = (lane == 0) ? 0ull : (~0ull >> (64 - lane));
-    for (u32 first = lo + blockIdx.x * TB; first < hi; first += gridDim.x * TB) {
-        const u32 id = first + threadIdx.x;
-        const bool in = id < hi;
-        CasIv p; p.a0 = p.a1 = p.b0 = p.b1 = 0;
-        u64 bk = 0; u32 wm = 0; int32_t dp = 0;
-        CasRes r; r.qa = r.qb = 0; r.ql = 0; r.lead = r.trail = NONE; r.state = 2;
-        if (in) { p = iv[id]; bk = best[id]; wm = wmax[id]; dp = depth[id]; r = res[id]; }
-        const int64_t la = (int64_t)p.a1 - p.a0, lb = (int64_t)p.b1 - p.b0;
-        const u32 bl = (u32)(bk >> KEY_SHIFT);
-        const bool can = in & (la >= (int64_t)minl) & (lb >= (int64_t)minl);
-        bool split = can & (bl >= minl) & (bl > wm);
-        bool und = can & !split & (wm >= minl);
-        bool forced = false, retry = false;
-        if (danger && und && (u64)(la + lb) > (u64)dg.leaf_n) {
-            const u32 fl = dg.flag[id];
-            const u64 kh = dg.best[id], kc = (bl >= minl && !(fl & 1u)) ? bk : 0ull;
-            if (!(fl & 2u)) {
-                if (kh == 0 && kc == 0) {
-                    if (bl < minl) und = false;
-                    else if ((fl >> 8) < 16u) { retry = true; und = false; }
-                } else {
-                    if (kh > kc) { r.qa = (sa_t)(KEY_LOW - (kh & KEY_LOW)); r.qb = dg.qb[id]; r.ql = (u32)(kh >> KEY_SHIFT); }
-                    split = true; forced = true; und = false;
-                }
-            }
-            if (!retry) atomicAdd(&counters[und ? C_NUNSOLVED : C_NSOLVED], 1u);
-        }
-        bool lead = retry, trail = false;
-        if (split) {
-            if (!forced && r.ql != bl) atomicOr(&counters[C_ERR], 2u);
-            lead = ((int64_t)r.qa - p.a0) + ((int64_t)r.qb - p.b0) > 0;
-            trail = ((int64_t)p.a1 - r.qa - r.ql) + ((int64_t)p.b1 - r.qb - r.ql) > 0;
-        }
-        const u64 b_lead = __ballot(lead), b_trail = __ballot(trail), b_split = __ballot(split), b_und = __ballot(und);
-        if (retry) atomicAdd(&counters[C_NRETRY], 1u);
-        if (lane == 0) { s_cnt[w][0] = (u32)__popcll(b_lead) + (u32)__popcll(b_trail); s_cnt[w][1] = (u32)__popcll(b_split); s_cnt[w][2] = (u32)__popcll(b_und); }
-        __syncthreads();
-        if (threadIdx.x < 3) {
-            u32 tot = 0;
-            for (int k = 0; k < TB / 64; k++) tot += s_cnt[k][threadIdx.x];
-            u32 *ctr = threadIdx.x == 0 ? &counters[C_NCHILD] : threadIdx.x == 1 ? io.anchor_count : &counters[C_NUND];
-            s_base[threadIdx.x] = tot ? atomicAdd(ctr, tot) : 0u;
-        }
-        __syncthreads();
-        u32 base_c = s_base[0], base_a = s_base[1], base_u = s_base[2];
-        for (int k = 0; k < w; k++) { base_c += s_cnt[k][0]; base_a += s_cnt[k][1]; base_u += s_cnt[k][2]; }
-        if (retry) {
-            const u32 slot = base_c + (u32)__popcll(b_lead & lt) + (u32)__popcll(b_trail & lt);
-            CasRes nr; nr.qa = 0; nr.qb = 0; nr.ql = 0; nr.lead = NONE; nr.trail = NONE; nr.state = 0;
-            if (slot < child_cap) {
-                iv[slot] = p; best[slot] = 0; wmax[slot] = 0; depth[slot] = dp; res[slot] = nr;
-                dg.best[slot] = 0; dg.flag[slot] = ((dg.flag[id] >> 8) + 1u) << 8; dg.ceil[slot] = bk;
-                r.lead = slot; r.trail = NONE;
-            } else atomicOr(&counters[C_ERR], 1u);
-            r.state = 3;
-        } else if (split) {
-            u32 slot = base_c + (u32)__popcll(b_lead & lt) + (u32)__popcll(b_trail & lt);
-            CasRes nr; nr.qa = 0; nr.qb = 0; nr.ql = 0; nr.lead = NONE; nr.trail = NONE; nr.state = 0;
-            if (lead) {
-                if (slot < child_cap) {
-                    CasIv c; c.a0 = p.a0; c.a1 = r.qa; c.b0 = p.b0; c.b1 = r.qb;
-                    iv[slot] = c; best[slot] = 0; wmax[slot] = 0; depth[slot] = dp + 1; res[slot] = nr;
-                    if (danger) { dg.best[slot] = 0; dg.flag[slot] = 0; dg.ceil[slot] = 0; }
-                    r.lead = slot;
-                } else atomicOr(&counters[C_ERR], 1u);
-                slot++;
-            }
-            if (trail) {
-                if (slot < child_cap) {
-                    CasIv c; c.a0 = (sa_t)((int64_t)r.qa + r.ql); c.a1 = p.a1; c.b0 = (sa_t)((int64_t)r.qb + r.ql); c.b1 = p.b1;
-                    iv[slot] = c; best[slot] = 0; wmax[slot] = 0; depth[slot] = dp + 1; res[slot] = nr;
-                    if (danger) { dg.best[slot] = 0; dg.flag[slot] = 0; dg.ceil[slot] = 0; }
-                    r.trail = slot;
-                } else atomicOr(&counters[C_ERR], 1u);
-            }
-            const u32 as = base_a + (u32)__popcll(b_split & lt);
-            if (as < io.anchor_cap) { io.anchor_l[as] = r.ql; io.anchor_pos[2 * (size_t)as] = (int64_t)r.qa; io.anchor_pos[2 * (size_t)as + 1] = (int64_t)r.qb; }
-            else atomicOr(&counters[C_ERR], 4u);
-            r.state = 1;
-        } else {
-            r.state = 2;
-        }
-        if (in) res[id] = r;
-        if (und) {
-            und_list[base_u + (u32)__popcll(b_und & lt)] = id;
-            if ((u64)(la + lb) > (u64)leaf_n) atomicMax(&counters[C_MAXN], (u32)((la + lb) > 0xFFFFFFFFll ? 0xFFFFFFFFll : (la + lb)));
-        }
-        __syncthreads();
-    }
+    if (skip_empty && lo == hi) return;
+    for (u32 first = lo + blockIdx.x * TB; first < hi; first += gridDim.x * TB)
+        cas_decide_stretch<TB, false>(first, hi, iv, best, wmax, depth, res, minl, counters, child_cap, und_list, leaf_n, io, dg, danger, s_cnt, s_base);
     if (threadIdx.x == 0) {
         __threadfence();
         if (atomicAdd(&counters[C_TICKET], 1u) == gridDim.x - 1) {
@@ -595,6 +624,78 @@
         }
     }
 }
+__global__ __launch_bounds__(TB) void k_cas_count(const u32 *__restrict__ c_child, u32 M, const u32 *__restrict__ w_child, u32 NW, u32 *__restrict__ counters) {
+    __shared__ u32 s_n[TB / 64][2];
+    u32 nm = 0, nw = 0;
+    for (u32 i = blockIdx.x * TB + threadIdx.x; i < M; i += gridDim.x * TB) nm += c_child[i] != NONE;
+    for (u32 i = blockIdx.x * TB + threadIdx.x; i < NW; i += gridDim.x * TB) nw += w_child[i] != NONE;
+#pragma unroll
+    for (int d = 32; d >= 1; d >>= 1) { nm += __shfl_down(nm, d, 64); nw += __shfl_down(nw, d, 64); }
+    if ((threadIdx.x & 63) == 0) { s_n[threadIdx.x >> 6][0] = nm; s_n[threadIdx.x >> 6][1] = nw; }
+    __syncthreads();
+    if (threadIdx.x < 2) {
+        u32 t = 0;
+        for (int k = 0; k < TB / 64; k++) t += s_n[k][threadIdx.x];
+        if (t) atomicAdd(&counters[threadIdx.x == 0 ? C_LIVEM : C_LIVEW], t);
+    }
+}
+__global__ __launch_bounds__(TB) void k_cas_live_flags(const u32 *__restrict__ c_child, u32 M, const u32 *__restrict__ w_child, u32 NW, u32 *__restrict__ flag) {
+    const u32 i = blockIdx.x * TB + threadIdx.x;
+    if (i < M) flag[i] = c_child[i] != NONE;
+    else if (i < M + NW) flag[i] = w_child[i - M] != NONE;
+    else if (i == M + NW) flag[i] = 0;
+}
+struct CasLists { sa_t *pa, *pb; u32 *len, *child; sa_t *wpos; u32 *wval, *wchild; };
+__global__ __launch_bounds__(TB) void k_cas_live_emit(CasLists src, u32 M, u32 NW, const u32 *__restrict__ flag, const u32 *__restrict__ off, CasLists dst, u32 dM, u32 dNW) {
+    const u32 i = blockIdx.x * TB + threadIdx.x;
+    if (i >= M + NW || !flag[i]) return;
+    if (i < M) {
+        const u32 j = off[i];
+        if (j < dM) { dst.pa[j] = src.pa[i]; dst.pb[j] = src.pb[i]; dst.len[j] = src.len[i]; dst.child[j] = src.child[i]; }
+    } else {
+        const u32 j = off[i] - off[M];
+        if (j < dNW) { dst.wpos[j] = src.wpos[i - M]; dst.wval[j] = src.wval[i - M]; dst.wchild[j] = src.wchild[i - M]; }
+    }
+}
+
+constexpr int CAS_TAIL_TB = 1024;
+constexpr u32 CAS_TAIL_LEVELS = 64;
+__global__ __launch_bounds__(CAS_TAIL_TB) void k_cas_tail(const sa_t *c_pa, const sa_t *c_pb, const u32 *c_len, u32 *c_child, u32 M, const sa_t *w_pos, const u32 *w_val,
+                                                          u32 *w_child, u32 NW, CasIv *iv, u64 *best, u32 *wmax, int32_t *depth, CasRes *res, u32 minl, u32 *counters,
+                                                          u32 child_cap, u32 *und_list, u32 leaf_n, RvCascadeIO io, int first) {
+    __shared__ u32 s_cnt[CAS_TAIL_TB / 64][3];
+    __shared__ u32 s_base[3];
+    __shared__ u32 s_range[3];
+    if (threadIdx.x == 0) { s_range[0] = counters[C_LO]; s_range[1] = counters[C_HI]; s_range[2] = 0; }
+    __syncthreads();
+    const CasDanger dg = {};
+    u32 levels = 0;
+    for (; levels < CAS_TAIL_LEVELS; levels++) {
+        const u32 lo = s_range[0], hi = s_range[1];
+        if (lo == hi || s_range[2]) break;
+        const int fst = first && levels == 0;
+        for (u32 b = 0; b < M; b += CAS_TAIL_TB) cas_assign_match(b + threadIdx.x, c_pa, c_pb, c_len, c_child, M, iv, res, best, (int64_t)minl, fst, nullptr);
+        for (u32 b = 0; b < NW; b += CAS_TAIL_TB) cas_assign_witness(b + threadIdx.x, w_pos, w_val, w_child, NW, iv, res, wmax, fst);
+        __threadfence(); __syncthreads();
+        for (u32 b = 0; b < M; b += CAS_TAIL_TB) cas_winner_match<true>(b + threadIdx.x, c_pa, c_pb, c_len, c_child, M, iv, res, best, (int64_t)minl);
+        __threadfence(); __syncthreads();
+        for (u32 f = lo; f < hi; f += CAS_TAIL_TB)
+            cas_decide_stretch<CAS_TAIL_TB, true>(f, hi, iv, best, wmax, depth, res, minl, counters, child_cap, und_list, leaf_n, io, dg, 0, s_cnt, s_base);
+        __threadfence(); __syncthreads();
+        if (threadIdx.x == 0) {
+            const u32 made = cas_ld<true>(&counters[C_NCHILD]);
+            s_range[0] = hi; s_range[1] = made < child_cap ? made : child_cap;
+            s_range[2] = (cas_ld<true>(&counters[C_ERR]) != 0u || cas_ld<true>(&counters[C_MAXN]) > leaf_n) ? 1u : 0u;
+        }
+        __syncthreads();
+    }
+    if (threadIdx.x == 0) {
+        counters[C_LO] = s_range[0]; counters[C_HI] = s_range[1];
+        counters[C_LEVELS] += levels; counters[C_TAILLV] += levels;
+        counters[C_NANCH] = cas_ld<true>(io.anchor_count);
+    }
+}
+
 __global__ __launch_bounds__(TB) void k_cas_stats(const u32 *__restrict__ counters, const int32_t *__restrict__ depth, RvCascadeIO io) {
     __shared__ unsigned long long s_bp[TB / 64];
     __shared__ u32 s_md[TB / 64];
@@ -845,8 +946,10 @@
 }
 
 int rv_cascade_run(rv_index *h, RvCascadeBufs &cb, const RvCascadeIO &io, int minl_in, RvCascadeOut *out, int danger, int reuse, const RvCascadeHost *host) {
+    const RvCascadeOut before = *out;
     memset(out, 0, sizeof *out);
     out->done = false;
+    if (reuse) { out->compactions = before.compactions; out->tail_entries = before.tail_entries; out->tail_from = before.tail_from; out->tail_levels = before.tail_levels; }
     Workspace &ws = h->ws;
     hipStream_t q = ws.stream;
     const int64_t n = h->n;
@@ -934,7 +1037,7 @@
     u32 *counters = bctr.as<u32>();
     RV_HIP(hipMemsetAsync(counters, 0, 64, q));
 
-    u32 hc[16];
+    u32 hc[16] = {0};
     u32 NW = reuse ? cb.NW : 0;
     if (!reuse) {
         u32 *wreg = bwr.as<u32>();
@@ -1063,7 +1166,6 @@
     }
 
     if (verbose) { (void)hipStreamSynchronize(q); tp[2] = cas_now(); }
-    const unsigned agrid = (unsigned)(ceil_div((int64_t)M, TB * CAS_ITEMS) + ceil_div((int64_t)NW, TB * CAS_ITEMS));
     const int batch = std::max(1, (int)ws.opt.cascade_batch);
     int queued = 0;
     RV_TRY(rv_working_text_begin(h, host ? host->side : nullptr));
@@ -1099,16 +1201,54 @@
         ws.stream = cb.prio_stream; prio.on = true;
         q = cb.prio_stream;
     }
+    const u32 *range = ws.opt.cascade_skip_empty ? (const u32 *)counters : nullptr;
+    dg.range = range;
+    const bool dwit = danger && NW;
+    const int64_t compact_pct = std::min<int64_t>(std::max<int64_t>(ws.opt.cascade_compact, 0), 100);
+    const u32 tail_cap = (danger || ws.opt.cascade_tail <= 0) ? 0u : (u32)std::min<int64_t>(ws.opt.cascade_tail, 1 << 20);
+    CasLists cur = {bpa.as<sa_t>(), bpb.as<sa_t>(), blen.as<u32>(), bcc.as<u32>(), const_cast<sa_t *>(wp), const_cast<u32 *>(wv), bwc.as<u32>()};
+    u32 curM = M, curNW = NW, seenM = 0, seenW = 0;
+    int packs = 0;
+    auto pack_live = [&](u32 liveM, u32 liveW) -> int {
+        if (danger) liveW = curNW;
+        DBuf &bto = cb.d[40 + (packs & 1)], &bfl = cb.d[42];
+        const size_t am = ((size_t)liveM + 15) & ~(size_t)15, aw = ((size_t)liveW + 15) & ~(size_t)15, tot = (size_t)curM + (danger ? 0 : curNW);
+        RV_TRY(bto.reserve(am * (2 * sizeof(sa_t) + 8) + aw * (sizeof(sa_t) + 8) + 64));
+        RV_TRY(bfl.reserve((tot + 16) * 8));
+        CasLists to = cur;
+        to.pa = bto.as<sa_t>(); to.pb = to.pa + am; to.len = (u32 *)(to.pb + am); to.child = to.len + am;
+        if (!danger) { to.wpos = (sa_t *)(to.child + am); to.wval = (u32 *)(to.wpos + aw); to.wchild = to.wval + aw; }
+        u32 *flag = bfl.as<u32>(), *off = flag + ((tot + 16) & ~(size_t)15);
+        const unsigned fb = (unsigned)ceil_div((int64_t)tot + 1, TB);
+        hipLaunchKernelGGL(k_cas_live_flags, dim3(fb), dim3(TB), 0, q, (const u32 *)cur.child, curM, (const u32 *)cur.wchild, danger ? 0u : curNW, flag);
+        RV_LAUNCH_CHECK();
+        RV_TRY(rv_exclusive_sum_u32(ws, flag, off, (int64_t)tot + 1));
+        hipLaunchKernelGGL(k_cas_live_emit, dim3(fb), dim3(TB), 0, q, cur, curM, danger ? 0u : curNW, (const u32 *)flag, (const u32 *)off, to, liveM, liveW);
+        RV_LAUNCH_CHECK();
+        cur = to; curM = liveM; curNW = liveW;
+        packs++; out->compactions++;
+        return 0;
+    };
+    bool tail_begun = false;
+    bool tail_next = tail_cap && (int64_t)M + NW <= (int64_t)tail_cap;
     for (;;) {
-        for (int b = 0; b < batch; b++, queued++) {
-            hipLaunchKernelGGL(k_cas_assign, dim3(agrid), dim3(TB), 0, q, (const sa_t *)bpa.as<sa_t>(), (const sa_t *)bpb.as<sa_t>(), (const u32 *)blen.as<u32>(), bcc.as<u32>(), M,
-                               wp, wv, bwc.as<u32>(), NW, (const CasIv *)biv.as<CasIv>(), (const CasRes *)bres.as<CasRes>(),
-                               bbest.as<u64>(), bwm.as<u32>(), (int64_t)minl, queued == 0 ? 1 : 0, (const u64 *)((danger && NW) ? dg.ceil : nullptr));
+        if (tail_next) {
+            if (!tail_begun) { tail_begun = true; out->tail_entries = (int64_t)curM + curNW; out->tail_from = (int64_t)hc[C_LEVELS]; out->tail_levels = 0; }
+            hipLaunchKernelGGL(k_cas_tail, dim3(1), dim3(CAS_TAIL_TB), 0, q, (const sa_t *)cur.pa, (const sa_t *)cur.pb, (const u32 *)cur.len, cur.child, curM,
+                               (const sa_t *)cur.wpos, (const u32 *)cur.wval, cur.wchild, curNW, biv.as<CasIv>(), bbest.as<u64>(), bwm.as<u32>(), bdep.as<int32_t>(),
+                               bres.as<CasRes>(), minl, counters, ccap_k, bund.as<u32>(), (u32)RV_LEAF_N, iok, queued == 0 ? 1 : 0);
             RV_LAUNCH_CHECK();
-            hipLaunchKernelGGL(k_cas_winner, dim3((unsigned)ceil_div((int64_t)M, TB)), dim3(TB), 0, q, (const sa_t *)bpa.as<sa_t>(), (const sa_t *)bpb.as<sa_t>(),
-                               (const u32 *)blen.as<u32>(), (const u32 *)bcc.as<u32>(), M, (const CasIv *)biv.as<CasIv>(), bres.as<CasRes>(), (const u64 *)bbest.as<u64>(), (int64_t)minl);
+            queued += (int)CAS_TAIL_LEVELS;
+        } else for (int b = 0; b < batch; b++, queued++) {
+            const unsigned agrid = (unsigned)(ceil_div((int64_t)curM, TB * CAS_ITEMS) + ceil_div((int64_t)curNW, TB * CAS_ITEMS));
+            hipLaunchKernelGGL(k_cas_assign, dim3(std::max(agrid, 1u)), dim3(TB), 0, q, (const sa_t *)cur.pa, (const sa_t *)cur.pb, (const u32 *)cur.len, cur.child, curM,
+                               (const sa_t *)cur.wpos, (const u32 *)cur.wval, cur.wchild, curNW, (const CasIv *)biv.as<CasIv>(), (const CasRes *)bres.as<CasRes>(),
+                               bbest.as<u64>(), bwm.as<u32>(), (int64_t)minl, queued == 0 ? 1 : 0, (const u64 *)(dwit ? dg.ceil : nullptr), range);
             RV_LAUNCH_CHECK();
-            if (danger && NW) {
+            hipLaunchKernelGGL(k_cas_winner, dim3((unsigned)std::max<int64_t>(1, ceil_div((int64_t)curM, TB))), dim3(TB), 0, q, (const sa_t *)cur.pa, (const sa_t *)cur.pb,
+                               (const u32 *)cur.len, (const u32 *)cur.child, curM, (const CasIv *)biv.as<CasIv>(), bres.as<CasRes>(), (const u64 *)bbest.as<u64>(), (int64_t)minl, range);
+            RV_LAUNCH_CHECK();
+            if (dwit) {
                 const unsigned wb = (unsigned)ceil_div((int64_t)NW, TB);
                 hipLaunchKernelGGL(k_cas_dmark, dim3(256), dim3(TB), 0, q, (const CasIv *)biv.as<CasIv>(), (const u64 *)bbest.as<u64>(), (const u32 *)bwm.as<u32>(), minl, (const u32 *)counters, dg);
                 RV_LAUNCH_CHECK();
@@ -1127,7 +1267,13 @@
                 RV_LAUNCH_CHECK();
             }
             hipLaunchKernelGGL(k_cas_decide, dim3(256), dim3(TB), 0, q, biv.as<CasIv>(), bbest.as<u64>(), bwm.as<u32>(), bdep.as<int32_t>(),
-                               bres.as<CasRes>(), minl, counters, ccap_k, bund.as<u32>(), (u32)RV_LEAF_N, iok, dg, (danger && NW) ? 1 : 0);
+                               bres.as<CasRes>(), minl, counters, ccap_k, bund.as<u32>(), (u32)RV_LEAF_N, iok, dg, dwit ? 1 : 0, range ? 1 : 0);
+            RV_LAUNCH_CHECK();
+        }
+        const bool counted = !tail_next && (compact_pct > 0 || tail_cap);
+        if (counted) {
+            const unsigned cg = (unsigned)std::min<int64_t>(256, std::max<int64_t>(1, ceil_div((int64_t)std::max(curM, curNW), TB * 8)));
+            hipLaunchKernelGGL(k_cas_count, dim3(cg), dim3(TB), 0, q, (const u32 *)cur.child, curM, (const u32 *)cur.wchild, curNW, counters);
             RV_LAUNCH_CHECK();
         }
         RV_TRY(send_known());
@@ -1135,9 +1281,18 @@
         if (hc[C_ERR] & ~5u) { rv_set_error("cascade: device error %u", hc[C_ERR]); return -1; }
         if (hc[C_ERR]) GIVE_UP("the cascade's tables are full");
         known = hc[C_NANCH];
+        if (tail_begun) out->tail_levels = hc[C_TAILLV];
         if (hc[C_MAXN] > (u32)RV_LEAF_N) break;
         if (hc[C_HI] == hc[C_LO]) break;
         if (queued > 1000000) { rv_set_error("cascade: no progress"); return -1; }
+        if (counted) {
+            const u32 liveM = hc[C_LIVEM] - seenM, liveW = hc[C_LIVEW] - seenW;
+            seenM = hc[C_LIVEM]; seenW = hc[C_LIVEW];
+            if (liveM > curM || liveW > curNW) { rv_set_error("cascade: more live entries than entries"); return -1; }
+            const int64_t live = (int64_t)liveM + (danger ? curNW : liveW), len = (int64_t)curM + curNW;
+            tail_next = tail_cap && live <= (int64_t)tail_cap;
+            if (live < len && (tail_next || (compact_pct > 0 && live * 100 <= len * compact_pct))) RV_TRY(pack_live(liveM, liveW));
+        }
     }
     prio.leave(); q = ws.stream;
     const int level = (int)hc[C_LEVELS];
@@ -1194,8 +1349,8 @@
     }
     if (verbose) {
         (void)hipStreamSynchronize(q); tp[4] = cas_now();
-        fprintf(stderr, "cascade%s: %u matches, %u witnesses, %d levels, %u sub-indices, %u undecided (%lld ranks rebuilt), %lld decided from witnesses | ms: scan %.2f witnesses+sort %.2f levels %.2f rebuild+leaf %.2f\n",
-                danger ? " (second attempt)" : "", M, NW, level, hi, U, (long long)out->rebuilt_ranks, (long long)out->solved, (tp[1] - tp[0]) * 1e3, (tp[2] - tp[1]) * 1e3, (tp[3] - tp[2]) * 1e3, (tp[4] - tp[3]) * 1e3);
+        fprintf(stderr, "cascade%s: %u matches, %u witnesses, %d levels, %u sub-indices, %u undecided (%lld ranks rebuilt), %lld decided from witnesses, lists packed %lld times, one workgroup from level %lld (%lld entries) for %lld levels | ms: scan %.2f witnesses+sort %.2f levels %.2f rebuild+leaf %.2f\n",
+                danger ? " (second attempt)" : "", M, NW, level, hi, U, (long long)out->rebuilt_ranks, (long long)out->solved, (long long)out->compactions, (long long)(out->tail_entries ? out->tail_from : -1), (long long)out->tail_entries, (long long)out->tail_levels, (tp[1] - tp[0]) * 1e3, (tp[2] - tp[1]) * 1e3, (tp[3] - tp[2]) * 1e3, (tp[4] - tp[3]) * 1e3);
     }
     out->done = true;
     out->sent = sent;
diff --git a/reveal_amd/csrc/rv_common.h b/reveal_amd/csrc/rv_common.h
--- a/reveal_amd/csrc/rv_common.h
+++ b/reveal_amd/csrc/rv_common.h
@@ -102,7 +102,10 @@
     X(cas_witness_pass, "RV_CAS_WITNESS_PASS", 0) \
     X(cap_limit, "RV_CAP_LIMIT", 0) \
     X(cap_sites, "RV_CAP_SITES", -1) \
-    X(many_chain_multi, "RV_MANY_CHAIN_MULTI", 0)
+    X(many_chain_multi, "RV_MANY_CHAIN_MULTI", 0) \
+    X(cascade_skip_empty, "RV_CASCADE_SKIP_EMPTY", 1) \
+    X(cascade_compact, "RV_CASCADE_COMPACT", 25) \
+    X(cascade_tail, "RV_CASCADE_TAIL", 8192)
 struct RvOptions {
 #define RV_X_(f, name, def) int64_t f = def;
     RV_OPTION_LIST(RV_X_)
```
